# aerius-labs/zksnap-circuits-halo2

Measured on AMD Instinct MI355X. Metric: BN254 G1 MSM Mpoints/sec, higher is better.
Workload: dtype u32x9 (254-bit modular integer, radix 2^29); 1 GPU; BN254 G1 MSM, 2^20 random points/scalars per GPU (BASELINE configs[1]), point-range sharded x1, inputs resident in HBM, bases registered once (prepared fixed-base table, as under ParamsKZG::commit); points_per_gpu=1048576, parallelism=point-range shard x1 + all_gather(96 B) + fold

## Files before the change

zksnap_circuits_halo2_amd/csrc/msm.hip:

```cpp
#include <hip/hip_runtime.h>
#include <atomic>
#include <cstdint>
#include <cstdio>
#include <cstring>
#include <cstdlib>
#include <mutex>
#include "ec_quad.hpp"
#include "fe_inverse.hpp"
#include "zkhip_internal.hpp"

namespace zkhip {

static inline size_t align_up(size_t v, size_t a) { return (v + a - 1) / a * a; }

constexpr int FINE_BITS = 12;
constexpr int MAX_GROUPS = 128;
constexpr int MAX_WIDE_W = 16;
struct win_layout { int c, W, narrow; };
__host__ __device__ __forceinline__ int win_bits(const win_layout& L, int w) { return w < L.W - L.narrow ? L.c : L.c - 1; }
__host__ __device__ __forceinline__ int win_off(const win_layout& L, int w) { const int full = L.W - L.narrow; return w <= full ? w * L.c : full * L.c + (w - full) * (L.c - 1); }
static int msm_narrow_windows(int c, int W) {
  static const bool uniform = getenv("ZKHIP_UNIFORM_WINDOWS") != nullptr;
  if (c <= 16 || uniform) return 0;
  const int narrow = W * c - 256;
  return narrow > 0 && narrow <= W ? narrow : 0;
}
constexpr int MAX_TASK_LEN = 128;
constexpr int TASK_SHIFT = 6;

struct task_t {
  uint32_t bucket, start, len;
};

__device__ __forceinline__ xyzz load_xyzz(const uint32_t* base, size_t idx) {
  const uint4* q = reinterpret_cast<const uint4*>(base + idx * 36);
  uint32_t w[36];
#pragma unroll
  for (int i = 0; i < 9; i++) {
    uint4 v = q[i];
    w[4 * i] = v.x; w[4 * i + 1] = v.y; w[4 * i + 2] = v.z; w[4 * i + 3] = v.w;
  }
  xyzz r;
#pragma unroll
  for (int i = 0; i < 9; i++) { r.X.l[i] = w[i]; r.Y.l[i] = w[9 + i]; r.ZZ.l[i] = w[18 + i]; r.ZZZ.l[i] = w[27 + i]; }
  return r;
}

__device__ __forceinline__ void store_xyzz(uint32_t* base, size_t idx, const xyzz& a) {
  uint32_t w[36];
#pragma unroll
  for (int i = 0; i < 9; i++) { w[i] = a.X.l[i]; w[9 + i] = a.Y.l[i]; w[18 + i] = a.ZZ.l[i]; w[27 + i] = a.ZZZ.l[i]; }
  uint4* q = reinterpret_cast<uint4*>(base + idx * 36);
#pragma unroll
  for (int i = 0; i < 9; i++) q[i] = make_uint4(w[4 * i], w[4 * i + 1], w[4 * i + 2], w[4 * i + 3]);
}

__device__ __forceinline__ xyzz xyzz_shfl_xor(const xyzz& a, int mask) {
  xyzz r;
#pragma unroll
  for (int i = 0; i < NL; i++) {
    r.X.l[i] = (uint32_t)__shfl_xor((int)a.X.l[i], mask, 64);
    r.Y.l[i] = (uint32_t)__shfl_xor((int)a.Y.l[i], mask, 64);
    r.ZZ.l[i] = (uint32_t)__shfl_xor((int)a.ZZ.l[i], mask, 64);
    r.ZZZ.l[i] = (uint32_t)__shfl_xor((int)a.ZZZ.l[i], mask, 64);
  }
  return r;
}

__device__ __forceinline__ fe load_fe9_generic(const uint32_t* p, size_t idx) {
  fe r;
#pragma unroll
  for (int i = 0; i < 9; i++) r.l[i] = p[idx * 9 + i];
  return r;
}
__device__ __forceinline__ void store_fe9_generic(uint32_t* p, size_t idx, const fe& a) {
#pragma unroll
  for (int i = 0; i < 9; i++) p[idx * 9 + i] = a.l[i];
}

template <typename DIGIT>
__global__ void __launch_bounds__(256) k_digits(const uint32_t* __restrict__ scalars, DIGIT* __restrict__ digits,
                                                uint32_t n, uint32_t n_pad, int c, int W, uint32_t K, size_t scalar_stride, int narrow) {
  const size_t idx = (size_t)blockIdx.x * blockDim.x + threadIdx.x;
  if (idx >= (size_t)K * n_pad) return;
  const uint32_t kb = (uint32_t)(idx / n_pad), i = (uint32_t)(idx % n_pad);
  digits += (size_t)kb * n_pad;
  const size_t row = (size_t)K * n_pad;
  if (i >= n) {
    for (int win = 0; win < W; win++) digits[(size_t)win * row + i] = 0;
    return;
  }
  uint32_t w[8];
  load_words(scalars + ((size_t)kb * scalar_stride + i) * 8, w);
  fe c32;
#pragma unroll
  for (int k = 0; k < NL; k++) c32.l[k] = FrParams::FROM_EXT_CANON[k];
  fe s = fe_canon_lt2p<FrParams>(fe_mul<FrParams>(c32, fe_unpack<0>(w)));
  fe_pack(s, w);
  const win_layout lay{c, W, narrow};
  uint32_t carry = 0;
  for (int win = 0; win < W; win++) {
    const int bit = win_off(lay, win), cw = win_bits(lay, win);
    const uint32_t half = 1u << (cw - 1), mask = (1u << cw) - 1;
    uint32_t v = 0;
    if (bit < 256) {
      int wi = bit >> 5, sh = bit & 31;
      uint64_t two = w[wi];
      if (wi + 1 < 8) two |= (uint64_t)w[wi + 1] << 32;
      v = (uint32_t)(two >> sh) & mask;
    }
    v += carry;
    int32_t d;
    if (v >= half) { d = (int32_t)v - (int32_t)(1u << cw); carry = 1; } else { d = (int32_t)v; carry = 0; }
    digits[(size_t)win * row + i] = (DIGIT)d;
  }
}

__global__ void __launch_bounds__(1024) k_digits_wide(const uint32_t* __restrict__ scalars, int32_t* __restrict__ digits, uint32_t n, uint32_t n_pad,
                                                       int c, int W, uint32_t* __restrict__ gcount, int narrow) {
  __shared__ uint32_t cnt[MAX_WIDE_W * MAX_GROUPS];
  for (uint32_t t = threadIdx.x; t < (uint32_t)W * MAX_GROUPS; t += blockDim.x) cnt[t] = 0;
  __syncthreads();
  const win_layout lay{c, W, narrow};
  for (uint32_t i = blockIdx.x * blockDim.x + threadIdx.x; i < n_pad; i += gridDim.x * blockDim.x) {
    if (i >= n) {
      for (int win = 0; win < W; win++) digits[(size_t)win * n_pad + i] = 0;
      continue;
    }
    uint32_t w[8];
    load_words(scalars + (size_t)i * 8, w);
    fe c32;
#pragma unroll
    for (int k = 0; k < NL; k++) c32.l[k] = FrParams::FROM_EXT_CANON[k];
    fe sv = fe_canon_lt2p<FrParams>(fe_mul<FrParams>(c32, fe_unpack<0>(w)));
    fe_pack(sv, w);
    uint32_t carry = 0;
    for (int win = 0; win < W; win++) {
      const int bit = win_off(lay, win), cw = win_bits(lay, win);
      const uint32_t half = 1u << (cw - 1), mask = (1u << cw) - 1;
      uint32_t v = 0;
      if (bit < 256) {
        const int wi = bit >> 5, sh = bit & 31;
        uint64_t two = w[wi];
        if (wi + 1 < 8) two |= (uint64_t)w[wi + 1] << 32;
        v = (uint32_t)(two >> sh) & mask;
      }
      v += carry;
      int32_t d;
      if (v >= half) { d = (int32_t)v - (int32_t)(1u << cw); carry = 1; } else { d = (int32_t)v; carry = 0; }
      digits[(size_t)win * n_pad + i] = d;
      if (d != 0) atomicAdd(&cnt[win * MAX_GROUPS + (((uint32_t)(d < 0 ? -d : d) - 1) >> FINE_BITS)], 1u);
    }
  }
  __syncthreads();
  for (uint32_t t = threadIdx.x; t < (uint32_t)W * MAX_GROUPS; t += blockDim.x)
    if (cnt[t]) atomicAdd(&gcount[t], cnt[t]);
}

namespace glv {
__device__ constexpr uint32_t G1[3] = {0xc7e0b3d7u, 0xd91d232eu, 0x2u};
__device__ constexpr uint32_t G2[5] = {0x391eb18eu, 0x7a7bd9d4u, 0xa773d2cfu, 0x4ccef014u, 0x2u};
__device__ constexpr uint32_t A1[2] = {0x94d213e3u, 0x89d32568u};
__device__ constexpr uint32_t A2[4] = {0x1221250bu, 0x0be4e154u, 0xeeb859fdu, 0x6f4d8248u};
__device__ constexpr uint32_t NB1[4] = {0x7d4f1128u, 0x8211bbebu, 0xeeb859fcu, 0x6f4d8248u};
__device__ constexpr uint32_t BETA_EXT[8] = {0xd782e155u, 0x71930c11u, 0xffbe3323u, 0xa6bb947cu, 0xd4741444u, 0xaa303344u, 0x26594943u, 0x2c3b3f0du};

template <int NA, int NB, int NO>
__device__ __forceinline__ void mul_low(const uint32_t (&a)[NA], const uint32_t* __restrict__ b, uint32_t (&out)[NO]) {
#pragma unroll
  for (int i = 0; i < NO; i++) out[i] = 0;
#pragma unroll
  for (int i = 0; i < NA; i++) {
    uint32_t carry = 0;
#pragma unroll
    for (int j = 0; j < NB; j++) {
      if (i + j < NO) {
        const uint64_t t = (uint64_t)a[i] * b[j] + out[i + j] + carry;
        out[i + j] = (uint32_t)t;
        carry = (uint32_t)(t >> 32);
      }
    }
    if (i + NB < NO) out[i + NB] = carry;
  }
}

__device__ __forceinline__ bool abs160(uint32_t (&v)[5], uint32_t (&mag)[4]) {
  const bool neg = (v[4] >> 31) != 0;
  uint32_t carry = neg ? 1u : 0u;
#pragma unroll
  for (int i = 0; i < 4; i++) {
    const uint32_t w = neg ? ~v[i] : v[i];
    const uint32_t t = w + carry;
    carry = (t < w) ? 1u : 0u;
    mag[i] = t;
  }
  return neg;
}

__device__ __forceinline__ void decompose(const uint32_t (&k)[8], uint32_t (&m1)[4], bool& s1, uint32_t (&m2)[4], bool& s2) {
  uint32_t t1[11], t2[13];
  mul_low<8, 3, 11>(k, G1, t1);
  mul_low<8, 5, 13>(k, G2, t2);
  const uint32_t c1[2] = {t1[8], t1[9]};
  const uint32_t c2[4] = {t2[8], t2[9], t2[10], t2[11]};
  uint32_t p[5], q[5], v[5];
  mul_low<2, 2, 5>(c1, A1, p);
  mul_low<4, 4, 5>(c2, A2, q);
  uint64_t borrow = 0;
#pragma unroll
  for (int i = 0; i < 5; i++) {
    const uint64_t d = (uint64_t)k[i] - p[i] - q[i] - borrow;
    v[i] = (uint32_t)d;
    borrow = (d >> 32) ? ((~(d >> 32) + 1) & 3) : 0;
  }
  s1 = abs160(v, m1);
  mul_low<2, 4, 5>(c1, NB1, p);
  mul_low<4, 2, 5>(c2, A1, q);
  borrow = 0;
#pragma unroll
  for (int i = 0; i < 5; i++) {
    const uint64_t d = (uint64_t)p[i] - q[i] - borrow;
    v[i] = (uint32_t)d;
    borrow = (d >> 32) ? 1 : 0;
  }
  s2 = abs160(v, m2);
}
}

template <typename DIGIT>
__global__ void __launch_bounds__(256) k_digits_glv(const uint32_t* __restrict__ scalars, DIGIT* __restrict__ digits, uint32_t n, uint32_t n2_pad, int c, int W) {
  const uint32_t i = blockIdx.x * blockDim.x + threadIdx.x;
  if (i < n2_pad - 2 * n) {
    for (int win = 0; win < W; win++) digits[(size_t)win * n2_pad + 2 * n + i] = 0;
  }
  if (i >= n) return;
  uint32_t w[8];
  load_words(scalars + (size_t)i * 8, w);
  fe c32;
#pragma unroll
  for (int k = 0; k < NL; k++) c32.l[k] = FrParams::FROM_EXT_CANON[k];
  fe s = fe_canon_lt2p<FrParams>(fe_mul<FrParams>(c32, fe_unpack<0>(w)));
  fe_pack(s, w);
  uint32_t m[2][4];
  bool neg[2];
  glv::decompose(w, m[0], neg[0], m[1], neg[1]);
  const uint32_t half = 1u << (c - 1), mask = (1u << c) - 1;
#pragma unroll
  for (int h = 0; h < 2; h++) {
    uint32_t carry = 0;
    DIGIT* col = digits + (size_t)h * n + i;
    for (int win = 0; win < W; win++) {
      const int bit = win * c;
      uint32_t v = 0;
      if (bit < 128) {
        const int wi = bit >> 5, sh = bit & 31;
        uint64_t two = m[h][wi];
        if (wi + 1 < 4) two |= (uint64_t)m[h][wi + 1] << 32;
        v = (uint32_t)(two >> sh) & mask;
      }
      v += carry;
      int32_t d;
      if (neg[h] ? (v > half) : (v >= half)) { d = (int32_t)v - (int32_t)(1u << c); carry = 1; } else { d = (int32_t)v; carry = 0; }
      col[(size_t)win * n2_pad] = (DIGIT)(neg[h] ? -d : d);
    }
  }
}

__global__ void __launch_bounds__(256) k_endo_bases(const uint32_t* __restrict__ bases, uint32_t n, uint32_t* __restrict__ endo) {
  const uint32_t i = blockIdx.x * blockDim.x + threadIdx.x;
  if (i >= n) return;
  affine_words pt = load_affine(bases, i);
  uint32_t bw[8], xw[8];
#pragma unroll
  for (int k = 0; k < 8; k++) bw[k] = glv::BETA_EXT[k];
  const fe beta = fe_mul<Fq>(fe_one<Fq>(), fe_from_ext_lazy(bw));
  fe_to_ext<Fq>(fe_mul<Fq>(beta, fe_from_ext_lazy(pt.x)), xw);
  uint4* o = reinterpret_cast<uint4*>(endo + (size_t)i * 16);
  o[0] = make_uint4(xw[0], xw[1], xw[2], xw[3]);
  o[1] = make_uint4(xw[4], xw[5], xw[6], xw[7]);
  o[2] = make_uint4(pt.y[0], pt.y[1], pt.y[2], pt.y[3]);
  o[3] = make_uint4(pt.y[4], pt.y[5], pt.y[6], pt.y[7]);
}

template <bool SCATTER>
__global__ void __launch_bounds__(1024) k_sort_pass(const int16_t* __restrict__ digits, uint32_t n_pad, uint32_t chunk,
                                                    int c, uint32_t* __restrict__ count_or_cursor,
                                                    uint32_t* __restrict__ sorted, uint32_t win_bucket_stride,
                                                    uint32_t ref_base, uint32_t ref_stride) {
  extern __shared__ uint32_t hist[];
  const uint32_t B = 1u << (c - 1);
  const int win = blockIdx.y;
  const uint32_t kb = blockIdx.z, K = gridDim.z;
  const uint32_t lo = blockIdx.x * chunk;
  const uint32_t hi = min(n_pad, lo + chunk);
  for (uint32_t b = threadIdx.x; b < B; b += blockDim.x) hist[b] = 0;
  __syncthreads();
  const uint4* dv = reinterpret_cast<const uint4*>(digits + ((size_t)win * K + kb) * n_pad);
  const uint32_t v_lo = lo >> 3, v_hi = hi >> 3;
  for (uint32_t vi = v_lo + threadIdx.x; vi < v_hi; vi += blockDim.x) {
    const uint4 q = dv[vi];
    const uint32_t w[4] = {q.x, q.y, q.z, q.w};
#pragma unroll
    for (int k = 0; k < 8; k++) {
      const int d = (int16_t)(w[k >> 1] >> ((k & 1) * 16));
      if (d != 0) atomicAdd(&hist[(d < 0 ? -d : d) - 1], 1u);
    }
  }
  __syncthreads();
  uint32_t* g = count_or_cursor + (size_t)win * win_bucket_stride + (size_t)kb * B;
  if (!SCATTER) {
    for (uint32_t b = threadIdx.x; b < B; b += blockDim.x) {
      uint32_t v = hist[b];
      if (v) atomicAdd(&g[b], v);
    }
  } else {
    for (uint32_t b0 = threadIdx.x; b0 < B; b0 += 8 * blockDim.x) {
      uint32_t v[8], r[8];
#pragma unroll
      for (int k = 0; k < 8; k++) { const uint32_t b = b0 + k * blockDim.x; v[k] = b < B ? hist[b] : 0u; }
#pragma unroll
      for (int k = 0; k < 8; k++) r[k] = v[k] ? atomicAdd(&g[b0 + k * blockDim.x], v[k]) : 0u;
#pragma unroll
      for (int k = 0; k < 8; k++) { const uint32_t b = b0 + k * blockDim.x; if (b < B) hist[b] = r[k]; }
    }
    __syncthreads();
    const uint32_t rbase = ref_base + (uint32_t)win * ref_stride;
    for (uint32_t vi = v_lo + threadIdx.x; vi < v_hi; vi += blockDim.x) {
      const uint4 q = dv[vi];
      const uint32_t w[4] = {q.x, q.y, q.z, q.w};
#pragma unroll
      for (int k = 0; k < 8; k++) {
        const int d = (int16_t)(w[k >> 1] >> ((k & 1) * 16));
        if (d != 0) {
          const uint32_t pos = atomicAdd(&hist[(d < 0 ? -d : d) - 1], 1u);
          sorted[pos] = (rbase + vi * 8 + k) | (d < 0 ? 0x80000000u : 0u);
        }
      }
    }
  }
}



__global__ void __launch_bounds__(1024) k_coarse_count(const int32_t* __restrict__ digits, uint32_t n_pad, uint32_t chunk, uint32_t* __restrict__ gcount, uint32_t gstride) {
  __shared__ uint32_t cnt[MAX_GROUPS];
  const int win = blockIdx.y;
  const uint32_t lo = blockIdx.x * chunk, hi = min(n_pad, lo + chunk);
  if (threadIdx.x < MAX_GROUPS) cnt[threadIdx.x] = 0;
  __syncthreads();
  const uint4* dv = reinterpret_cast<const uint4*>(digits + (size_t)win * n_pad);
  const uint32_t v_lo = lo >> 2, v_hi = hi >> 2;
  for (uint32_t vi = v_lo + threadIdx.x; vi < v_hi; vi += 4 * blockDim.x) {
    uint4 q[4];
#pragma unroll
    for (int u = 0; u < 4; u++) { const uint32_t vj = vi + u * blockDim.x; q[u] = vj < v_hi ? dv[vj] : make_uint4(0, 0, 0, 0); }
#pragma unroll
    for (int u = 0; u < 4; u++) {
      const int32_t d4[4] = {(int32_t)q[u].x, (int32_t)q[u].y, (int32_t)q[u].z, (int32_t)q[u].w};
#pragma unroll
      for (int k = 0; k < 4; k++) {
        const int32_t d = d4[k];
        if (d != 0) atomicAdd(&cnt[(uint32_t)win * gstride + (((uint32_t)(d < 0 ? -d : d) - 1) >> FINE_BITS)], 1u);
      }
    }
  }
  __syncthreads();
  if (threadIdx.x < MAX_GROUPS && cnt[threadIdx.x]) atomicAdd(&gcount[win * MAX_GROUPS + threadIdx.x], cnt[threadIdx.x]);
}

constexpr uint32_t COARSE_CHUNK = 8192;
__global__ void __launch_bounds__(1024) k_coarse_sorted(const int32_t* __restrict__ digits, uint32_t n_pad, uint32_t* __restrict__ gcursor,
                                                        uint32_t* __restrict__ stage_ref, uint16_t* __restrict__ stage_fine,
                                                        uint32_t ref_base, uint32_t ref_stride, uint32_t gstride) {
  __shared__ uint32_t cur[MAX_GROUPS], delta[MAX_GROUPS];
  __shared__ uint32_t refs[COARSE_CHUNK];
  __shared__ uint16_t fines[COARSE_CHUNK];
  __shared__ uint32_t mask[COARSE_CHUNK / 32], wpre[COARSE_CHUNK / 32];
  const int win = blockIdx.y;
  const uint32_t gbase = (uint32_t)win * gstride;
  const uint32_t lo = blockIdx.x * COARSE_CHUNK, hi = min(n_pad, lo + COARSE_CHUNK);
  if (lo >= hi) return;
  if (threadIdx.x < MAX_GROUPS) cur[threadIdx.x] = 0;
  if (threadIdx.x < COARSE_CHUNK / 32) mask[threadIdx.x] = 0;
  __syncthreads();
  const uint4* dv = reinterpret_cast<const uint4*>(digits + (size_t)win * n_pad);
  const uint32_t v_lo = lo >> 2, v_hi = hi >> 2;
  static_assert(COARSE_CHUNK == 8192, "a lane owns two 4-digit vectors of the chunk");
  const uint32_t vi = v_lo + threadIdx.x, vj = vi + 1024u;
  const uint4 q0 = vi < v_hi ? dv[vi] : make_uint4(0, 0, 0, 0), q1 = vj < v_hi ? dv[vj] : make_uint4(0, 0, 0, 0);
  const int32_t d8[8] = {(int32_t)q0.x, (int32_t)q0.y, (int32_t)q0.z, (int32_t)q0.w, (int32_t)q1.x, (int32_t)q1.y, (int32_t)q1.z, (int32_t)q1.w};
#pragma unroll
  for (int k = 0; k < 8; k++) {
    const int32_t d = d8[k];
    if (d != 0) atomicAdd(&cur[gbase + (((uint32_t)(d < 0 ? -d : d) - 1) >> FINE_BITS)], 1u);
  }
  __syncthreads();
  if (threadIdx.x < 64) {
    const uint32_t c0 = cur[2 * threadIdx.x], c1 = cur[2 * threadIdx.x + 1], s = c0 + c1;
    uint32_t x = s;
#pragma unroll
    for (int off = 1; off < 64; off <<= 1) {
      const uint32_t y = __shfl_up(x, off, 64);
      if ((int)threadIdx.x >= off) x += y;
    }
    const uint32_t l0 = x - s, l1 = l0 + c0;
    uint32_t* const wcur = gcursor + (uint32_t)win * MAX_GROUPS;
    const uint32_t g0 = c0 ? atomicAdd(&wcur[2 * threadIdx.x], c0) : 0u, g1 = c1 ? atomicAdd(&wcur[2 * threadIdx.x + 1], c1) : 0u;
    cur[2 * threadIdx.x] = l0; cur[2 * threadIdx.x + 1] = l1;
    const uint32_t nz = (c0 != 0) + (c1 != 0);
    uint32_t y = nz;
#pragma unroll
    for (int off = 1; off < 64; off <<= 1) {
      const uint32_t t = __shfl_up(y, off, 64);
      if ((int)threadIdx.x >= off) y += t;
    }
    uint32_t rank = y - nz;
    if (c0) { delta[rank++] = g0 - l0; atomicOr(&mask[l0 >> 5], 1u << (l0 & 31)); }
    if (c1) { delta[rank] = g1 - l1; atomicOr(&mask[l1 >> 5], 1u << (l1 & 31)); }
    __threadfence_block();
    uint32_t pc[4], ps = 0;
#pragma unroll
    for (int k = 0; k < 4; k++) { pc[k] = (uint32_t)__popc(mask[4 * threadIdx.x + k]); ps += pc[k]; }
    uint32_t z = ps;
#pragma unroll
    for (int off = 1; off < 64; off <<= 1) {
      const uint32_t t = __shfl_up(z, off, 64);
      if ((int)threadIdx.x >= off) z += t;
    }
    uint32_t zb = z - ps;
#pragma unroll
    for (int k = 0; k < 4; k++) { wpre[4 * threadIdx.x + k] = zb; zb += pc[k]; }
  }
  __syncthreads();
  const uint32_t rbase = ref_base + (uint32_t)win * ref_stride;
#pragma unroll
  for (int k = 0; k < 8; k++) {
    const int32_t d = d8[k];
    if (d != 0) {
      const uint32_t b = (uint32_t)(d < 0 ? -d : d) - 1;
      const uint32_t pos = atomicAdd(&cur[gbase + (b >> FINE_BITS)], 1u);
      refs[pos] = (rbase + (k < 4 ? vi : vj) * 4 + (k & 3)) | (d < 0 ? 0x80000000u : 0u);
      fines[pos] = (uint16_t)(b & ((1u << FINE_BITS) - 1));
    }
  }
  __syncthreads();
  const uint32_t total = cur[MAX_GROUPS - 1];
  for (uint32_t i = threadIdx.x; i < total; i += blockDim.x) {
    const uint32_t r = wpre[i >> 5] + (uint32_t)__popc(mask[i >> 5] & ((2u << (i & 31)) - 1u)) - 1u;
    const uint32_t pos = delta[r] + i;
    stage_ref[pos] = refs[i];
    stage_fine[pos] = fines[i];
  }
}

constexpr uint32_t SORT_CHUNK = 28672;

__global__ void __launch_bounds__(64) k_group_offsets(const uint32_t* __restrict__ wcount, int W, int G, uint32_t* __restrict__ goff, uint32_t* __restrict__ wcursor,
                                                       uint32_t* __restrict__ cstart, uint32_t chunk) {
  if (blockIdx.x != 0 || threadIdx.x >= 64) return;
  const int lane = threadIdx.x;
  uint32_t c0 = 0, c1 = 0;
  for (int w = 0; w < W; w++) {
    if (2 * lane < G) c0 += wcount[w * MAX_GROUPS + 2 * lane];
    if (2 * lane + 1 < G) c1 += wcount[w * MAX_GROUPS + 2 * lane + 1];
  }
  const uint32_t k0 = (c0 + chunk - 1) / chunk, k1 = (c1 + chunk - 1) / chunk;
  uint32_t x = c0 + c1, y = k0 + k1;
#pragma unroll
  for (int off = 1; off < 64; off <<= 1) {
    const uint32_t xs = __shfl_up(x, off, 64), ys = __shfl_up(y, off, 64);
    if (lane >= off) { x += xs; y += ys; }
  }
  const uint32_t ex = x - (c0 + c1), ey = y - (k0 + k1);
  if (2 * lane < G) { goff[2 * lane] = ex; cstart[2 * lane] = ey; }
  if (2 * lane + 1 < G) { goff[2 * lane + 1] = ex + c0; cstart[2 * lane + 1] = ey + k0; }
  uint32_t r0 = ex, r1 = ex + c0;
  for (int w = 0; w < W; w++) {
    if (2 * lane < G) { wcursor[w * MAX_GROUPS + 2 * lane] = r0; r0 += wcount[w * MAX_GROUPS + 2 * lane]; }
    if (2 * lane + 1 < G) { wcursor[w * MAX_GROUPS + 2 * lane + 1] = r1; r1 += wcount[w * MAX_GROUPS + 2 * lane + 1]; }
  }
  if (lane == 63) { goff[G] = x; cstart[G] = y; }
}

#ifndef ZKHIP_FINE_BATCH
#define ZKHIP_FINE_BATCH 7
#endif
constexpr int FINE_BATCH = ZKHIP_FINE_BATCH;
__device__ __forceinline__ void fine_histogram(const uint16_t* __restrict__ stage_fine, uint32_t start, uint32_t end, uint32_t* __restrict__ cur) {
  for (uint32_t p = start + threadIdx.x; p < end; p += FINE_BATCH * blockDim.x) {
    uint32_t f[FINE_BATCH];
#pragma unroll
    for (int k = 0; k < FINE_BATCH; k++) { const uint32_t q = p + k * blockDim.x; f[k] = q < end ? stage_fine[q] : 0xffffffffu; }
#pragma unroll
    for (int k = 0; k < FINE_BATCH; k++) if (f[k] != 0xffffffffu) atomicAdd(&cur[f[k]], 1u);
  }
}

__global__ void __launch_bounds__(1024) k_fine_sorted(const uint16_t* __restrict__ stage_fine, const uint32_t* __restrict__ stage_ref,
                                                      const uint32_t* __restrict__ goff, const uint32_t* __restrict__ cstart, int G,
                                                      uint32_t* __restrict__ cursor, uint32_t* __restrict__ sorted) {
  extern __shared__ uint32_t hist[];
  constexpr uint32_t FB = 1u << FINE_BITS;
  constexpr uint32_t CHUNK = SORT_CHUNK;
  static_assert(FB == 4096, "one thread owns four buckets in the scan");
  __shared__ uint32_t wsum[16];
  uint32_t* cur = hist;
  uint32_t* delta = hist + FB;
  uint32_t* refs = hist + 2 * FB;
  const uint32_t w = blockIdx.x;
  if (w >= cstart[G]) return;
  uint32_t glo = 0, ghi = (uint32_t)G;
  while (ghi - glo > 1) { const uint32_t mid = (glo + ghi) >> 1; if (cstart[mid] <= w) glo = mid; else ghi = mid; }
  const uint32_t g = glo;
  const uint32_t start = goff[g] + (w - cstart[g]) * CHUNK, end = min(goff[g + 1], start + CHUNK), cnt_n = end - start;
  for (uint32_t b = threadIdx.x; b < FB; b += blockDim.x) cur[b] = 0;
  __syncthreads();
  fine_histogram(stage_fine, start, end, cur);
  __syncthreads();
  uint32_t c[4], l[4], s = 0;
#pragma unroll
  for (int k = 0; k < 4; k++) { c[k] = cur[4 * threadIdx.x + k]; s += c[k]; }
  const int lane = threadIdx.x & 63, wave = threadIdx.x >> 6;
  uint32_t x = s;
#pragma unroll
  for (int off = 1; off < 64; off <<= 1) {
    const uint32_t y = __shfl_up(x, off, 64);
    if (lane >= off) x += y;
  }
  if (lane == 63) wsum[wave] = x;
  __syncthreads();
  uint32_t before = 0;
#pragma unroll
  for (int i = 0; i < 16; i++) if (i < wave) before += wsum[i];
  uint32_t run = before + x - s;
  uint32_t* gl = cursor + (size_t)g * FB;
  uint32_t gb[4];
#pragma unroll
  for (int k = 0; k < 4; k++) { l[k] = run; run += c[k]; }
#pragma unroll
  for (int k = 0; k < 4; k++) gb[k] = c[k] ? atomicAdd(&gl[4 * threadIdx.x + k], c[k]) : 0u;
  {
    uint32_t* mask = refs + CHUNK;
    uint32_t* wpre = mask + CHUNK / 32;
    const uint32_t nz = (c[0] != 0) + (c[1] != 0) + (c[2] != 0) + (c[3] != 0);
    uint32_t y = nz;
#pragma unroll
    for (int off = 1; off < 64; off <<= 1) {
      const uint32_t t = __shfl_up(y, off, 64);
      if (lane >= off) y += t;
    }
    __syncthreads();
    if (lane == 63) wsum[wave] = y;
    for (uint32_t w2 = threadIdx.x; w2 < CHUNK / 32; w2 += blockDim.x) mask[w2] = 0;
    __syncthreads();
    uint32_t rank = y - nz;
#pragma unroll
    for (int i = 0; i < 16; i++) if (i < wave) rank += wsum[i];
#pragma unroll
    for (int k = 0; k < 4; k++) {
      cur[4 * threadIdx.x + k] = l[k];
      if (c[k]) {
        delta[rank++] = gb[k] - l[k];
        atomicOr(&mask[l[k] >> 5], 1u << (l[k] & 31));
      }
    }
    __syncthreads();
    const uint32_t pc = threadIdx.x < CHUNK / 32 ? (uint32_t)__popc(mask[threadIdx.x]) : 0u;
    uint32_t z = pc;
#pragma unroll
    for (int off = 1; off < 64; off <<= 1) {
      const uint32_t t = __shfl_up(z, off, 64);
      if (lane >= off) z += t;
    }
    __syncthreads();
    if (lane == 63) wsum[wave] = z;
    __syncthreads();
    uint32_t zb = z - pc;
#pragma unroll
    for (int i = 0; i < 16; i++) if (i < wave) zb += wsum[i];
    if (threadIdx.x < CHUNK / 32) wpre[threadIdx.x] = zb;
  }
  __syncthreads();
  {
    for (uint32_t p = start + threadIdx.x; p < end; p += FINE_BATCH * blockDim.x) {
      uint32_t f[FINE_BATCH], r[FINE_BATCH];
#pragma unroll
      for (int k = 0; k < FINE_BATCH; k++) { const uint32_t q = p + k * blockDim.x; f[k] = q < end ? stage_fine[q] : 0xffffffffu; r[k] = q < end ? stage_ref[q] : 0u; }
#pragma unroll
      for (int k = 0; k < FINE_BATCH; k++) if (f[k] != 0xffffffffu) refs[atomicAdd(&cur[f[k]], 1u)] = r[k];
    }
    __syncthreads();
    const uint32_t* mask = refs + CHUNK;
    const uint32_t* wpre = mask + CHUNK / 32;
    for (uint32_t i = threadIdx.x; i < cnt_n; i += blockDim.x) {
      const uint32_t r = wpre[i >> 5] + (uint32_t)__popc(mask[i >> 5] & ((2u << (i & 31)) - 1u)) - 1u;
      sorted[delta[r] + i] = refs[i];
    }
  }
}

__global__ void __launch_bounds__(1024) k_fine_count(const uint16_t* __restrict__ stage_fine, const uint32_t* __restrict__ goff,
                                                     const uint32_t* __restrict__ cstart, int G, uint32_t* __restrict__ count, uint32_t chunk) {
  constexpr uint32_t FB = 1u << FINE_BITS;
  __shared__ uint32_t cur[FB];
  const uint32_t w = blockIdx.x;
  if (w >= cstart[G]) return;
  uint32_t glo = 0, ghi = (uint32_t)G;
  while (ghi - glo > 1) { const uint32_t mid = (glo + ghi) >> 1; if (cstart[mid] <= w) glo = mid; else ghi = mid; }
  const uint32_t g = glo;
  const uint32_t start = goff[g] + (w - cstart[g]) * chunk, end = min(goff[g + 1], start + chunk);
  for (uint32_t b = threadIdx.x; b < FB; b += blockDim.x) cur[b] = 0;
  __syncthreads();
  fine_histogram(stage_fine, start, end, cur);
  __syncthreads();
  uint32_t* gl = count + (size_t)g * FB;
  for (uint32_t b = threadIdx.x; b < FB; b += blockDim.x) {
    const uint32_t v = cur[b];
    if (v) atomicAdd(&gl[b], v);
  }
}

constexpr int SCAN_BLOCK = 256, SCAN_PER_THREAD = 4,
          SCAN_TILE = SCAN_BLOCK * SCAN_PER_THREAD;

template <int MODE>
__device__ __forceinline__ uint32_t scan_xform(uint32_t v, uint32_t task_shift) {
  return MODE == 0 ? v : (v + (1u << task_shift) - 1) >> task_shift;
}

__device__ __forceinline__ uint32_t block_exclusive_scan(uint32_t v, uint32_t* lds, uint32_t& total) {
  const int lane = threadIdx.x & 63, wave = threadIdx.x >> 6;
  uint32_t x = v;
#pragma unroll
  for (int off = 1; off < 64; off <<= 1) {
    uint32_t y = __shfl_up(x, off, 64);
    if (lane >= off) x += y;
  }
  if (lane == 63) lds[wave] = x;
  __syncthreads();
  uint32_t base = 0, tot = 0;
#pragma unroll
  for (int i = 0; i < SCAN_BLOCK / 64; i++) {
    uint32_t t = lds[i];
    if (i < wave) base += t;
    tot += t;
  }
  __syncthreads();
  total = tot;
  return base + x - v;
}

__global__ void __launch_bounds__(SCAN_BLOCK) k_scan_sums2(const uint32_t* __restrict__ in, uint32_t n, uint32_t* __restrict__ sums0,
                                                           uint32_t* __restrict__ sums1, uint32_t task_shift) {
  __shared__ uint32_t lds[4];
  const uint32_t base = blockIdx.x * SCAN_TILE + threadIdx.x * SCAN_PER_THREAD;
  uint32_t s0 = 0, s1 = 0;
#pragma unroll
  for (int i = 0; i < SCAN_PER_THREAD; i++) if (base + i < n) { const uint32_t v = in[base + i]; s0 += v; s1 += scan_xform<1>(v, task_shift); }
  uint32_t t0, t1;
  block_exclusive_scan(s0, lds, t0);
  block_exclusive_scan(s1, lds, t1);
  if (threadIdx.x == 0) { sums0[blockIdx.x] = t0; sums1[blockIdx.x] = t1; }
}

__global__ void __launch_bounds__(SCAN_BLOCK) k_scan_top2(uint32_t* __restrict__ sums0, uint32_t* __restrict__ sums1, uint32_t nb,
                                                          uint32_t* __restrict__ total0, uint32_t* __restrict__ total1) {
  __shared__ uint32_t lds[4];
  uint32_t run0 = 0, run1 = 0;
  for (uint32_t base = 0; base < nb; base += SCAN_BLOCK) {
    const uint32_t i = base + threadIdx.x;
    const uint32_t v0 = i < nb ? sums0[i] : 0, v1 = i < nb ? sums1[i] : 0;
    uint32_t t0, t1;
    const uint32_t e0 = block_exclusive_scan(v0, lds, t0), e1 = block_exclusive_scan(v1, lds, t1);
    if (i < nb) { sums0[i] = run0 + e0; sums1[i] = run1 + e1; }
    run0 += t0; run1 += t1;
  }
  if (threadIdx.x == 0) { *total0 = run0; *total1 = run1; }
}

__global__ void __launch_bounds__(SCAN_BLOCK) k_scan_apply2(const uint32_t* __restrict__ in, uint32_t n, const uint32_t* __restrict__ sums0,
                                                            const uint32_t* __restrict__ sums1, const uint32_t* __restrict__ total0,
                                                            const uint32_t* __restrict__ total1, uint32_t* __restrict__ offset,
                                                            uint32_t* __restrict__ cursor, uint32_t* __restrict__ task_off, uint32_t task_shift) {
  __shared__ uint32_t lds[4];
  const uint32_t base = blockIdx.x * SCAN_TILE + threadIdx.x * SCAN_PER_THREAD;
  uint32_t v[SCAN_PER_THREAD], s0 = 0, s1 = 0;
#pragma unroll
  for (int i = 0; i < SCAN_PER_THREAD; i++) { v[i] = base + i < n ? in[base + i] : 0; s0 += v[i]; s1 += scan_xform<1>(v[i], task_shift); }
  uint32_t t0, t1;
  uint32_t e0 = block_exclusive_scan(s0, lds, t0) + sums0[blockIdx.x];
  uint32_t e1 = block_exclusive_scan(s1, lds, t1) + sums1[blockIdx.x];
#pragma unroll
  for (int i = 0; i < SCAN_PER_THREAD; i++) {
    if (base + i < n) { offset[base + i] = e0; cursor[base + i] = e0; task_off[base + i] = e1; }
    e0 += v[i];
    e1 += scan_xform<1>(v[i], task_shift);
  }
  if (blockIdx.x == 0 && threadIdx.x == 0) { offset[n] = *total0; task_off[n] = *total1; }
}

constexpr uint32_t SCAN_SINGLE_MAX = 8192;
template <int MODE>
__global__ void __launch_bounds__(1024) k_scan_single(const uint32_t* __restrict__ in, uint32_t n, uint32_t* __restrict__ total_out,
                                                      uint32_t* __restrict__ out, uint32_t* __restrict__ out2, uint32_t task_shift,
                                                      uint32_t* __restrict__ len_cursor) {
  __shared__ uint32_t wsum[16];
  __shared__ uint32_t lh[MAX_TASK_LEN + 1];
  if (MODE == 1 && threadIdx.x <= MAX_TASK_LEN) lh[threadIdx.x] = 0;
  __syncthreads();
  const int lane = threadIdx.x & 63, wave = threadIdx.x >> 6;
  const uint32_t full = 1u << task_shift;
  uint32_t running = 0, n_full = 0;
  for (uint32_t tile = 0; tile < n; tile += 8192) {
    const uint32_t base = tile + threadIdx.x * 8;
    uint32_t v[8], s = 0;
#pragma unroll
    for (int i = 0; i < 8; i++) {
      const uint32_t raw = base + i < n ? in[base + i] : 0u;
      v[i] = scan_xform<MODE>(raw, task_shift);
      s += v[i];
      if (MODE == 1 && raw) {
        n_full += v[i] - 1;
        atomicAdd(&lh[raw - ((v[i] - 1) << task_shift)], 1u);
      }
    }
    uint32_t x = s;
#pragma unroll
    for (int off = 1; off < 64; off <<= 1) {
      const uint32_t y = __shfl_up(x, off, 64);
      if (lane >= off) x += y;
    }
    if (lane == 63) wsum[wave] = x;
    __syncthreads();
    uint32_t before = 0, tot = 0;
#pragma unroll
    for (int i = 0; i < 16; i++) {
      const uint32_t t = wsum[i];
      if (i < wave) before += t;
      tot += t;
    }
    __syncthreads();
    uint32_t ex = running + before + x - s;
#pragma unroll
    for (int i = 0; i < 8; i++) {
      if (base + i < n) { out[base + i] = ex; if (out2) out2[base + i] = ex; }
      ex += v[i];
    }
    running += tot;
  }
  if (threadIdx.x == 0) { out[n] = running; *total_out = running; }
  if (MODE == 1) {
    if (n_full) atomicAdd(&lh[full], n_full);
    __syncthreads();
    if (threadIdx.x == 0) {
      uint32_t run = 0;
      for (int L = MAX_TASK_LEN; L >= 1; L--) { len_cursor[L] = run; run += lh[L]; }
    }
  }
}

constexpr uint32_t HEAVY_SLICE = 2048;
constexpr uint32_t COOP_TASKS = 32;
__global__ void __launch_bounds__(256) k_make_tasks(const uint32_t* __restrict__ offset, const uint32_t* __restrict__ task_off,
                                                    uint32_t nbuckets, task_t* __restrict__ tasks, uint32_t task_shift,
                                                    uint32_t* __restrict__ max_parts, uint32_t* __restrict__ len_count, uint32_t seq_parts,
                                                    uint32_t* __restrict__ heavy_count, uint2* __restrict__ heavy, uint32_t heavy_cap) {
  __shared__ uint32_t lh[MAX_TASK_LEN + 1];
  if (threadIdx.x <= MAX_TASK_LEN) lh[threadIdx.x] = 0;
  __syncthreads();
  uint32_t nt = 0;
  const uint32_t lane = threadIdx.x & 63u;
  for (uint32_t base = blockIdx.x * blockDim.x + (threadIdx.x & ~63u); base < nbuckets; base += gridDim.x * blockDim.x) {
    const uint32_t k = base + lane;
    uint32_t s = 0, e = 0, t = 0, m = 0;
    if (k < nbuckets) { s = offset[k]; e = offset[k + 1]; t = task_off[k]; m = task_off[k + 1] - t; }
    const bool coop = m > COOP_TASKS;
    if (!coop) {
      for (uint32_t j = 0; j < m; j++) {
        task_t tk;
        tk.bucket = k;
        tk.start = s + (j << task_shift);
        tk.len = min(1u << task_shift, e - tk.start);
        tasks[t + j] = tk;
      }
    }
    if (m) {
      if (m > 1) atomicAdd(&lh[1u << task_shift], m - 1);
      atomicAdd(&lh[(e - s) - ((m - 1) << task_shift)], 1u);
    }
    if (m > seq_parts) {
      const uint32_t P = (m + HEAVY_SLICE - 1) / HEAVY_SLICE;
      const uint32_t idx = atomicAdd(heavy_count, P);
      for (uint32_t i = 0; i < P; i++)
        if (idx + i < heavy_cap) heavy[idx + i] = make_uint2(k, i);
    }
    nt = max(nt, m);
    unsigned long long big = __ballot(coop);
    while (big) {
      const int src = __ffsll((long long)big) - 1;
      big &= big - 1;
      const uint32_t bk = (uint32_t)__shfl((int)k, src, 64), bs = (uint32_t)__shfl((int)s, src, 64), be = (uint32_t)__shfl((int)e, src, 64),
                     bt = (uint32_t)__shfl((int)t, src, 64), bm = (uint32_t)__shfl((int)m, src, 64);
      for (uint32_t j = lane; j < bm; j += 64) {
        task_t tk;
        tk.bucket = bk;
        tk.start = bs + (j << task_shift);
        tk.len = min(1u << task_shift, be - tk.start);
        tasks[bt + j] = tk;
      }
    }
  }
  __syncthreads();
  if (len_count && threadIdx.x <= MAX_TASK_LEN && lh[threadIdx.x]) atomicAdd(&len_count[threadIdx.x], lh[threadIdx.x]);
#pragma unroll
  for (int off = 32; off >= 1; off >>= 1) nt = max(nt, (uint32_t)__shfl_xor((int)nt, off, 64));
  if ((threadIdx.x & 63) == 0 && nt > 1) atomicMax(max_parts, nt);
}

__global__ void k_order_offsets(const uint32_t* __restrict__ len_count, uint32_t* __restrict__ len_cursor) {
  static_assert(MAX_TASK_LEN == 128, "two lengths per lane of one wavefront");
  if (blockIdx.x != 0 || threadIdx.x >= 64) return;
  const int lane = threadIdx.x, L0 = MAX_TASK_LEN - 2 * lane, L1 = L0 - 1;
  const uint32_t c0 = len_count[L0], c1 = len_count[L1];
  uint32_t x = c0 + c1;
#pragma unroll
  for (int off = 1; off < 64; off <<= 1) {
    const uint32_t y = __shfl_up(x, off, 64);
    if (lane >= off) x += y;
  }
  const uint32_t ex = x - (c0 + c1);
  len_cursor[L0] = ex;
  len_cursor[L1] = ex + c0;
}

constexpr int ORDER_JMAX = 64;
__global__ void __launch_bounds__(256) k_make_order(const uint32_t* __restrict__ offset, const uint32_t* __restrict__ task_off,
                                                    uint32_t nbuckets, uint32_t task_shift, uint32_t* __restrict__ len_cursor,
                                                    const uint32_t* __restrict__ sorted, uint4* __restrict__ order) {
  __shared__ uint32_t lh[MAX_TASK_LEN + 1];
  __shared__ uint32_t jcnt[ORDER_JMAX + 1], joff[ORDER_JMAX + 1];
  if (threadIdx.x <= MAX_TASK_LEN) lh[threadIdx.x] = 0;
  if (threadIdx.x <= ORDER_JMAX) jcnt[threadIdx.x] = 0;
  __syncthreads();
  const uint32_t full = 1u << task_shift, step = gridDim.x * blockDim.x;
  for (uint32_t k = blockIdx.x * blockDim.x + threadIdx.x; k < nbuckets; k += step) {
    const uint32_t nt = task_off[k + 1] - task_off[k];
    if (nt) {
      const uint32_t rem = (offset[k + 1] - offset[k]) - ((nt - 1) << task_shift);
      atomicAdd(&lh[rem], 1u);
      const uint32_t nfull = nt - 1, head = min(nfull, (uint32_t)ORDER_JMAX);
      for (uint32_t j = 0; j < head; j++) atomicAdd(&jcnt[j], 1u);
      if (nfull > head) atomicAdd(&jcnt[ORDER_JMAX], nfull - head);
    }
  }
  __syncthreads();
  if (threadIdx.x == 0) {
    uint32_t run = 0;
    for (int j = 0; j <= ORDER_JMAX; j++) { joff[j] = run; run += jcnt[j]; }
    const uint32_t base = run ? atomicAdd(&len_cursor[full], run) : 0u;
    for (int j = 0; j <= ORDER_JMAX; j++) joff[j] += base;
  }
  if (threadIdx.x <= MAX_TASK_LEN && threadIdx.x != full) { const uint32_t v = lh[threadIdx.x]; lh[threadIdx.x] = v ? atomicAdd(&len_cursor[threadIdx.x], v) : 0u; }
  __syncthreads();
  if (threadIdx.x == 0 && lh[full]) lh[full] = atomicAdd(&len_cursor[full], lh[full]);
  __syncthreads();
  const uint32_t lane = threadIdx.x & 63u;
  for (uint32_t base = blockIdx.x * blockDim.x + (threadIdx.x & ~63u); base < nbuckets; base += step) {
    const uint32_t k = base + lane;
    uint32_t t = 0, nt = 0, s0 = 0, pos = 0, nfull = 0, head = 0;
    if (k < nbuckets) { t = task_off[k]; nt = task_off[k + 1] - t; }
    if (nt) {
      s0 = offset[k];
      const uint32_t rem = (offset[k + 1] - s0) - ((nt - 1) << task_shift);
      nfull = nt - 1;
      head = min(nfull, (uint32_t)ORDER_JMAX);
      for (uint32_t j = 0; j < head; j++) {
        const uint32_t st = s0 + (j << task_shift);
        order[atomicAdd(&joff[j], 1u)] = make_uint4(t + j, st, full, sorted[st]);
      }
      if (nfull > head) pos = atomicAdd(&joff[ORDER_JMAX], nfull - head);
      const uint32_t st = s0 + ((nt - 1) << task_shift);
      order[atomicAdd(&lh[rem], 1u)] = make_uint4(nt == 1 ? (0x80000000u | k) : t + nt - 1, st, rem, sorted[st]);
    }
    const bool coop = nfull - head > COOP_TASKS;
    if (!coop) {
      for (uint32_t j = head; j < nfull; j++) {
        const uint32_t st = s0 + (j << task_shift);
        order[pos + j - head] = make_uint4(t + j, st, full, sorted[st]);
      }
    }
    unsigned long long big = __ballot(coop);
    while (big) {
      const int src = __ffsll((long long)big) - 1;
      big &= big - 1;
      const uint32_t bt = (uint32_t)__shfl((int)t, src, 64), bs0 = (uint32_t)__shfl((int)s0, src, 64), bpos = (uint32_t)__shfl((int)pos, src, 64),
                     bnfull = (uint32_t)__shfl((int)nfull, src, 64), bhead = (uint32_t)__shfl((int)head, src, 64);
      for (uint32_t j = bhead + lane; j < bnfull; j += 64) {
        const uint32_t st = bs0 + (j << task_shift);
        order[bpos + j - bhead] = make_uint4(bt + j, st, full, sorted[st]);
      }
    }
  }
}

template <bool TABLE>
__global__ void __launch_bounds__(128) __attribute__((amdgpu_waves_per_eu(4, 4))) k_accumulate(const task_t* __restrict__ tasks, const uint32_t* __restrict__ ntasks_p,
                                                    const uint4* __restrict__ order, const uint32_t* __restrict__ sorted,
                                                    const uint32_t* __restrict__ bases, uint32_t* __restrict__ partials,
                                                    uint32_t* __restrict__ buckets, const uint32_t* __restrict__ bases2, uint32_t split) {
  auto point = [&](uint32_t idx) -> affine_words {
    if constexpr (!TABLE) { if (idx >= split) return load_affine(bases2, idx - split); }
    return load_affine(bases, idx);
  };
  const uint32_t ntasks = *ntasks_p;
  for (uint32_t i = blockIdx.x * blockDim.x + threadIdx.x; i < ntasks; i += gridDim.x * blockDim.x) {
    const uint4 rec = order[i];
    const uint32_t t = rec.x;
    struct { uint32_t start, len; } tk = {rec.y, rec.z};
    xyzz acc = xyzz_identity();
    const uint32_t* refs = sorted + tk.start;
    uint32_t ref = rec.w;
    affine_words pt = point(ref & 0x7fffffffu);
    uint32_t j = 0;
    if constexpr (TABLE) {
      if (!affine_is_identity(pt)) {
        acc.X = fe_unpack<0>(pt.x);
        acc.Y = fe_unpack<0>(pt.y);
        if (ref >> 31) acc.Y = fe_norm(fe_neg_red(acc.Y, Fq::P2_S1));
        acc.ZZ = acc.ZZZ = fe_one<Fq>();
      }
      if (tk.len > 1) {
        ref = refs[1];
        pt = point(ref & 0x7fffffffu);
      }
      j = 1;
    }
    uint32_t nref = j + 1 < tk.len ? refs[j + 1] : 0u;
    for (; j < tk.len; j++) {
      affine_words cur = pt;
      uint32_t cref = ref;
      if (j + 1 < tk.len) {
        ref = nref;
        pt = point(ref & 0x7fffffffu);
      }
      if (j + 2 < tk.len) nref = refs[j + 2];
      if (affine_is_identity(cur)) continue;
      fe x2, y2;
      if constexpr (TABLE) {
        x2 = fe_unpack<0>(cur.x);
        y2 = fe_unpack<0>(cur.y);
        if (cref >> 31) y2 = fe_neg_red(y2, Fq::P2_S1);
      } else {
        x2 = fe_from_ext_lazy(cur.x);
        y2 = fe_from_ext_lazy(cur.y);
        if (cref >> 31) y2 = fe_neg_red(y2, Fq::P64_S1);
      }
      xyzz_madd<true>(acc, x2, y2);
    }
    if (t >> 31) store_xyzz(buckets, t & 0x7fffffffu, acc);
    else store_xyzz(partials, t, acc);
  }
}

constexpr uint32_t HEAVY_WGS = 256;
constexpr uint32_t HEAVY_QUAD_MAX = 256;

__device__ __forceinline__ xyzz workgroup_sum_128(xyzz acc, uint32_t* __restrict__ xch) {
#pragma unroll 1
  for (uint32_t half = 64; half >= 1; half >>= 1) {
    __syncthreads();
    if (threadIdx.x >= half && threadIdx.x < 2 * half) store_xyzz(xch, threadIdx.x - half, acc);
    __syncthreads();
    if (threadIdx.x < half) acc = xyzz_add(acc, load_xyzz(xch, threadIdx.x));
  }
  return acc;
}

__device__ __forceinline__ void combine_heavy_buckets(uint32_t wg, const uint32_t* __restrict__ task_off, uint32_t* __restrict__ partials,
                                                      uint32_t* __restrict__ buckets, const uint32_t* __restrict__ heavy_count,
                                                      const uint2* __restrict__ heavy, uint32_t heavy_cap, uint32_t* __restrict__ heavy_done,
                                                      uint32_t* __restrict__ xch , uint32_t quad_max) {
  __shared__ uint32_t is_last;
  const uint32_t nh = min(*heavy_count, heavy_cap);
  for (uint32_t i = wg; i < nh; i += HEAVY_WGS) {
    const uint2 e = heavy[i];
    const uint32_t k = e.x, sl = e.y, t = task_off[k], m = task_off[k + 1] - t;
    const uint32_t P = (m + HEAVY_SLICE - 1) / HEAVY_SLICE, lo = sl * HEAVY_SLICE, hi = min(m, lo + HEAVY_SLICE);
    if (m <= quad_max) {
      const uint32_t q = threadIdx.x & 3, quad = threadIdx.x >> 2;
      xyzz acc = xyzz_identity();
#pragma unroll 1
      for (uint32_t j = quad; j < m; j += 32) acc = xyzz_add_quad(acc, load_xyzz(partials, t + j), q);
#pragma unroll 1
      for (int mask = 4; mask < 64; mask <<= 1) acc = xyzz_add_quad(acc, xyzz_shfl_xor(acc, mask), q);
      __syncthreads();
      if (threadIdx.x == 64) store_xyzz(xch, 0, acc);
      __syncthreads();
      if (threadIdx.x < 4) {
        acc = xyzz_add_quad(acc, load_xyzz(xch, 0), q);
        if (q == 0) store_xyzz(buckets, k, acc);
      }
      continue;
    }
    xyzz acc = xyzz_identity();
#pragma unroll 1
    for (uint32_t j = lo + threadIdx.x; j < hi; j += 128) acc = xyzz_add(acc, load_xyzz(partials, t + j));
    acc = workgroup_sum_128(acc, xch);
    if (P == 1) {
      if (threadIdx.x == 0) store_xyzz(buckets, k, acc);
      continue;
    }
    if (threadIdx.x == 0) {
      store_xyzz(partials, t + lo, acc);
      __threadfence();
      is_last = atomicAdd(&heavy_done[i - sl], 1u) == P - 1;
    }
    __syncthreads();
    if (!is_last) continue;
    __threadfence();
    acc = xyzz_identity();
#pragma unroll 1
    for (uint32_t j = threadIdx.x; j < P; j += 128) acc = xyzz_add(acc, load_xyzz(partials, t + j * HEAVY_SLICE));
    acc = workgroup_sum_128(acc, xch);
    if (threadIdx.x == 0) store_xyzz(buckets, k, acc);
  }
}

template <int COMBINE_LANES>
__global__ void __launch_bounds__(128) k_combine_seq(const uint32_t* __restrict__ task_off, uint32_t nbuckets,
                                                     uint32_t* __restrict__ partials, uint32_t* __restrict__ buckets,
                                                     uint32_t seq_parts, uint32_t blocks, const uint32_t* __restrict__ heavy_count,
                                                     const uint2* __restrict__ heavy, uint32_t heavy_cap, uint32_t* __restrict__ heavy_done, uint32_t quad_max) {
  __shared__ __attribute__((aligned(16))) uint32_t xch[64 * 36];
  if (blockIdx.x >= blocks) { combine_heavy_buckets(blockIdx.x - blocks, task_off, partials, buckets, heavy_count, heavy, heavy_cap, heavy_done, xch, quad_max); return; }
  const uint32_t gid = blockIdx.x * blockDim.x + threadIdx.x;
  const uint32_t k = gid / COMBINE_LANES, q = gid % COMBINE_LANES;
  const bool live = k < nbuckets;
  xyzz acc = xyzz_identity();
  uint32_t m = 0;
  if (live) {
    const uint32_t t = task_off[k];
    m = task_off[k + 1] - t;
    const uint32_t left = (m == 1 || m > seq_parts) ? 0u : m;
#pragma unroll 1
    for (uint32_t j = q; j < left; j += COMBINE_LANES) acc = xyzz_add(acc, load_xyzz(partials, t + j));
  }
#pragma unroll 1
  for (int mask = 1; mask < COMBINE_LANES; mask <<= 1) acc = xyzz_add(acc, xyzz_shfl_xor(acc, mask));
  if (live && q == 0 && m != 1 && m <= seq_parts) store_xyzz(buckets, k, acc);
}

template <int COMBINE_LANES>
__global__ void __launch_bounds__(128) k_combine_seq_quad(const uint32_t* __restrict__ task_off, uint32_t nbuckets,
                                                          uint32_t* __restrict__ partials, uint32_t* __restrict__ buckets,
                                                          uint32_t seq_parts, uint32_t blocks, const uint32_t* __restrict__ heavy_count,
                                                          const uint2* __restrict__ heavy, uint32_t heavy_cap, uint32_t* __restrict__ heavy_done, uint32_t quad_max) {
  __shared__ __attribute__((aligned(16))) uint32_t xch[64 * 36];
  if (blockIdx.x >= blocks) { combine_heavy_buckets(blockIdx.x - blocks, task_off, partials, buckets, heavy_count, heavy, heavy_cap, heavy_done, xch, quad_max); return; }
  const uint32_t gid = blockIdx.x * blockDim.x + threadIdx.x;
  const uint32_t q = gid & 3, lane = (gid >> 2) % COMBINE_LANES, k = (gid >> 2) / COMBINE_LANES;
  const bool live = k < nbuckets;
  xyzz acc = xyzz_identity();
  uint32_t m = 0;
  if (live) {
    const uint32_t t = task_off[k];
    m = task_off[k + 1] - t;
    const uint32_t left = (m == 1 || m > seq_parts) ? 0u : m;
#pragma unroll 1
    for (uint32_t j = lane; j < left; j += COMBINE_LANES) acc = xyzz_add_quad(acc, load_xyzz(partials, t + j), q);
  }
#pragma unroll 1
  for (int mask = 1; mask < COMBINE_LANES; mask <<= 1) acc = xyzz_add_quad(acc, xyzz_shfl_xor(acc, 4 * mask), q);
  if (live && lane == 0 && q == 0 && m != 1 && m <= seq_parts) store_xyzz(buckets, k, acc);
}

__global__ void __launch_bounds__(128) k_pyramid_step(const uint32_t* __restrict__ in, uint32_t* __restrict__ out,
                                                      uint32_t N, int s, uint32_t in_stride, uint32_t out_stride) {
  const uint32_t per_win = N / 2 + (uint32_t)s * (N / 4);
  const int win = blockIdx.y;
  const uint32_t* wi = in + (size_t)win * in_stride * 36;
  uint32_t* wo = out + (size_t)win * out_stride * 36;
#pragma unroll 1
  for (uint32_t tid = blockIdx.x * blockDim.x + threadIdx.x; tid < per_win; tid += gridDim.x * blockDim.x) {
    uint32_t ia, ib;
    if (tid < N / 2) {
      ia = 2 * tid; ib = 2 * tid + 1;
    } else {
      uint32_t r = tid - N / 2;
      uint32_t l = r / (N / 4), u = r % (N / 4);
      if ((int)l == s - 1) { ia = 4 * u + 1; ib = 4 * u + 3; }
      else { ia = N + l * (N / 2) + 2 * u; ib = ia + 1; }
    }
    store_xyzz(wo, tid, xyzz_add(load_xyzz(wi, ia), load_xyzz(wi, ib)));
  }
}

__global__ void __launch_bounds__(128) k_pyramid_step_quad(const uint32_t* __restrict__ in, uint32_t* __restrict__ out,
                                                           uint32_t N, int s, uint32_t in_stride, uint32_t out_stride) {
  const uint32_t per_win = N / 2 + (uint32_t)s * (N / 4);
  const uint32_t gid = blockIdx.x * blockDim.x + threadIdx.x;
  const uint32_t tid = gid >> 2, q = gid & 3;
  if (tid >= per_win) return;
  const int win = blockIdx.y;
  const uint32_t* wi = in + (size_t)win * in_stride * 36;
  uint32_t* wo = out + (size_t)win * out_stride * 36;
  uint32_t ia, ib;
  if (tid < N / 2) {
    ia = 2 * tid; ib = 2 * tid + 1;
  } else {
    uint32_t r = tid - N / 2;
    uint32_t l = r / (N / 4), u = r % (N / 4);
    if ((int)l == s - 1) { ia = 4 * u + 1; ib = 4 * u + 3; }
    else { ia = N + l * (N / 2) + 2 * u; ib = ia + 1; }
  }
  const xyzz r = xyzz_add_quad(load_xyzz(wi, ia), load_xyzz(wi, ib), q);
  if (q == 0) store_xyzz(wo, tid, r);
}

__global__ void __launch_bounds__(64) k_window_horner(const uint32_t* __restrict__ in, uint32_t in_stride, int nz,
                                                      uint32_t* __restrict__ winsum, int W) {
  const int gid = blockIdx.x * blockDim.x + threadIdx.x;
  const int win = gid >> 5, lane = gid & 31;
  xyzz acc = xyzz_identity();
  if (win < W) {
    const uint32_t* wi = in + (size_t)win * in_stride * 36;
    int dbl = 0;
    if (lane < nz) { acc = load_xyzz(wi, 2 + lane); dbl = lane; }
    else if (lane == nz) { acc = load_xyzz(wi, 1); dbl = nz; }
    else if (lane == nz + 1) acc = xyzz_add(load_xyzz(wi, 0), load_xyzz(wi, 1));
#pragma unroll 1
    for (int i = 0; i < dbl; i++) acc = xyzz_dbl(acc);
  }
#pragma unroll 1
  for (int mask = 1; mask < 32; mask <<= 1) acc = xyzz_add(acc, xyzz_shfl_xor(acc, mask));
  if (win < W && lane == 0) store_xyzz(winsum, win, acc);
}

__global__ void __launch_bounds__(128) k_window_horner_quad(const uint32_t* __restrict__ in, uint32_t in_stride, int nz,
                                                            uint32_t* __restrict__ winsum, uint32_t* __restrict__ jac_out) {
  __shared__ __attribute__((aligned(16))) uint32_t xch[36];
  const int win = blockIdx.x, term = threadIdx.x >> 2;
  const uint32_t q = threadIdx.x & 3;
  const uint32_t* wi = in + (size_t)win * in_stride * 36;
  xyzz acc = xyzz_identity();
  int dbl = 0;
  if (term < nz) { acc = load_xyzz(wi, 2 + term); dbl = term; }
  else if (term == nz) { acc = load_xyzz(wi, 1); dbl = nz; }
  else if (term == nz + 1) acc = xyzz_add_quad(load_xyzz(wi, 0), load_xyzz(wi, 1), q);
#pragma unroll 1
  for (int i = 0; i < dbl; i++) acc = xyzz_dbl_quad(acc, q);
#pragma unroll 1
  for (int mask = 4; mask < 64; mask <<= 1) acc = xyzz_add_quad(acc, xyzz_shfl_xor(acc, mask), q);
  if (threadIdx.x == 64) store_xyzz(xch, 0, acc);
  __syncthreads();
  if (threadIdx.x < 4) {
    acc = xyzz_add_quad(acc, load_xyzz(xch, 0), q);
    if (q == 0) {
      if (jac_out) store_jacobian(acc, jac_out + (size_t)win * 24);
      else store_xyzz(winsum, win, acc);
    }
  }
}

__global__ void __launch_bounds__(64) k_fold(const uint32_t* __restrict__ winsum, int W, int c, uint32_t* __restrict__ out) {
  if (threadIdx.x >= 4 || blockIdx.x != 0) return;
  const uint32_t q = threadIdx.x;
  xyzz acc = load_xyzz(winsum, W - 1);
  for (int w = W - 2; w >= 0; w--) {
#pragma unroll 1
    for (int i = 0; i < c; i++) acc = xyzz_dbl_quad(acc, q);
    acc = xyzz_add_quad(acc, load_xyzz(winsum, w), q);
  }
  if (q == 0) store_jacobian(acc, out);
}

__global__ void __launch_bounds__(64) k_store_results(const uint32_t* __restrict__ winsum, uint32_t K, uint32_t* __restrict__ out) {
  const uint32_t k = blockIdx.x * blockDim.x + threadIdx.x;
  if (k < K) store_jacobian(load_xyzz(winsum, k), out + (size_t)k * 24);
}

__global__ void __launch_bounds__(64) k_sum_jacobian(const uint32_t* __restrict__ in, int m, uint32_t* __restrict__ out, uint32_t stride) {
  const uint32_t q = threadIdx.x & 3;
  const int grp = threadIdx.x >> 2;
  in += (size_t)blockIdx.x * 24;
  out += (size_t)blockIdx.x * 24;
  xyzz acc = xyzz_identity();
  for (int i = grp; i < m; i += 16) acc = xyzz_add_quad(acc, load_jacobian(in + (size_t)i * stride * 24), q);
#pragma unroll 1
  for (int mask = 4; mask < 64; mask <<= 1) {
    if ((mask >> 2) >= m && mask > 4) break;
    acc = xyzz_add_quad(acc, xyzz_shfl_xor(acc, mask), q);
  }
  if (threadIdx.x == 0) store_jacobian(acc, out);
}

static bool msm_top_window_is_degenerate(int c) {
  const int W = (256 + c - 1) / c, top_bits = 254 - (W - 1) * c;
  return top_bits > 0 && top_bits < 6;
}

static bool msm_glv_enabled() {
  static const bool on = getenv("ZKHIP_NO_GLV") == nullptr;
  return on;
}
static inline int msm_windows(int c, bool glv) {
  if (!glv) return (256 + c - 1) / c;
  return (128 + c - 1) / c + ((c == 2 || c == 4) ? 1 : 0);
}

int msm_pick_window(size_t n) {
  const bool glv = msm_glv_enabled();
  int best = 16;
  double best_cost = 1e300;
  for (int c = 2; c <= 16; c++) {
    const int Wi = msm_windows(c, glv), top_bits = (glv ? 127 : 254) - (Wi - 1) * c;
    if (top_bits > 0 && top_bits < 6) continue;
    const double cost = (double)Wi * (10.0 * (double)(glv ? 2 * n : n) + 28.0 * (double)(1u << (c - 1)));
    if (cost < best_cost) { best_cost = cost; best = c; }
  }
  return best;
}


constexpr int MAX_WINDOW_PREPARED = 20;

int msm_pick_window_prepared(size_t n) {
  const bool large = n >= ((size_t)1 << 20);
  int best = 2;
  double best_cost = 1e300;
  for (int c = 2; c <= MAX_WINDOW_PREPARED; c++) {
    const double W = (256 + c - 1) / c, buckets = (double)(1u << (c - 1));
    if (msm_top_window_is_degenerate(c) && c <= 16) continue;
    if (c > 16 && !large) continue;
    if (c == 17) continue;
    double cost;
    if (!large) cost = W * 10.0 * (double)n + 28.0 * buckets;
    else {
      const double eff = c == 20 ? 1.0 : (c == 19 ? 1.13 : (c == 18 ? 1.06 : 1.07));
      cost = W * (10.0 * eff + 1.0) * (double)n + 39.0 * buckets + 1.1e6 * (double)(c - 2) + 13.0e6;
    }
    if (cost < best_cost) { best_cost = cost; best = c; }
  }
  if (n >= ((size_t)1 << 14) && n < ((size_t)3 << 14)) best = 15;
  if (const char* e = getenv("ZKHIP_MAX_WINDOW")) { int m = atoi(e); if (m >= 2 && best > m) best = m; }
  return best;
}

struct msm_layout {
  uint32_t task_shift;
  size_t max_tasks;
  void* digits;
  uint32_t* stage_ref; uint16_t* stage_fine;
  char* zero_lo; size_t zero_bytes;
  uint32_t *gcounters, *counters, *count, *sorted, *offset, *cursor, *task_off, *bsum1, *bsum2;
  task_t* tasks; uint4* order;
  uint32_t *partials, *pyrA, *pyrB, *winsum;
  uint32_t* endo;
  int combine_lanes;
  uint32_t seq_parts;
  uint2* heavy; uint32_t heavy_cap;
  uint32_t* heavy_done;
  size_t total;
};

static uint32_t msm_task_shift(size_t entries , size_t NB, size_t xyzz_bytes = 144) {
  uint32_t task_shift = TASK_SHIFT;
  static const int knob = [] { const char* e = getenv("ZKHIP_TASK_SHIFT"); return e ? atoi(e) : 0; }();
  if (knob >= 2 && knob <= 7) task_shift = (uint32_t)knob;
  else if ((entries >> 7) >= ((size_t)3 << 16)) task_shift = 7;
  const bool g2 = xyzz_bytes == 288;
  if ((entries >> TASK_SHIFT) < ((size_t)1 << (g2 ? 14 : 17))) {
    const double occ = (double)entries / (double)NB;
    double best = 1e300;
    for (uint32_t sh = 2; sh <= (uint32_t)TASK_SHIFT; sh++) {
      const double L = (double)(1u << sh), parts = occ / L;
      const double est = 5.0 * L + (g2 ? 15.0 : 10.0) * (parts > 1.0 ? parts - 1.0 : 0.0);
      if (est < best) { best = est; task_shift = sh; }
    }
  }
  return task_shift;
}

static bool msm_two_level(int c, bool glv, size_t n_in, bool shared_buckets, size_t K) {
  if (c > 16) return true;
  static const long thr_glv = [] { const char* e = getenv("ZKHIP_GLV_TWO_LEVEL_MIN"); return e ? atol(e) : (1L << 18); }();
  static const long thr_prep = [] { const char* e = getenv("ZKHIP_PREP_TWO_LEVEL_MIN"); return e ? atol(e) : (1L << 16); }();
  if (c != 16 || K != 1) return false;
  if (glv) return thr_glv > 0 && n_in >= (size_t)thr_glv;
  return shared_buckets && thr_prep > 0 && n_in >= (size_t)thr_prep;
}

static msm_layout msm_lay_out(char* base, size_t n_in, size_t K, int c, bool prepared, size_t xyzz_bytes = 144, bool glv = false) {
  msm_layout L;
  const size_t n = glv ? 2 * n_in : n_in;
  const size_t W = (size_t)msm_windows(c, glv), B = (size_t)1 << (c - 1), WB = prepared ? K : W, NB = WB * B;
  const bool wide = msm_two_level(c, glv, n_in, prepared, K);
  const size_t nk = n * K, entries = W * nk;
  const size_t n_pad = (n + 7) & ~(size_t)7;
  L.task_shift = msm_task_shift(entries, NB, xyzz_bytes);
  L.max_tasks = (entries >> L.task_shift) + NB + 1;
  const double parts_avg = (double)entries / (double)NB / (double)(1u << L.task_shift);
  L.combine_lanes = parts_avg <= 2.0 ? 1 : (parts_avg <= 4.0 ? 2 : (parts_avg <= 12.0 ? 4 : 8));
  L.seq_parts = 16u * (uint32_t)L.combine_lanes;
  L.heavy_cap = (uint32_t)(std::min<size_t>(L.max_tasks / (L.seq_parts + 1) + 1, NB) + L.max_tasks / HEAVY_SLICE + 1);
  char* p = base;
  auto carve = [&](size_t bytes) { void* r = p; p += align_up(bytes, 256); return r; };
  L.digits = carve(W * K * n_pad * (wide ? sizeof(int32_t) : sizeof(int16_t)));
  L.stage_ref = wide ? (uint32_t*)carve(entries * sizeof(uint32_t)) : nullptr;
  L.stage_fine = wide ? (uint16_t*)carve(entries * sizeof(uint16_t)) : nullptr;
  L.zero_lo = p;
  L.gcounters = wide ? (uint32_t*)carve(32768) : nullptr;
  L.counters = (uint32_t*)carve(2048);
  L.count = (uint32_t*)carve((NB + 1) * sizeof(uint32_t));
  L.heavy_done = (uint32_t*)carve((size_t)L.heavy_cap * sizeof(uint32_t));
  L.zero_bytes = (size_t)(p - L.zero_lo);
  L.sorted = (uint32_t*)carve(entries * sizeof(uint32_t));
  L.offset = (uint32_t*)carve((NB + 1) * sizeof(uint32_t));
  L.cursor = (uint32_t*)carve((NB + 1) * sizeof(uint32_t));
  L.task_off = (uint32_t*)carve((NB + 1) * sizeof(uint32_t));
  L.heavy = (uint2*)carve((size_t)L.heavy_cap * sizeof(uint2));
  L.bsum1 = (uint32_t*)carve((NB / SCAN_TILE + 2) * sizeof(uint32_t));
  L.bsum2 = (uint32_t*)carve((NB / SCAN_TILE + 2) * sizeof(uint32_t));
  L.tasks = (task_t*)carve(L.max_tasks * sizeof(task_t));
  L.order = (uint4*)carve(L.max_tasks * sizeof(uint4));
  L.partials = (uint32_t*)carve(L.max_tasks * xyzz_bytes);
  L.pyrA = (uint32_t*)carve(WB * B * xyzz_bytes);
  L.pyrB = (uint32_t*)carve(WB * B * xyzz_bytes);
  L.winsum = (uint32_t*)carve((W + K) * xyzz_bytes);
  L.endo = glv ? (uint32_t*)carve(n_in * (xyzz_bytes == 288 ? 128 : 64)) : nullptr;
  L.total = (size_t)(p - base);
  return L;
}

bool msm_uses_glv(bool prepared, size_t batch, size_t xyzz_bytes) { return !prepared && batch == 1 && (xyzz_bytes == 144 || xyzz_bytes == 288) && msm_glv_enabled(); }
int msm_glv_windows(int c) { return msm_windows(c, true); }

int msm_direct_max_log() {
  static const int v = [] { const char* e = getenv("ZKHIP_DIRECT_MAX_LOG"); const int x = e ? atoi(e) : 15; return (x >= 0 && x <= 18) ? x : 15; }();
  return v;
}
static inline bool msm_direct_wanted(size_t n) { const int L = msm_direct_max_log(); return L > 0 && n >= 2 && n <= ((size_t)1 << L); }

size_t msm_workspace_bytes(size_t n_one, int c, bool prepared, size_t batch, size_t xyzz_bytes) {
  if (n_one == 0 || batch == 0) return 0;
  size_t b = msm_lay_out(nullptr, n_one, batch, c, prepared, xyzz_bytes, msm_uses_glv(prepared, batch, xyzz_bytes)).total;
  if (prepared && batch == 1 && xyzz_bytes == 144 && msm_direct_wanted(n_one)) b = std::max(b, msm_direct_workspace_bytes(n_one));
  return b;
}

int msm_build_tasks(const uint32_t* d_scalars, size_t n_in, size_t batch, size_t scalar_stride, int c, bool shared_buckets, uint32_t ref_base, uint32_t ref_stride,
                    size_t xyzz_bytes, void* ws, size_t ws_bytes, hipStream_t stream, msm_tasks_view* out, bool glv) {
  const uint32_t K = (uint32_t)batch;
  const bool wide = msm_two_level(c, glv, n_in, shared_buckets, batch);
  const int W = msm_windows(c, glv);
  if (glv && (K != 1 || c > 16 || shared_buckets)) { set_error("msm: GLV digits are for one vector of the general path"); return ZKHIP_EINVAL; }
  const size_t n = glv ? 2 * n_in : n_in;
  const uint32_t B = 1u << (c - 1);
  const int WB = shared_buckets ? (int)K : W;
  const uint32_t NB = (uint32_t)WB * B;
  if ((size_t)W * n * K >= (1ull << 32) || (size_t)WB * B >= (1ull << 31)) { set_error("msm: W*n*batch overflows 32-bit slot index"); return ZKHIP_EINVAL; }
  if (c > 16 && (!shared_buckets || K != 1)) { set_error("msm: windows above 16 bits need one shared bucket set"); return ZKHIP_EINVAL; }
  if (wide && !shared_buckets && (size_t)W * (B >> FINE_BITS) > (size_t)MAX_GROUPS) { set_error("msm: two-level sort: %d windows x %u groups exceed %d", W, B >> FINE_BITS, MAX_GROUPS); return ZKHIP_EINVAL; }
  if (wide && W > MAX_WIDE_W) { set_error("msm: %d windows of %d bits exceed the wide path's %d", W, c, MAX_WIDE_W); return ZKHIP_EINVAL; }
  const msm_layout lay = msm_lay_out((char*)ws, n_in, K, c, shared_buckets, xyzz_bytes, glv);
  if (ws_bytes < lay.total) { set_error("msm: workspace too small (%zu < %zu bytes)", ws_bytes, lay.total); return ZKHIP_EINVAL; }
  const uint32_t task_shift = lay.task_shift;
  const uint32_t n_pad = (uint32_t)((n + 7) & ~(size_t)7);
  void* const digits = lay.digits;
  uint32_t* const stage_ref = lay.stage_ref;
  uint16_t* const stage_fine = lay.stage_fine;
  uint32_t *const gcounters = lay.gcounters, *const counters = lay.counters, *const count = lay.count, *const sorted = lay.sorted,
           *const offset = lay.offset, *const cursor = lay.cursor, *const task_off = lay.task_off, *const bsum1 = lay.bsum1, *const bsum2 = lay.bsum2;
  task_t* const tasks = lay.tasks;
  uint4* const order = lay.order;

  prof_begin(stream);
  HIPCHK(hipMemsetAsync(lay.zero_lo, 0, lay.zero_bytes, stream));
  const size_t sstride = K > 1 ? scalar_stride : n;
  const size_t nk = n * K, max_tasks = lay.max_tasks;
  (void)nk; (void)max_tasks;
  const unsigned dblocks = (unsigned)(((size_t)K * n_pad + 255) / 256);
  const int narrow = (shared_buckets && !glv) ? msm_narrow_windows(c, W) : 0;
  if (glv && wide) hipLaunchKernelGGL(k_digits_glv<int32_t>, dim3((unsigned)((std::max<size_t>(n_in, 8) + 255) / 256)), dim3(256), 0, stream, d_scalars, (int32_t*)digits, (uint32_t)n_in, n_pad, c, W);
  else if (glv) hipLaunchKernelGGL(k_digits_glv<int16_t>, dim3((unsigned)((std::max<size_t>(n_in, 8) + 255) / 256)), dim3(256), 0, stream, d_scalars, (int16_t*)digits, (uint32_t)n_in, n_pad, c, W);
  else if (wide) {
    static const bool fused_count = getenv("ZKHIP_NO_FUSED_COUNT") == nullptr;
    if (fused_count) {
      static const unsigned wg_knob = [] { const char* e = getenv("ZKHIP_DIGIT_WGS"); const int v = e ? atoi(e) : 0; return v >= 64 && v <= 4096 ? (unsigned)v : 0u; }();
      const unsigned wg_cap = wg_knob ? wg_knob : (n_pad > (1u << 21) ? 1024u : 512u);
      const unsigned wblocks = (unsigned)std::min<size_t>(((size_t)n_pad + 1023) / 1024, wg_cap);
      hipLaunchKernelGGL(k_digits_wide, dim3(wblocks), dim3(1024), 0, stream, d_scalars, (int32_t*)digits, (uint32_t)n, n_pad, c, W, gcounters + 1024, narrow);
    } else {
      hipLaunchKernelGGL(k_digits<int32_t>, dim3(dblocks), dim3(256), 0, stream, d_scalars, (int32_t*)digits, (uint32_t)n, n_pad, c, W, K, sstride, narrow);
    }
  }
  else hipLaunchKernelGGL(k_digits<int16_t>, dim3(dblocks), dim3(256), 0, stream, d_scalars, (int16_t*)digits, (uint32_t)n, n_pad, c, W, K, sstride, 0);
  prof_mark(stream, "digits");
  uint32_t chunks = (uint32_t)((n + 65535) / 65536);
  while (chunks * (uint32_t)W * K < 256 && chunks < (n + 4095) / 4096) chunks *= 2;
  if (chunks == 0) chunks = 1;
  const uint32_t chunk = (uint32_t)((((n + chunks - 1) / chunks) + 7) & ~(size_t)7);
  const size_t lds = wide ? ((size_t)4 << FINE_BITS) : (size_t)B * sizeof(uint32_t);
  static std::once_flag attr_once[64];
  static hipError_t attr_err[64];
  int cur_dev = 0;
  HIPCHK(hipGetDevice(&cur_dev));
  std::call_once(attr_once[cur_dev & 63], [&] {
    hipError_t e = hipFuncSetAttribute((const void*)k_sort_pass<false>, hipFuncAttributeMaxDynamicSharedMemorySize, 128 * 1024);
    if (e == hipSuccess) e = hipFuncSetAttribute((const void*)k_sort_pass<true>, hipFuncAttributeMaxDynamicSharedMemorySize, 128 * 1024);
    if (e == hipSuccess) e = hipFuncSetAttribute((const void*)k_fine_sorted, hipFuncAttributeMaxDynamicSharedMemorySize, (2 * (1 << FINE_BITS) + SORT_CHUNK + SORT_CHUNK / 16) * 4);
    attr_err[cur_dev & 63] = e;
  });
  HIPCHK(attr_err[cur_dev & 63]);
  const uint32_t gstride = (wide && !shared_buckets) ? (B >> FINE_BITS) : 0u;
  const int G = wide ? (int)(gstride ? (uint32_t)W * gstride : (B >> FINE_BITS)) : 1;
  const uint32_t sort_chunk = SORT_CHUNK;
  const uint32_t sort_chunks = (uint32_t)(((size_t)W * n + sort_chunk - 1) / sort_chunk) + (uint32_t)G;
  const uint32_t wb_stride = shared_buckets ? 0u : B;
  if (wide) {
    static const bool fused_count2 = getenv("ZKHIP_NO_FUSED_COUNT") == nullptr;
    if (!fused_count2 || glv)
      hipLaunchKernelGGL(k_coarse_count, dim3(chunks, W), dim3(1024), 0, stream, (const int32_t*)digits, n_pad, chunk, gcounters + 1024, gstride);
    hipLaunchKernelGGL(k_group_offsets, dim3(1), dim3(64), 0, stream, gcounters + 1024, W, G, gcounters + 128, gcounters + 3072, gcounters + 512, sort_chunk);
    static_assert(MAX_GROUPS == 128, "k_coarse_sorted scans two groups per lane of one wavefront");
    hipLaunchKernelGGL(k_coarse_sorted, dim3((n_pad + COARSE_CHUNK - 1) / COARSE_CHUNK, W), dim3(1024), 0, stream, (const int32_t*)digits, n_pad, gcounters + 3072,
                       stage_ref, stage_fine, ref_base, ref_stride, gstride);
    prof_mark(stream, "coarse");
    hipLaunchKernelGGL(k_fine_count, dim3(sort_chunks), dim3(1024), 0, stream, stage_fine, gcounters + 128, gcounters + 512, G, count, sort_chunk);
  } else {
    hipLaunchKernelGGL(k_sort_pass<false>, dim3(chunks, W, K), dim3(1024), lds, stream, (const int16_t*)digits, n_pad, chunk, c, count, (uint32_t*)nullptr, wb_stride, ref_base, ref_stride);
  }
  prof_mark(stream, "count");
  const uint32_t nblk = (NB + SCAN_TILE - 1) / SCAN_TILE;
  const bool scan_single = NB <= SCAN_SINGLE_MAX;
  if (scan_single) {
    hipLaunchKernelGGL(k_scan_single<0>, dim3(1), dim3(1024), 0, stream, count, (uint32_t)NB, counters + 0, offset, cursor, 0u, (uint32_t*)nullptr);
  } else {
    hipLaunchKernelGGL(k_scan_sums2, dim3(nblk), dim3(SCAN_BLOCK), 0, stream, count, NB, bsum1, bsum2, task_shift);
    hipLaunchKernelGGL(k_scan_top2, dim3(1), dim3(SCAN_BLOCK), 0, stream, bsum1, bsum2, nblk, counters + 0, counters + 1);
    hipLaunchKernelGGL(k_scan_apply2, dim3(nblk), dim3(SCAN_BLOCK), 0, stream, count, NB, bsum1, bsum2, counters + 0, counters + 1, offset, cursor, task_off, task_shift);
  }
  prof_mark(stream, "scan");
  if (wide) {
    hipLaunchKernelGGL(k_fine_sorted, dim3(sort_chunks), dim3(1024), (size_t)(2u * (1u << FINE_BITS) + SORT_CHUNK + SORT_CHUNK / 16) * 4, stream, stage_fine, stage_ref,
                       gcounters + 128, gcounters + 512, G, cursor, sorted);
  }
  else hipLaunchKernelGGL(k_sort_pass<true>, dim3(chunks, W, K), dim3(1024), lds, stream, (const int16_t*)digits, n_pad, chunk, c, cursor, sorted, wb_stride, ref_base, ref_stride);
  prof_mark(stream, "scatter");
  static const unsigned task_wg_cap = [] { const char* e = getenv("ZKHIP_TASK_WGS"); const int v = e ? atoi(e) : 0; return v >= 1 && v <= 4096 ? (unsigned)v : 256u; }();
  const unsigned task_blocks = (unsigned)std::min<size_t>((NB + 255) / 256, task_wg_cap);
  if (scan_single) {
    hipLaunchKernelGGL(k_scan_single<1>, dim3(1), dim3(1024), 0, stream, count, (uint32_t)NB, counters + 1, task_off, (uint32_t*)nullptr, task_shift, counters + 192);
    hipLaunchKernelGGL(k_make_tasks, dim3(task_blocks), dim3(256), 0, stream, offset, task_off, NB, tasks, task_shift, counters + 2, (uint32_t*)nullptr, lay.seq_parts,
                       counters + 3, lay.heavy, lay.heavy_cap);
  } else {
    hipLaunchKernelGGL(k_make_tasks, dim3(task_blocks), dim3(256), 0, stream, offset, task_off, NB, tasks, task_shift, counters + 2, counters + 32, lay.seq_parts,
                       counters + 3, lay.heavy, lay.heavy_cap);
    hipLaunchKernelGGL(k_order_offsets, dim3(1), dim3(64), 0, stream, counters + 32, counters + 192);
  }
  hipLaunchKernelGGL(k_make_order, dim3(task_blocks), dim3(256), 0, stream, offset, task_off, NB, task_shift, counters + 192, sorted, order);
  prof_mark(stream, "tasks");
  out->c = c; out->W = W; out->WB = WB; out->B = B; out->NB = NB; out->task_shift = task_shift; out->max_tasks = lay.max_tasks; out->nk = n * K;
  out->tasks = tasks; out->ntasks = counters + 1; out->max_parts = counters + 2; out->order = order; out->sorted = sorted; out->task_off = task_off;
  out->partials = lay.partials; out->pyrA = lay.pyrA; out->pyrB = lay.pyrB; out->winsum = lay.winsum;
  out->combine_lanes = lay.combine_lanes; out->seq_parts = lay.seq_parts; out->heavy_count = counters + 3; out->heavy = lay.heavy; out->heavy_cap = lay.heavy_cap; out->heavy_done = lay.heavy_done;
  out->endo = lay.endo;
  HIPCHK(hipGetLastError());
  return ZKHIP_OK;
}

static int msm_accumulate_combine(const msm_tasks_view& tv, const uint32_t* d_bases, bool prepared, bool glv, size_t n, uint32_t* buckets, hipStream_t stream) {
  const uint32_t NB = tv.NB;
  const size_t max_tasks = tv.max_tasks;
  const task_t* const tasks = (const task_t*)tv.tasks;
  uint32_t* const counters = tv.ntasks - 1;
  const uint4* const order = tv.order;
  const uint32_t *const sorted = tv.sorted, *const task_off = tv.task_off;
  uint32_t* const partials = tv.partials;
  {
    uint32_t blocks = (uint32_t)((max_tasks + 127) / 128);
    if (blocks > 256 * 64) blocks = 256 * 64;
    if (prepared) hipLaunchKernelGGL(k_accumulate<true>, dim3(blocks), dim3(128), 0, stream, tasks, counters + 1, order, sorted, d_bases, partials, buckets, (const uint32_t*)nullptr, 0xffffffffu);
    else hipLaunchKernelGGL(k_accumulate<false>, dim3(blocks), dim3(128), 0, stream, tasks, counters + 1, order, sorted, d_bases, partials, buckets, (const uint32_t*)tv.endo,
                            glv ? (uint32_t)n : 0xffffffffu);
  }
  prof_mark(stream, "accumulate");
  {
    const int combine_lanes = tv.combine_lanes;
    const uint32_t seq_parts = tv.seq_parts;
    const size_t lanes_total = (size_t)NB * combine_lanes;
    const bool quad = lanes_total * 4 <= 131072;
    static const uint32_t heavy_quad_max = [] { const char* e = getenv("ZKHIP_HEAVY_QUAD_MAX"); const long v = e ? atol(e) : -1; return v >= 0 && v <= 2048 ? (uint32_t)v : HEAVY_QUAD_MAX; }();
    const unsigned blocks = (unsigned)((lanes_total * (quad ? 4 : 1) + 127) / 128);
#define ZK_LAUNCH_COMBINE(L)                                                                                                                        \
    do {                                                                                                                                              \
      if (quad) hipLaunchKernelGGL(k_combine_seq_quad<L>, dim3(blocks + HEAVY_WGS), dim3(128), 0, stream, task_off, NB, partials, buckets, seq_parts, blocks,   \
                                   tv.heavy_count, (const uint2*)tv.heavy, tv.heavy_cap, tv.heavy_done, heavy_quad_max);                              \
      else hipLaunchKernelGGL(k_combine_seq<L>, dim3(blocks + HEAVY_WGS), dim3(128), 0, stream, task_off, NB, partials, buckets, seq_parts, blocks,             \
                              tv.heavy_count, (const uint2*)tv.heavy, tv.heavy_cap, tv.heavy_done, heavy_quad_max);                                   \
    } while (0)
    if (combine_lanes == 1) ZK_LAUNCH_COMBINE(1);
    else if (combine_lanes == 2) ZK_LAUNCH_COMBINE(2);
    else if (combine_lanes == 4) ZK_LAUNCH_COMBINE(4);
    else ZK_LAUNCH_COMBINE(8);
#undef ZK_LAUNCH_COMBINE
  }
  prof_mark(stream, "combine");
  return ZKHIP_OK;
}

static int msm_reduce_buckets(int WB, uint32_t B, int c, uint32_t K, bool prepared, uint32_t* cur, uint32_t* nxt, uint32_t* winsum, uint32_t* d_out, hipStream_t stream) {
  static const size_t quad_max = [] { const char* e = getenv("ZKHIP_PYR_QUAD_MAX"); const long v = e ? atol(e) : 0; return v >= 256 && v <= (1 << 20) ? (size_t)v : (size_t)65536; }();
  static const long pyr_persist = [] { const char* e = getenv("ZKHIP_PYR_PERSIST"); const long v = e ? atol(e) : 0; return v >= 64 && v <= 65536 ? v : 0L; }();
  uint32_t in_stride = B;
  int nz = 0;
  {
    uint32_t N = B;
    int s = 1;
    while (N > 2) {
      uint32_t per_win = N / 2 + (uint32_t)s * (N / 4);
      uint32_t out_stride = per_win;
      if ((size_t)per_win * WB <= quad_max) hipLaunchKernelGGL(k_pyramid_step_quad, dim3((4 * per_win + 127) / 128, WB), dim3(128), 0, stream, cur, nxt, N, s, in_stride, out_stride);
      else {
        unsigned blocks = (per_win + 127) / 128;
        if (pyr_persist > 0 && WB == 1) blocks = std::min<unsigned>(blocks, (unsigned)pyr_persist);
        hipLaunchKernelGGL(k_pyramid_step, dim3(blocks, WB), dim3(128), 0, stream, cur, nxt, N, s, in_stride, out_stride);
      }
      uint32_t* t = cur; cur = nxt; nxt = t;
      in_stride = out_stride;
      N >>= 1;
      s++;
    }
    nz = s - 1;
  }
  prof_mark(stream, "pyramid");
  if (B == 1) { set_error("msm: internal: B == 1"); return ZKHIP_EINVAL; }
  const bool direct = prepared && WB <= 2048;
  if (WB <= 2048) hipLaunchKernelGGL(k_window_horner_quad, dim3(WB), dim3(128), 0, stream, cur, in_stride, nz, winsum, direct ? d_out : (uint32_t*)nullptr);
  else hipLaunchKernelGGL(k_window_horner, dim3((WB * 32 + 63) / 64), dim3(64), 0, stream, cur, in_stride, nz, winsum, WB);
  prof_mark(stream, "horner");
  if (prepared) { if (!direct) hipLaunchKernelGGL(k_store_results, dim3((K + 63) / 64), dim3(64), 0, stream, winsum, K, d_out); }
  else hipLaunchKernelGGL(k_fold, dim3(1), dim3(64), 0, stream, winsum, WB, c, d_out);
  prof_mark(stream, "fold");
  HIPCHK(hipGetLastError());
  return ZKHIP_OK;
}

int msm_g1_device(const uint32_t* d_scalars, const uint32_t* d_bases, size_t n, uint32_t* d_out, void* ws, size_t ws_bytes,
                  int c_override, hipStream_t stream, const prepared_bases* prepared, size_t prepared_off, size_t batch,
                  size_t scalar_stride) {
  if (batch == 0) return ZKHIP_OK;
  if (n == 0) {
    for (size_t k = 0; k < batch; k++) hipLaunchKernelGGL(k_sum_jacobian, dim3(1), dim3(64), 0, stream, (const uint32_t*)nullptr, 0, d_out + k * 24, 1u);
    HIPCHK(hipGetLastError());
    return ZKHIP_OK;
  }
  if (batch > 1 && (!prepared || prepared->c > 16 || batch > 65535)) { set_error("msm: batch needs prepared bases with a window <= 16 bits"); return ZKHIP_EINVAL; }
  const uint32_t K = (uint32_t)batch;
  if (n >= (1ull << 31)) { set_error("msm: n = %zu too large", n); return ZKHIP_EINVAL; }
  const int c = prepared ? prepared->c : (c_override > 0 ? c_override : msm_pick_window(n));
  if (c < 2 || c > (prepared ? MAX_WINDOW_PREPARED : 16)) { set_error("msm: window bits %d out of range", c); return ZKHIP_EINVAL; }
  if (prepared) {
    if (prepared_off + n > prepared->n) { set_error("msm: range exceeds the prepared bases"); return ZKHIP_EINVAL; }
    if ((size_t)((256 + c - 1) / c) * prepared->n >= (1ull << 31)) { set_error("msm: prepared table too large for 31-bit point references"); return ZKHIP_EINVAL; }
    d_bases = prepared->table;
    if (prepared->direct && batch == 1) return msm_g1_direct(d_scalars, n, prepared, prepared_off, d_out, ws, ws_bytes, stream);
  }
  msm_tasks_view tv;
  const bool glv = msm_uses_glv(prepared != nullptr, batch, 144);
  int rc = msm_build_tasks(d_scalars, n, batch, scalar_stride, c, prepared != nullptr, prepared ? (uint32_t)prepared_off : 0u, prepared ? (uint32_t)prepared->n : 0u,
                           144, ws, ws_bytes, stream, &tv, glv);
  if (rc != ZKHIP_OK) return rc;
  if (glv) hipLaunchKernelGGL(k_endo_bases, dim3((unsigned)((n + 255) / 256)), dim3(256), 0, stream, d_bases, (uint32_t)n, tv.endo);
  if ((rc = msm_accumulate_combine(tv, d_bases, prepared != nullptr, glv, n, tv.pyrA, stream)) != ZKHIP_OK) return rc;
  return msm_reduce_buckets(tv.WB, tv.B, c, K, prepared != nullptr, tv.pyrA, tv.pyrB, tv.winsum, d_out, stream);
}

__global__ void __launch_bounds__(128) k_bucket_sets_add(uint32_t* __restrict__ acc, const uint32_t* __restrict__ add, uint32_t nb) {
  const uint32_t k = blockIdx.x * blockDim.x + threadIdx.x;
  if (k >= nb) return;
  store_xyzz(acc, k, xyzz_add(load_xyzz(acc, k), load_xyzz(add, k)));
}

static size_t msm_chunk_lay_bytes(size_t chunk_cap, int c) {
  size_t b = msm_lay_out(nullptr, chunk_cap, 1, c, true).total;
  if (chunk_cap > 1) b = std::max(b, msm_lay_out(nullptr, chunk_cap - 1, 1, c, true).total);
  return align_up(b, 256);
}

size_t msm_chunk_workspace_bytes(size_t chunk_cap, int c) {
  if (chunk_cap == 0) return 0;
  return msm_chunk_lay_bytes(chunk_cap, c) + align_up(((size_t)1 << (c - 1)) * 144, 256);
}

int msm_chunk_add(const uint32_t* d_scalars, size_t n, const prepared_bases* pb, size_t pb_off, size_t chunk_cap, bool first, void* ws, size_t ws_bytes, hipStream_t stream) {
  if (!pb || n == 0 || n > chunk_cap || pb_off + n > pb->n) { set_error("msm_chunk_add: bad piece (n = %zu, capacity %zu)", n, chunk_cap); return ZKHIP_EINVAL; }
  const size_t lay_bytes = msm_chunk_lay_bytes(chunk_cap, pb->c);
  if (ws_bytes < msm_chunk_workspace_bytes(chunk_cap, pb->c)) { set_error("msm_chunk_add: workspace too small"); return ZKHIP_EINVAL; }
  uint32_t* const acc = (uint32_t*)((char*)ws + lay_bytes);
  msm_tasks_view tv;
  int rc = msm_build_tasks(d_scalars, n, 1, 0, pb->c, true, (uint32_t)pb_off, (uint32_t)pb->n, 144, ws, lay_bytes, stream, &tv, false);
  if (rc != ZKHIP_OK) return rc;
  if ((rc = msm_accumulate_combine(tv, pb->table, true, false, n, first ? acc : tv.pyrA, stream)) != ZKHIP_OK) return rc;
  if (!first) hipLaunchKernelGGL(k_bucket_sets_add, dim3((tv.NB + 127) / 128), dim3(128), 0, stream, acc, (const uint32_t*)tv.pyrA, tv.NB);
  HIPCHK(hipGetLastError());
  return ZKHIP_OK;
}

int msm_chunk_finish(const prepared_bases* pb, size_t chunk_cap, uint32_t* d_out, void* ws, size_t ws_bytes, hipStream_t stream) {
  if (!pb || ws_bytes < msm_chunk_workspace_bytes(chunk_cap, pb->c)) { set_error("msm_chunk_finish: workspace too small"); return ZKHIP_EINVAL; }
  const msm_layout lay = msm_lay_out((char*)ws, chunk_cap, 1, pb->c, true);
  uint32_t* const acc = (uint32_t*)((char*)ws + msm_chunk_lay_bytes(chunk_cap, pb->c));
  return msm_reduce_buckets(1, 1u << (pb->c - 1), pb->c, 1, true, acc, lay.pyrA, lay.winsum, d_out, stream);
}


constexpr int GEN_CHUNK = 32;

__device__ __forceinline__ xyzz scalar_mul_affine(const uint32_t (&kw)[8], const fe& gx, const fe& gy) {
  xyzz acc = xyzz_identity();
  for (int bit = 255; bit >= 0; bit--) {
    acc = xyzz_dbl(acc);
    if ((kw[bit >> 5] >> (bit & 31)) & 1) xyzz_madd(acc, gx, gy);
  }
  return acc;
}

__device__ __forceinline__ fe fq_inverse(const fe& a) { return fe_inverse<Fq>(a); }

__global__ void __launch_bounds__(64) k_gen_walk(const uint32_t* __restrict__ t0_d ,
                                                 uint32_t n, uint32_t* __restrict__ out, uint32_t* __restrict__ tmp_pts,
                                                 uint32_t* __restrict__ tmp_pref) {
  const uint32_t j = blockIdx.x * blockDim.x + threadIdx.x;
  const uint32_t lo = j * GEN_CHUNK;
  if (lo >= n) return;
  const uint32_t cnt = min((uint32_t)GEN_CHUNK, n - lo);
  uint32_t w0[8], wd[8], kw[8];
#pragma unroll
  for (int i = 0; i < 8; i++) { w0[i] = t0_d[i]; wd[i] = t0_d[8 + i]; }
  fe one_r = fe_one<FrParams>();
  fe t0 = fe_mul<FrParams>(one_r, fe_from_ext_lazy(w0));
  fe dd = fe_mul<FrParams>(one_r, fe_from_ext_lazy(wd));
  fe lo_f = fe_zero();
  lo_f.l[0] = lo & LMASK; lo_f.l[1] = lo >> LB;
  fe r2; 
#pragma unroll
  for (int i = 0; i < NL; i++) r2.l[i] = FrParams::R2[i];
  fe lo_m = fe_mul<FrParams>(r2, lo_f);
  fe k = fe_norm(fe_add(t0, fe_mul<FrParams>(lo_m, dd)));
  fe raw1;
#pragma unroll
  for (int i = 0; i < NL; i++) raw1.l[i] = FrParams::RAW_ONE[i];
  fe kc = fe_canon_lt2p<FrParams>(fe_mul<FrParams>(raw1, k));
  fe_pack(kc, kw);
  fe dc = fe_canon_lt2p<FrParams>(fe_mul<FrParams>(raw1, dd));
  uint32_t dw[8];
  fe_pack(dc, dw);
  fe gx = fe_one<Fq>();
  fe gy = fe_norm(fe_dbl(gx));
  xyzz P = scalar_mul_affine(kw, gx, gy);
  xyzz D = scalar_mul_affine(dw, gx, gy);
  fe pref = fe_one<Fq>();
  for (uint32_t i = 0; i < cnt; i++) {
    store_xyzz(tmp_pts, lo + i, P);
    store_fe9_generic(tmp_pref, lo + i, pref);
    if (!xyzz_is_identity(P)) pref = fe_mul<Fq>(pref, fe_mul<Fq>(P.ZZ, P.ZZZ));
    P = xyzz_add(P, D);
  }
  fe inv = fq_inverse(pref);
  for (uint32_t ii = cnt; ii-- > 0;) {
    xyzz Q = load_xyzz(tmp_pts, lo + ii);
    uint32_t* o = out + (size_t)(lo + ii) * 16;
    if (xyzz_is_identity(Q)) {
#pragma unroll
      for (int t = 0; t < 16; t++) o[t] = 0;
      continue;
    }
    fe pre = load_fe9_generic(tmp_pref, lo + ii);
    fe winv = fe_mul<Fq>(inv, pre);
    inv = fe_mul<Fq>(inv, fe_mul<Fq>(Q.ZZ, Q.ZZZ));
    fe x = fe_mul<Fq>(fe_mul<Fq>(winv, Q.ZZZ), Q.X);
    fe y = fe_mul<Fq>(fe_mul<Fq>(winv, Q.ZZ), Q.Y);
    uint32_t wx[8], wy[8];
    fe_to_ext<Fq>(x, wx);
    fe_to_ext<Fq>(y, wy);
#pragma unroll
    for (int t = 0; t < 8; t++) { o[t] = wx[t]; o[8 + t] = wy[t]; }
  }
}

static void fr_pow2_montgomery(int e, uint32_t out[8]) {
  static const uint64_t RMOD[4] = {0x43e1f593f0000001ull, 0x2833e84879b97091ull, 0xb85045b68181585dull, 0x30644e72e131a029ull};
  uint64_t v[4] = {0xac96341c4ffffffbull, 0x36fc76959f60cd29ull, 0x666ea36f7879462eull, 0x0e0a77c19a07df2full};
  for (int k = 0; k < e; k++) {
    uint64_t carry = 0;
    for (int i = 0; i < 4; i++) { const uint64_t nc = v[i] >> 63; v[i] = (v[i] << 1) | carry; carry = nc; }
    bool ge = true;
    for (int i = 3; i >= 0; i--) { if (v[i] != RMOD[i]) { ge = v[i] > RMOD[i]; break; } }
    if (ge) {
      unsigned __int128 borrow = 0;
      for (int i = 0; i < 4; i++) {
        const unsigned __int128 d = (unsigned __int128)v[i] - RMOD[i] - borrow;
        v[i] = (uint64_t)d;
        borrow = (d >> 64) ? 1 : 0;
      }
    }
  }
  for (int i = 0; i < 4; i++) { out[2 * i] = (uint32_t)v[i]; out[2 * i + 1] = (uint32_t)(v[i] >> 32); }
}

size_t g1_gen_walk_workspace(size_t n) { return align_up(n * 144, 256) + align_up(n * 36, 256) + 256; }

int g1_gen_walk_device(const uint32_t t0_ext[8], const uint32_t d_ext[8], size_t n, uint32_t* d_out, void* ws, size_t ws_bytes, hipStream_t stream) {
  if (n == 0) return ZKHIP_OK;
  if (n >= (1ull << 31)) { set_error("gen_walk: n too large"); return ZKHIP_EINVAL; }
  if (ws_bytes < g1_gen_walk_workspace(n)) { set_error("gen_walk: workspace too small"); return ZKHIP_EINVAL; }
  char* p = (char*)ws;
  uint32_t* tmp_pts = (uint32_t*)p; p += align_up(n * 144, 256);
  uint32_t* tmp_pref = (uint32_t*)p; p += align_up(n * 36, 256);
  uint32_t* consts = (uint32_t*)p;
  uint32_t h[16];
  memcpy(h, t0_ext, 32); memcpy(h + 8, d_ext, 32);
  HIPCHK(hipMemcpyAsync(consts, h, 64, hipMemcpyHostToDevice, stream));
  HIPCHK(hipStreamSynchronize(stream));
  const uint32_t threads = (uint32_t)((n + GEN_CHUNK - 1) / GEN_CHUNK);
  hipLaunchKernelGGL(k_gen_walk, dim3((threads + 63) / 64), dim3(64), 0, stream, consts, (uint32_t)n, d_out, tmp_pts, tmp_pref);
  HIPCHK(hipGetLastError());
  return ZKHIP_OK;
}


constexpr int FIXED_C = 16, FIXED_W = 16, FIXED_CHUNK = 32;
constexpr uint32_t FIXED_B = 1u << (FIXED_C - 1);

__global__ void __launch_bounds__(64) k_fixed_base_mul(const uint32_t* __restrict__ scalars, uint32_t n, const uint32_t* __restrict__ table,
                                                       uint32_t* __restrict__ out, uint32_t* __restrict__ tmp_pts, uint32_t* __restrict__ tmp_pref) {
  const uint32_t j = blockIdx.x * blockDim.x + threadIdx.x;
  const uint32_t lo = j * FIXED_CHUNK;
  if (lo >= n) return;
  const uint32_t cnt = min((uint32_t)FIXED_CHUNK, n - lo);
  fe c32;
#pragma unroll
  for (int k = 0; k < NL; k++) c32.l[k] = FrParams::FROM_EXT_CANON[k];
  fe pref = fe_one<Fq>();
  for (uint32_t i = 0; i < cnt; i++) {
    uint32_t w[8];
    load_words(scalars + (size_t)(lo + i) * 8, w);
    fe_pack(fe_canon_lt2p<FrParams>(fe_mul<FrParams>(c32, fe_unpack<0>(w))), w);
    xyzz acc = xyzz_identity();
    uint32_t carry = 0;
#pragma unroll 1
    for (int win = 0; win < FIXED_W; win++) {
      const uint32_t v = ((w[win >> 1] >> ((win & 1) * 16)) & 0xffffu) + carry;
      int32_t d;
      if (v >= FIXED_B) { d = (int32_t)v - (int32_t)(1u << FIXED_C); carry = 1; } else { d = (int32_t)v; carry = 0; }
      if (d == 0) continue;
      const affine_words pt = load_affine(table, (size_t)win * FIXED_B + (uint32_t)(d < 0 ? -d : d) - 1);
      fe y2 = fe_from_ext_lazy(pt.y);
      if (d < 0) y2 = fe_neg_red(y2, Fq::P64_S1);
      xyzz_madd(acc, fe_from_ext_lazy(pt.x), y2);
    }
    store_xyzz(tmp_pts, lo + i, acc);
    store_fe9_generic(tmp_pref, lo + i, pref);
    if (!xyzz_is_identity(acc)) pref = fe_mul<Fq>(pref, fe_mul<Fq>(acc.ZZ, acc.ZZZ));
  }
  fe inv = fq_inverse(pref);
  for (uint32_t ii = cnt; ii-- > 0;) {
    const xyzz Q = load_xyzz(tmp_pts, lo + ii);
    uint32_t* o = out + (size_t)(lo + ii) * 16;
    if (xyzz_is_identity(Q)) {
#pragma unroll
      for (int t = 0; t < 16; t++) o[t] = 0;
      continue;
    }
    const fe pre = load_fe9_generic(tmp_pref, lo + ii);
    const fe winv = fe_mul<Fq>(inv, pre);
    inv = fe_mul<Fq>(inv, fe_mul<Fq>(Q.ZZ, Q.ZZZ));
    const fe x = fe_mul<Fq>(fe_mul<Fq>(winv, Q.ZZZ), Q.X);
    const fe y = fe_mul<Fq>(fe_mul<Fq>(winv, Q.ZZ), Q.Y);
    uint32_t wx[8], wy[8];
    fe_to_ext<Fq>(x, wx);
    fe_to_ext<Fq>(y, wy);
#pragma unroll
    for (int t = 0; t < 8; t++) { o[t] = wx[t]; o[8 + t] = wy[t]; }
  }
}

size_t g1_fixed_base_table_bytes() { return (size_t)FIXED_W * FIXED_B * 64; }
size_t g1_fixed_base_workspace(size_t n) {
  const size_t a = g1_gen_walk_workspace(FIXED_B), b = align_up(n * 144, 256) + align_up(n * 36, 256);
  return (a > b ? a : b) + 256;
}

int g1_fixed_base_table_build(uint32_t* d_table, void* ws, size_t ws_bytes, hipStream_t stream) {
  for (int w = 0; w < FIXED_W; w++) {
    uint32_t step[8];
    fr_pow2_montgomery(16 * w, step);
    int rc = g1_gen_walk_device(step, step, FIXED_B, d_table + (size_t)w * FIXED_B * 16, ws, ws_bytes, stream);
    if (rc != ZKHIP_OK) return rc;
  }
  return ZKHIP_OK;
}

int g1_fixed_base_mul_device(const uint32_t* d_scalars, size_t n, const uint32_t* d_table, uint32_t* d_out, void* ws, size_t ws_bytes, hipStream_t stream) {
  if (n == 0) return ZKHIP_OK;
  if (n >= (1ull << 31)) { set_error("fixed_base_mul: n too large"); return ZKHIP_EINVAL; }
  if (ws_bytes < g1_fixed_base_workspace(n)) { set_error("fixed_base_mul: workspace too small"); return ZKHIP_EINVAL; }
  char* p = (char*)ws;
  uint32_t* tmp_pts = (uint32_t*)p; p += align_up(n * 144, 256);
  uint32_t* tmp_pref = (uint32_t*)p;
  const uint32_t threads = (uint32_t)((n + FIXED_CHUNK - 1) / FIXED_CHUNK);
  hipLaunchKernelGGL(k_fixed_base_mul, dim3((threads + 63) / 64), dim3(64), 0, stream, d_scalars, (uint32_t)n, d_table, d_out, tmp_pts, tmp_pref);
  HIPCHK(hipGetLastError());
  return ZKHIP_OK;
}

__device__ __forceinline__ void store_table_point(uint32_t* table, size_t idx, const fe& x, const fe& y) {
  uint32_t wx[8], wy[8];
  fe_pack(fe_canon_lt2p<Fq>(x), wx);
  fe_pack(fe_canon_lt2p<Fq>(y), wy);
  uint4* q = reinterpret_cast<uint4*>(table + idx * 16);
  q[0] = make_uint4(wx[0], wx[1], wx[2], wx[3]); q[1] = make_uint4(wx[4], wx[5], wx[6], wx[7]);
  q[2] = make_uint4(wy[0], wy[1], wy[2], wy[3]); q[3] = make_uint4(wy[4], wy[5], wy[6], wy[7]);
}

__global__ void __launch_bounds__(64) k_build_table(const uint32_t* __restrict__ bases, uint32_t n, int c, int W,
                                                    uint32_t* __restrict__ table, uint32_t* __restrict__ tmp_pts,
                                                    uint32_t* __restrict__ tmp_pref, int narrow) {
  const win_layout lay{c, W, narrow};
  const uint32_t i = blockIdx.x * blockDim.x + threadIdx.x;
  if (i >= n) return;
  affine_words pt = load_affine(bases, i);
  if (affine_is_identity(pt)) {
    for (int w = 0; w < W; w++) {
      uint4* q = reinterpret_cast<uint4*>(table + ((size_t)w * n + i) * 16);
      q[0] = q[1] = q[2] = q[3] = make_uint4(0, 0, 0, 0);
    }
    return;
  }
  xyzz P = xyzz_identity();
  xyzz_madd(P, fe_from_ext_lazy(pt.x), fe_from_ext_lazy(pt.y));
  store_table_point(table, i, P.X, P.Y);
  fe pref = fe_one<Fq>();
  for (int w = 1; w < W; w++) {
    for (int k = 0, nd = win_bits(lay, w - 1); k < nd; k++) P = xyzz_dbl(P);
    store_xyzz(tmp_pts, (size_t)(w - 1) * n + i, P);
    store_fe9_generic(tmp_pref, (size_t)(w - 1) * n + i, pref);
    pref = fe_mul<Fq>(pref, fe_mul<Fq>(P.ZZ, P.ZZZ));
  }
  fe inv = fq_inverse(pref);
  for (int w = W - 1; w >= 1; w--) {
    xyzz Q = load_xyzz(tmp_pts, (size_t)(w - 1) * n + i);
    fe pre = load_fe9_generic(tmp_pref, (size_t)(w - 1) * n + i);
    fe winv = fe_mul<Fq>(inv, pre);
    inv = fe_mul<Fq>(inv, fe_mul<Fq>(Q.ZZ, Q.ZZZ));
    fe x = fe_mul<Fq>(fe_mul<Fq>(winv, Q.ZZZ), Q.X);
    fe y = fe_mul<Fq>(fe_mul<Fq>(winv, Q.ZZ), Q.Y);
    store_table_point(table, (size_t)w * n + i, x, y);
  }
}

int prepare_bases_device(const uint32_t* d_bases, size_t n, hipStream_t stream, prepared_bases** out, int c_override, size_t n_whole) {
  if (n == 0 || n >= (1ull << 27)) { set_error("prepare_bases: n = %zu out of range", n); return ZKHIP_EINVAL; }
  const int c = c_override > 0 ? c_override : msm_pick_window_prepared(n);
  if (c < 2 || c > MAX_WINDOW_PREPARED) { set_error("prepare_bases: window bits %d out of range [2,%d]", c, MAX_WINDOW_PREPARED); return ZKHIP_EINVAL; }
  const int W = (256 + c - 1) / c;
  prepared_bases* pb = new prepared_bases();
  pb->n = n; pb->c = c; pb->W = W; pb->table = nullptr; pb->direct = nullptr;
  void *table = nullptr, *tmp = nullptr;
  const size_t tbytes = (size_t)W * n * 64, tmp_pts = align_up((size_t)(W - 1) * n * 144, 256), tmp_pref = align_up((size_t)(W - 1) * n * 36, 256);
  if (hipMalloc(&table, tbytes) != hipSuccess) { delete pb; set_error("prepare_bases: hipMalloc(%zu) failed", tbytes); return ZKHIP_ENOMEM; }
  if (hipMalloc(&tmp, tmp_pts + tmp_pref) != hipSuccess) { (void)hipFree(table); delete pb; set_error("prepare_bases: hipMalloc(%zu) failed", tmp_pts + tmp_pref); return ZKHIP_ENOMEM; }
  hipLaunchKernelGGL(k_build_table, dim3((unsigned)((n + 63) / 64)), dim3(64), 0, stream, d_bases, (uint32_t)n, c, W, (uint32_t*)table,
                     (uint32_t*)tmp, (uint32_t*)((char*)tmp + tmp_pts), msm_narrow_windows(c, W));
  hipError_t e = hipGetLastError();
  if (e == hipSuccess) e = hipStreamSynchronize(stream);
  (void)hipFree(tmp);
  if (e != hipSuccess) { (void)hipFree(table); delete pb; set_error("prepare_bases: %s", hipGetErrorString(e)); return ZKHIP_EHIP; }
  pb->table = (uint32_t*)table;
  if (c_override <= 0 && msm_direct_wanted(std::max(n, n_whole)) && prepare_direct_table(pb, d_bases, stream) != ZKHIP_OK) pb->direct = nullptr;
  *out = pb;
  return ZKHIP_OK;
}

size_t direct_table_bytes(size_t n);
static std::atomic<size_t> g_direct_bytes{0};

void release_prepared(prepared_bases* pb) {
  if (!pb) return;
  if (pb->table) (void)hipFree(pb->table);
  if (pb->direct) { (void)hipFree(pb->direct); g_direct_bytes -= direct_table_bytes(pb->n); }
  delete pb;
}

constexpr int DIRECT_W = 32, DIRECT_M = 128;

__global__ void __launch_bounds__(64) k_direct_build(const uint32_t* __restrict__ wtable , uint32_t n_all,
                                                     uint32_t i0, uint32_t cnt, uint32_t* __restrict__ direct, uint32_t* __restrict__ tmp_pts,
                                                     uint32_t* __restrict__ tmp_pref) {
  const uint32_t tid = blockIdx.x * blockDim.x + threadIdx.x, T = cnt * DIRECT_W;
  if (tid >= T) return;
  const uint32_t i = i0 + tid / DIRECT_W, w = tid % DIRECT_W;
  const affine_words pt = load_affine(wtable, (size_t)w * n_all + i);
  uint4* const slot = reinterpret_cast<uint4*>(direct + ((size_t)i * DIRECT_W + w) * DIRECT_M * 16);
  if (affine_is_identity(pt)) {
    for (int k = 0; k < DIRECT_M * 4; k++) slot[k] = make_uint4(0, 0, 0, 0);
    return;
  }
  slot[0] = make_uint4(pt.x[0], pt.x[1], pt.x[2], pt.x[3]); slot[1] = make_uint4(pt.x[4], pt.x[5], pt.x[6], pt.x[7]);
  slot[2] = make_uint4(pt.y[0], pt.y[1], pt.y[2], pt.y[3]); slot[3] = make_uint4(pt.y[4], pt.y[5], pt.y[6], pt.y[7]);
  const fe x = fe_unpack<0>(pt.x), y = fe_unpack<0>(pt.y);
  xyzz acc = xyzz_identity();
  xyzz_madd(acc, x, y);
  fe pref = fe_one<Fq>();
  for (int k = 2; k <= DIRECT_M; k++) {
    xyzz_madd(acc, x, y);
    store_xyzz(tmp_pts, (size_t)(k - 2) * T + tid, acc);
    store_fe9_generic(tmp_pref, (size_t)(k - 2) * T + tid, pref);
    pref = fe_mul<Fq>(pref, fe_mul<Fq>(acc.ZZ, acc.ZZZ));
  }
  fe inv = fq_inverse(pref);
  for (int k = DIRECT_M; k >= 2; k--) {
    const xyzz Q = load_xyzz(tmp_pts, (size_t)(k - 2) * T + tid);
    const fe pre = load_fe9_generic(tmp_pref, (size_t)(k - 2) * T + tid);
    const fe winv = fe_mul<Fq>(inv, pre);
    inv = fe_mul<Fq>(inv, fe_mul<Fq>(Q.ZZ, Q.ZZZ));
    store_table_point(direct, ((size_t)i * DIRECT_W + w) * DIRECT_M + (k - 1), fe_mul<Fq>(fe_mul<Fq>(winv, Q.ZZZ), Q.X), fe_mul<Fq>(fe_mul<Fq>(winv, Q.ZZ), Q.Y));
  }
}

template <int WPT>
__device__ __forceinline__ void direct_accumulate_body(const uint32_t* __restrict__ scalars, uint32_t n, uint32_t off,
                                                       const uint32_t* __restrict__ direct, uint32_t* __restrict__ partials) {
  constexpr uint32_t GROUPS = DIRECT_W / WPT;
  constexpr int WORDS = WPT >= 4 ? WPT / 4 : 1;
  constexpr int PER = WPT >= 4 ? 4 : WPT;
  const uint32_t tid = blockIdx.x * blockDim.x + threadIdx.x;
  if (tid >= n * GROUPS) return;
  const uint32_t i = tid / GROUPS, g = tid % GROUPS;
  uint32_t w[8];
  load_words(scalars + (size_t)i * 8, w);
  fe c32;
#pragma unroll
  for (int k = 0; k < NL; k++) c32.l[k] = FrParams::FROM_EXT_CANON[k];
  fe sv = fe_canon_lt2p<FrParams>(fe_mul<FrParams>(c32, fe_unpack<0>(w)));
  fe_pack(sv, w);
  uint32_t carry = 0;
  const uint32_t first = g * WPT;
#pragma unroll
  for (int wi = 0; wi < 8; wi++) {
#pragma unroll
    for (int b = 0; b < 4; b++) {
      const uint32_t win = (uint32_t)(wi * 4 + b);
      const uint32_t v = ((w[wi] >> (8 * b)) & 255u) + carry;
      if (win < first) carry = v >= 128u ? 1u : 0u;
    }
  }
  xyzz acc = xyzz_identity();
  static_for<0, WORDS>([&](auto hc) {
    constexpr int h = decltype(hc)::value;
    const uint32_t word = first / 4 + h, byte0 = WPT >= 4 ? 0u : first % 4;
    uint32_t own = 0;
#pragma unroll
    for (int wi = 0; wi < 8; wi++) own = ((uint32_t)wi == word) ? w[wi] : own;
    int32_t dg[PER];
#pragma unroll
    for (int b = 0; b < PER; b++) {
      const uint32_t v = ((own >> (8 * (byte0 + b))) & 255u) + carry;
      if (v >= 128u) { dg[b] = (int32_t)v - 256; carry = 1; } else { dg[b] = (int32_t)v; carry = 0; }
    }
    affine_words pts[PER];
    static_for<0, PER>([&](auto bc) {
      constexpr int b = decltype(bc)::value;
      const uint32_t mag = (uint32_t)(dg[b] < 0 ? -dg[b] : dg[b]);
      const size_t idx = (((size_t)(off + i) * DIRECT_W + first + PER * h + b) * DIRECT_M) + (mag ? mag - 1 : 0);
      pts[b] = load_affine(direct, idx);
    });
    static_for<0, PER>([&](auto bc) {
      constexpr int b = decltype(bc)::value;
      if (dg[b] != 0 && !affine_is_identity(pts[b])) {
        fe x2 = fe_unpack<0>(pts[b].x), y2 = fe_unpack<0>(pts[b].y);
        if (dg[b] < 0) y2 = fe_neg_red(y2, Fq::P2_S1);
        if (xyzz_is_identity(acc)) { acc.X = x2; acc.Y = dg[b] < 0 ? fe_norm(y2) : y2; acc.ZZ = acc.ZZZ = fe_one<Fq>(); }
        else xyzz_madd_nz<true>(acc, x2, y2);
      }
    });
  });
  store_xyzz(partials, tid, acc);
}
static inline int direct_wpt(size_t n) {
  if (n <= 1024) return 1;
  if (n <= 2048) return 2;
  if (n <= 4096) return 4;
  if (n <= 8192) return 2;
  if (n <= 16384) return 4;
  return 8;
}
#define ZK_DIRECT_KERNEL(W, OCC_LO, OCC_HI)                                                                                                          \
  __global__ void __launch_bounds__(128) __attribute__((amdgpu_waves_per_eu(OCC_LO, OCC_HI))) k_direct_accumulate##W(                                 \
      const uint32_t* __restrict__ scalars, uint32_t n, uint32_t off, const uint32_t* __restrict__ direct, uint32_t* __restrict__ partials) {         \
    direct_accumulate_body<W>(scalars, n, off, direct, partials);                                                                                     \
  }
ZK_DIRECT_KERNEL(1, 4, 4)
ZK_DIRECT_KERNEL(2, 4, 4)
ZK_DIRECT_KERNEL(4, 4, 4)
ZK_DIRECT_KERNEL(8, 2, 3)
#undef ZK_DIRECT_KERNEL

__global__ void __launch_bounds__(512) k_points_sum_quad(const uint32_t* __restrict__ in, uint32_t m, uint32_t S, uint32_t* __restrict__ out,
                                                         uint32_t* __restrict__ jac_out) {
  __shared__ __attribute__((aligned(16))) uint32_t xch[8 * 36];
  const uint32_t q = threadIdx.x & 3, quad = threadIdx.x >> 2, wave = threadIdx.x >> 6;
  const uint32_t base = blockIdx.x * 128u * S;
  xyzz acc = xyzz_identity();
#pragma unroll 1
  for (uint32_t s_ = 0; s_ < S; s_++) {
    const uint32_t idx = base + s_ * 128u + quad;
    if (idx < m) acc = xyzz_add_quad(acc, load_xyzz(in, idx), q);
  }
#pragma unroll 1
  for (int mask = 4; mask < 64; mask <<= 1) acc = xyzz_add_quad(acc, xyzz_shfl_xor(acc, mask), q);
  if ((threadIdx.x & 63) == 0) store_xyzz(xch, wave, acc);
  __syncthreads();
  if (wave == 0) {
    acc = (quad < 8) ? load_xyzz(xch, quad) : xyzz_identity();
#pragma unroll 1
    for (int mask = 4; mask < 32; mask <<= 1) acc = xyzz_add_quad(acc, xyzz_shfl_xor(acc, mask), q);
    if (threadIdx.x == 0) {
      if (jac_out) store_jacobian(acc, jac_out);
      else store_xyzz(out, blockIdx.x, acc);
    }
  }
}

size_t direct_table_bytes(size_t n) { return n * (size_t)DIRECT_W * DIRECT_M * 64; }

static inline size_t direct_partials(size_t n) { return n * (size_t)DIRECT_W / (size_t)direct_wpt(n); }
size_t msm_direct_workspace_bytes(size_t n) { return align_up(direct_partials(n) * 144, 256) + align_up(((direct_partials(n) + 511) / 512 + 1) * 144, 256); }

int prepare_direct_table(prepared_bases* pb, const uint32_t* d_bases, hipStream_t stream) {
  const size_t n = pb->n;
  void *direct = nullptr, *wt = nullptr, *tmp = nullptr;
  const size_t slice = std::min<size_t>(n, 4096), T = slice * DIRECT_W;
  const size_t wt_bytes = (size_t)DIRECT_W * n * 64, wtmp_pts = align_up((size_t)(DIRECT_W - 1) * n * 144, 256), wtmp_pref = align_up((size_t)(DIRECT_W - 1) * n * 36, 256);
  const size_t tmp_pts = align_up((size_t)(DIRECT_M - 1) * T * 144, 256), tmp_pref = align_up((size_t)(DIRECT_M - 1) * T * 36, 256);
  const size_t tmp_bytes = std::max(wtmp_pts + wtmp_pref, tmp_pts + tmp_pref);
  {
    static const size_t budget = [] { const char* e = getenv("ZKHIP_DIRECT_BUDGET_GIB"); const long v = e ? atol(e) : 24; return (size_t)(v >= 0 && v <= 4096 ? v : 24) << 30; }();
    size_t free_b = 0, total_b = 0;
    const size_t want = direct_table_bytes(n) + wt_bytes + tmp_bytes;
    if (g_direct_bytes.load() + direct_table_bytes(n) > budget || hipMemGetInfo(&free_b, &total_b) != hipSuccess || want > free_b / 2) {
      (void)hipGetLastError();
      set_error("direct table: %zu bytes not built (budget %zu, in use %zu, free %zu)", direct_table_bytes(n), budget, g_direct_bytes.load(), free_b);
      return ZKHIP_ENOMEM;
    }
  }
  if (hipMalloc(&direct, direct_table_bytes(n)) != hipSuccess) { (void)hipGetLastError(); set_error("direct table: hipMalloc(%zu) failed", direct_table_bytes(n)); return ZKHIP_ENOMEM; }
  if (hipMalloc(&wt, wt_bytes) != hipSuccess || hipMalloc(&tmp, tmp_bytes) != hipSuccess) {
    (void)hipGetLastError();
    (void)hipFree(direct); if (wt) (void)hipFree(wt);
    set_error("direct table: temporary allocation failed");
    return ZKHIP_ENOMEM;
  }
  hipLaunchKernelGGL(k_build_table, dim3((unsigned)((n + 63) / 64)), dim3(64), 0, stream, d_bases, (uint32_t)n, 8, DIRECT_W, (uint32_t*)wt, (uint32_t*)tmp,
                     (uint32_t*)((char*)tmp + wtmp_pts), 0);
  for (size_t i0 = 0; i0 < n; i0 += slice) {
    const size_t cnt = std::min(slice, n - i0);
    hipLaunchKernelGGL(k_direct_build, dim3((unsigned)((cnt * DIRECT_W + 63) / 64)), dim3(64), 0, stream, (const uint32_t*)wt, (uint32_t)n, (uint32_t)i0, (uint32_t)cnt,
                       (uint32_t*)direct, (uint32_t*)tmp, (uint32_t*)((char*)tmp + tmp_pts));
  }
  hipError_t e = hipGetLastError();
  if (e == hipSuccess) e = hipStreamSynchronize(stream);
  (void)hipFree(wt); (void)hipFree(tmp);
  if (e != hipSuccess) { (void)hipFree(direct); set_error("direct table: %s", hipGetErrorString(e)); return ZKHIP_EHIP; }
  pb->direct = (uint32_t*)direct;
  g_direct_bytes += direct_table_bytes(n);
  return ZKHIP_OK;
}

int msm_g1_direct(const uint32_t* d_scalars, size_t n, const prepared_bases* pb, size_t off, uint32_t* d_out, void* ws, size_t ws_bytes, hipStream_t stream) {
  if (!pb || !pb->direct || off + n > pb->n) { set_error("msm_direct: bad range"); return ZKHIP_EINVAL; }
  if (n == 0) { hipLaunchKernelGGL(k_sum_jacobian, dim3(1), dim3(64), 0, stream, (const uint32_t*)nullptr, 0, d_out, 1u); HIPCHK(hipGetLastError()); return ZKHIP_OK; }
  if (ws_bytes < msm_direct_workspace_bytes(n)) { set_error("msm_direct: workspace too small"); return ZKHIP_EINVAL; }
  uint32_t* const partials = (uint32_t*)ws;
  uint32_t* const level1 = (uint32_t*)((char*)ws + align_up(direct_partials(n) * 144, 256));
  prof_begin(stream);
  const int wpt = direct_wpt(n);
  uint32_t m = (uint32_t)direct_partials(n);
  const dim3 grid((m + 127) / 128), block(128);
  const uint32_t* const tab = (const uint32_t*)pb->direct;
  if (wpt == 1) hipLaunchKernelGGL(k_direct_accumulate1, grid, block, 0, stream, d_scalars, (uint32_t)n, (uint32_t)off, tab, partials);
  else if (wpt == 2) hipLaunchKernelGGL(k_direct_accumulate2, grid, block, 0, stream, d_scalars, (uint32_t)n, (uint32_t)off, tab, partials);
  else if (wpt == 4) hipLaunchKernelGGL(k_direct_accumulate4, grid, block, 0, stream, d_scalars, (uint32_t)n, (uint32_t)off, tab, partials);
  else hipLaunchKernelGGL(k_direct_accumulate8, grid, block, 0, stream, d_scalars, (uint32_t)n, (uint32_t)off, tab, partials);
  prof_mark(stream, "direct_accumulate");
  const uint32_t* cur = partials;
  uint32_t* nxt = level1;
  while (m > 512) {
    const uint32_t outs = (m + 511) / 512;
    hipLaunchKernelGGL(k_points_sum_quad, dim3(outs), dim3(512), 0, stream, cur, m, 4u, nxt, (uint32_t*)nullptr);
    const uint32_t* t = cur; cur = nxt; nxt = (uint32_t*)t;
    m = outs;
  }
  hipLaunchKernelGGL(k_points_sum_quad, dim3(1), dim3(512), 0, stream, cur, m, (m + 127) / 128, (uint32_t*)nullptr, d_out);
  prof_mark(stream, "direct_sum");
  HIPCHK(hipGetLastError());
  return ZKHIP_OK;
}

__device__ __forceinline__ xyzz xyzz_negate(const xyzz& a) {
  xyzz r = a;
  r.Y = fe_norm(fe_neg_red(a.Y, Fq::P6_S1));
  return r;
}

__device__ __forceinline__ xyzz xyzz_scalar_mul(const xyzz& B, const uint32_t (&kw)[8]) {
  xyzz acc = xyzz_identity();
  if (xyzz_is_identity(B)) return acc;
  int bit = 253;
  while (bit >= 0 && !((kw[bit >> 5] >> (bit & 31)) & 1)) bit--;
#pragma unroll 1
  for (; bit >= 0; bit--) {
    acc = xyzz_dbl(acc);
    if ((kw[bit >> 5] >> (bit & 31)) & 1) acc = xyzz_add(acc, B);
  }
  return acc;
}

__device__ __forceinline__ void fr_ext_to_integer(const fe& internal_reduced, uint32_t (&kw)[8]) {
  fe raw1;
#pragma unroll
  for (int i = 0; i < NL; i++) raw1.l[i] = FrParams::RAW_ONE[i];
  fe_pack(fe_canon_lt2p<FrParams>(fe_mul<FrParams>(raw1, internal_reduced)), kw);
}

__device__ __forceinline__ fe fr_ext_to_internal(const uint32_t* ext_words) {
  fe k;
#pragma unroll
  for (int i = 0; i < NL; i++) k.l[i] = FrParams::FROM_EXT[i];
  uint32_t w[8];
#pragma unroll
  for (int i = 0; i < 8; i++) w[i] = ext_words[i];
  return fe_mul<FrParams>(k, fe_unpack<0>(w));
}

__device__ __forceinline__ fe fr_pow_small(fe base, uint32_t e) {
  fe acc = fe_one<FrParams>();
  while (e) {
    if (e & 1) acc = fe_mul<FrParams>(acc, base);
    base = fe_sqr<FrParams>(base);
    e >>= 1;
  }
  return acc;
}

struct fr_words { uint32_t w[8]; };

template <int FORMAT>
__global__ void __launch_bounds__(64) k_g1fft_load(const uint32_t* __restrict__ in, uint32_t n, int log_n, fr_words scale, int has_scale,
                                                   uint32_t* __restrict__ work) {
  const uint32_t i = blockIdx.x * blockDim.x + threadIdx.x;
  if (i >= n) return;
  xyzz P;
  if (FORMAT == 0) {
    const affine_words pt = load_affine(in, i);
    P = xyzz_identity();
    if (!affine_is_identity(pt)) xyzz_madd(P, fe_from_ext_lazy(pt.x), fe_from_ext_lazy(pt.y));
  } else {
    P = load_jacobian(in + (size_t)i * 24);
  }
  if (has_scale) {
    uint32_t kw[8];
    fr_ext_to_integer(fr_ext_to_internal(scale.w), kw);
    P = xyzz_scalar_mul(P, kw);
  }
  store_xyzz(work, log_n ? (__brev(i) >> (32 - log_n)) : 0u, P);
}

__global__ void __launch_bounds__(64) k_g1fft_level(uint32_t* __restrict__ work, uint32_t n, int s, int log_n, fr_words omega) {
  const uint32_t t = blockIdx.x * blockDim.x + threadIdx.x;
  if (t >= n / 2) return;
  const uint32_t blocks = n >> s, half = 1u << (s - 1);
  const uint32_t j = t / blocks, blk = t - j * blocks;
  const uint32_t i0 = (blk << s) + j, i1 = i0 + half;
  xyzz T = load_xyzz(work, i1);
  if (j) {
    uint32_t kw[8];
    fr_ext_to_integer(fr_pow_small(fr_ext_to_internal(omega.w), j * blocks), kw);
    T = xyzz_scalar_mul(T, kw);
  }
  const xyzz A = load_xyzz(work, i0);
  store_xyzz(work, i0, xyzz_add(A, T));
  store_xyzz(work, i1, xyzz_add(A, xyzz_negate(T)));
}

__global__ void __launch_bounds__(64) k_g1fft_store_jacobian(const uint32_t* __restrict__ work, uint32_t n, uint32_t* __restrict__ out) {
  const uint32_t i = blockIdx.x * blockDim.x + threadIdx.x;
  if (i < n) store_jacobian(load_xyzz(work, i), out + (size_t)i * 24);
}

constexpr int AFFINE_CHUNK = 32;
static inline uint32_t affine_chunk(size_t n) { uint32_t ch = AFFINE_CHUNK; while (ch > 1 && n / ch < 65536) ch >>= 1; return ch; }
__global__ void __launch_bounds__(64) k_xyzz_to_affine(const uint32_t* __restrict__ work, uint32_t n, uint32_t* __restrict__ out,
                                                       uint32_t* __restrict__ tmp_pref, uint32_t ch) {
  const uint32_t lo = (blockIdx.x * blockDim.x + threadIdx.x) * ch;
  if (lo >= n) return;
  const uint32_t cnt = min(ch, n - lo);
  fe pref = fe_one<Fq>();
  for (uint32_t i = 0; i < cnt; i++) {
    const xyzz Q = load_xyzz(work, lo + i);
    store_fe9_generic(tmp_pref, lo + i, pref);
    if (!xyzz_is_identity(Q)) pref = fe_mul<Fq>(pref, fe_mul<Fq>(Q.ZZ, Q.ZZZ));
  }
  fe inv = fq_inverse(pref);
  for (uint32_t ii = cnt; ii-- > 0;) {
    const xyzz Q = load_xyzz(work, lo + ii);
    uint32_t* o = out + (size_t)(lo + ii) * 16;
    if (xyzz_is_identity(Q)) {
#pragma unroll
      for (int t = 0; t < 16; t++) o[t] = 0;
      continue;
    }
    const fe pre = load_fe9_generic(tmp_pref, lo + ii);
    const fe winv = fe_mul<Fq>(inv, pre);
    inv = fe_mul<Fq>(inv, fe_mul<Fq>(Q.ZZ, Q.ZZZ));
    const fe x = fe_mul<Fq>(fe_mul<Fq>(winv, Q.ZZZ), Q.X);
    const fe y = fe_mul<Fq>(fe_mul<Fq>(winv, Q.ZZ), Q.Y);
    uint32_t wx[8], wy[8];
    fe_to_ext<Fq>(x, wx);
    fe_to_ext<Fq>(y, wy);
#pragma unroll
    for (int t = 0; t < 8; t++) { o[t] = wx[t]; o[8 + t] = wy[t]; }
  }
}

__global__ void __launch_bounds__(64) k_jacobian_to_xyzz(const uint32_t* __restrict__ in, uint32_t n, uint32_t* __restrict__ work) {
  const uint32_t i = blockIdx.x * blockDim.x + threadIdx.x;
  if (i < n) store_xyzz(work, i, load_jacobian(in + (size_t)i * 24));
}

size_t g1_batch_normalize_workspace(size_t n) { return align_up(n * 144, 256) + align_up(n * 36, 256) + 256; }

int g1_batch_normalize_device(const uint32_t* d_in, size_t n, uint32_t* d_out, void* ws, size_t ws_bytes, hipStream_t stream) {
  if (n == 0) return ZKHIP_OK;
  if (n >= (1ull << 31)) { set_error("batch_normalize: n too large"); return ZKHIP_EINVAL; }
  if (ws_bytes < g1_batch_normalize_workspace(n)) { set_error("batch_normalize: workspace too small"); return ZKHIP_EINVAL; }
  uint32_t* work = (uint32_t*)ws;
  uint32_t* pref = (uint32_t*)((char*)ws + align_up(n * 144, 256));
  hipLaunchKernelGGL(k_jacobian_to_xyzz, dim3((unsigned)((n + 63) / 64)), dim3(64), 0, stream, d_in, (uint32_t)n, work);
  { const uint32_t ach = affine_chunk(n); hipLaunchKernelGGL(k_xyzz_to_affine, dim3((unsigned)(((n + ach - 1) / ach + 63) / 64)), dim3(64), 0, stream, work, (uint32_t)n, d_out, pref, ach); }
  HIPCHK(hipGetLastError());
  return ZKHIP_OK;
}

size_t g1_fft_workspace(size_t n) { return align_up(n * 144, 256) + align_up(n * 36, 256) + 256; }

int g1_fft_device(const uint32_t* d_in, int in_format, uint32_t* d_out, int out_format, uint32_t log_n, const uint32_t omega_ext[8],
                  const uint32_t* scale_ext, void* ws, size_t ws_bytes, hipStream_t stream) {
  if (log_n > 26) { set_error("g1_fft: log_n = %u out of range", log_n); return ZKHIP_EINVAL; }
  const size_t n = (size_t)1 << log_n;
  if (ws_bytes < g1_fft_workspace(n)) { set_error("g1_fft: workspace too small"); return ZKHIP_EINVAL; }
  uint32_t* work = (uint32_t*)ws;
  uint32_t* pref = (uint32_t*)((char*)ws + align_up(n * 144, 256));
  fr_words om, sc;
  for (int i = 0; i < 8; i++) { om.w[i] = omega_ext[i]; sc.w[i] = scale_ext ? scale_ext[i] : 0u; }
  const unsigned gb = (unsigned)((n + 63) / 64);
  if (in_format == 0) hipLaunchKernelGGL(k_g1fft_load<0>, dim3(gb), dim3(64), 0, stream, d_in, (uint32_t)n, (int)log_n, sc, scale_ext ? 1 : 0, work);
  else hipLaunchKernelGGL(k_g1fft_load<1>, dim3(gb), dim3(64), 0, stream, d_in, (uint32_t)n, (int)log_n, sc, scale_ext ? 1 : 0, work);
  for (uint32_t s = 1; s <= log_n; s++)
    hipLaunchKernelGGL(k_g1fft_level, dim3((unsigned)((n / 2 + 63) / 64)), dim3(64), 0, stream, work, (uint32_t)n, (int)s, (int)log_n, om);
  if (out_format == 1) hipLaunchKernelGGL(k_g1fft_store_jacobian, dim3(gb), dim3(64), 0, stream, work, (uint32_t)n, d_out);
  else { const uint32_t ach = affine_chunk(n); hipLaunchKernelGGL(k_xyzz_to_affine, dim3((unsigned)(((n + ach - 1) / ach + 63) / 64)), dim3(64), 0, stream, work, (uint32_t)n, d_out, pref, ach); }
  HIPCHK(hipGetLastError());
  return ZKHIP_OK;
}

int sum_jacobian_device(const uint32_t* d_in, int m, uint32_t* d_out, hipStream_t stream, size_t count) {
  if (count == 0) return ZKHIP_OK;
  hipLaunchKernelGGL(k_sum_jacobian, dim3((uint32_t)count), dim3(64), 0, stream, d_in, m, d_out, (uint32_t)count);
  HIPCHK(hipGetLastError());
  return ZKHIP_OK;
}

}
```

zksnap_circuits_halo2_amd/csrc/zkhip_internal.hpp:

```cpp
#pragma once
#include <string>
#include <hip/hip_runtime.h>
#include <cstddef>
#include <cstdint>
#include <cstring>
#include "../../include/zkhip.h"

namespace zkhip {

void set_error(const char* fmt, ...) __attribute__((format(printf, 1, 2)));

#define HIPCHK(x) do { hipError_t e_ = (x); if (e_ != hipSuccess) { ::zkhip::set_error("%s failed: %s", #x, hipGetErrorString(e_)); return ZKHIP_EHIP; } } while (0)

void prof_begin(hipStream_t stream);
void prof_mark(hipStream_t stream, const char* name);

int g1_gen_walk_device(const uint32_t t0_ext[8], const uint32_t d_ext[8], size_t n, uint32_t* d_out, void* ws, size_t ws_bytes, hipStream_t stream);
size_t g1_gen_walk_workspace(size_t n);
size_t g1_fixed_base_table_bytes();
size_t g1_fixed_base_workspace(size_t n);
int g1_fixed_base_table_build(uint32_t* d_table, void* ws, size_t ws_bytes, hipStream_t stream);
int g1_fixed_base_mul_device(const uint32_t* d_scalars, size_t n, const uint32_t* d_table, uint32_t* d_out, void* ws, size_t ws_bytes, hipStream_t stream);
int msm_pick_window(size_t n);
size_t msm_workspace_bytes(size_t n, int c, bool prepared = false, size_t batch = 1, size_t xyzz_bytes = 144);
struct msm_tasks_view {
  int c, W, WB;
  uint32_t B, NB, task_shift;
  size_t max_tasks, nk;
  const void* tasks;
  uint32_t* ntasks;
  uint32_t* max_parts;
  const uint4* order;
  const uint32_t* sorted;
  const uint32_t* task_off;
  uint32_t *partials, *pyrA, *pyrB, *winsum;
  int combine_lanes;
  uint32_t seq_parts;
  const uint32_t* heavy_count;
  const void* heavy;
  uint32_t heavy_cap;
  uint32_t* heavy_done;
  uint32_t* endo;
};
bool msm_uses_glv(bool prepared, size_t batch, size_t xyzz_bytes);
int msm_glv_windows(int c);
int msm_build_tasks(const uint32_t* d_scalars, size_t n, size_t batch, size_t scalar_stride, int c, bool shared_buckets, uint32_t ref_base, uint32_t ref_stride,
                    size_t xyzz_bytes, void* ws, size_t ws_bytes, hipStream_t stream, msm_tasks_view* out, bool glv = false);
size_t msm_g2_workspace_bytes(size_t n);
int msm_g2_device(const uint32_t* d_scalars, const uint32_t* d_bases, size_t n, uint32_t* d_out, void* ws, size_t ws_bytes, hipStream_t stream);
int test_g2_op(int op, const uint32_t* d_a, const uint32_t* d_b, uint32_t* d_out, size_t n, hipStream_t stream);
struct prepared_bases {
  uint32_t* table;
  size_t n;
  int c, W;
  uint32_t* direct = nullptr;
};
size_t direct_table_bytes(size_t n);
size_t msm_direct_workspace_bytes(size_t n);
int prepare_direct_table(prepared_bases* pb, const uint32_t* d_bases, hipStream_t stream);
int msm_g1_direct(const uint32_t* d_scalars, size_t n, const prepared_bases* pb, size_t off, uint32_t* d_out, void* ws, size_t ws_bytes, hipStream_t stream);
int msm_pick_window_prepared(size_t n);
int msm_g1_device(const uint32_t* d_scalars, const uint32_t* d_bases, size_t n, uint32_t* d_out, void* ws, size_t ws_bytes,
                  int c_override, hipStream_t stream, const prepared_bases* prepared = nullptr, size_t prepared_off = 0, size_t batch = 1,
                  size_t scalar_stride = 0);
size_t msm_chunk_workspace_bytes(size_t chunk_cap, int c);
int msm_chunk_add(const uint32_t* d_scalars, size_t n, const prepared_bases* pb, size_t pb_off, size_t chunk_cap, bool first, void* ws, size_t ws_bytes, hipStream_t stream);
int msm_chunk_finish(const prepared_bases* pb, size_t chunk_cap, uint32_t* d_out, void* ws, size_t ws_bytes, hipStream_t stream);
int prepare_bases_device(const uint32_t* d_bases, size_t n, hipStream_t stream, prepared_bases** out, int c_override = 0, size_t n_whole = 0);
void release_prepared(prepared_bases* pb);
int sum_jacobian_device(const uint32_t* d_in, int m, uint32_t* d_out, hipStream_t stream, size_t count = 1);
size_t g1_batch_normalize_workspace(size_t n);
int g1_batch_normalize_device(const uint32_t* d_in, size_t n, uint32_t* d_out, void* ws, size_t ws_bytes, hipStream_t stream);
size_t g1_fft_workspace(size_t n);
int g1_fft_device(const uint32_t* d_in, int in_format, uint32_t* d_out, int out_format, uint32_t log_n, const uint32_t omega_ext[8],
                  const uint32_t* scale_ext, void* ws, size_t ws_bytes, hipStream_t stream);

int ntt_passes(uint32_t L);
int ntt_transform(const uint32_t* d_in, uint32_t in_len, uint32_t in_stride, uint32_t* d_out, uint32_t out_len, uint32_t out_stride,
                  uint32_t batch, uint32_t L, const uint32_t omega_ext[8], const uint32_t* in_scale, uint32_t in_period,
                  const uint32_t* out_scale, uint32_t out_period, uint32_t* tmp0, uint32_t* tmp1, hipStream_t stream);
int fr_mul_periodic_device(uint32_t* d_a, size_t n, const uint32_t* d_table_ext, uint32_t period, hipStream_t stream);
int fr_scale_device(uint32_t* d_a, size_t n, const uint32_t scale_ext[8], hipStream_t stream);
void ntt_clear_cache();

struct arg_ring {
  static constexpr int SLOTS = 8;
  static constexpr size_t SLOT_BYTES = 32768;
  void* host = nullptr;
  hipEvent_t ev[SLOTS] = {};
  bool used[SLOTS] = {};
  int turn = 0;
  int upload(void* dst, const void* src, size_t bytes, hipStream_t stream) {
    if (bytes == 0) return ZKHIP_OK;
    if (bytes > SLOT_BYTES) return plain(dst, src, bytes, stream);
    if (!host && hipHostMalloc(&host, SLOTS * SLOT_BYTES, hipHostMallocDefault) != hipSuccess) { (void)hipGetLastError(); host = nullptr; return plain(dst, src, bytes, stream); }
    const int s = turn;
    turn = (turn + 1) % SLOTS;
    if (!ev[s] && hipEventCreateWithFlags(&ev[s], hipEventDisableTiming) != hipSuccess) { (void)hipGetLastError(); ev[s] = nullptr; return plain(dst, src, bytes, stream); }
    if (used[s] && hipEventSynchronize(ev[s]) != hipSuccess) { set_error("arg_ring: event wait failed"); return ZKHIP_EHIP; }
    void* slot = (char*)host + (size_t)s * SLOT_BYTES;
    std::memcpy(slot, src, bytes);
    if (hipMemcpyAsync(dst, slot, bytes, hipMemcpyHostToDevice, stream) != hipSuccess || hipEventRecord(ev[s], stream) != hipSuccess) { set_error("arg_ring: copy failed"); return ZKHIP_EHIP; }
    used[s] = true;
    return ZKHIP_OK;
  }
  static int plain(void* dst, const void* src, size_t bytes, hipStream_t stream) {
    if (hipMemcpyAsync(dst, src, bytes, hipMemcpyHostToDevice, stream) != hipSuccess || hipStreamSynchronize(stream) != hipSuccess) { set_error("upload of call arguments failed"); return ZKHIP_EHIP; }
    return ZKHIP_OK;
  }
  void release() {
    for (int i = 0; i < SLOTS; i++) if (ev[i]) { if (used[i]) (void)hipEventSynchronize(ev[i]); (void)hipEventDestroy(ev[i]); ev[i] = nullptr; used[i] = false; }
    if (host) { (void)hipHostFree(host); host = nullptr; }
  }
};
static inline int upload_args(arg_ring* ring, void* dst, const void* src, size_t bytes, hipStream_t stream) {
  return ring ? ring->upload(dst, src, bytes, stream) : arg_ring::plain(dst, src, bytes, stream);
}

size_t poly_workspace_bytes(size_t n);
int fr_eval_polynomial_device(const uint32_t* d_a, size_t n, const uint32_t x_host[8], uint32_t* d_result, void* ws, size_t ws_bytes, hipStream_t stream);
size_t poly_batch_workspace_bytes(size_t n, size_t count);
int fr_eval_polynomial_batch_device(const void* const* d_polys_host, size_t count, size_t n, const uint32_t x_host[8], uint32_t* d_results,
                                    void* ws, size_t ws_bytes, hipStream_t stream, arg_ring* ring = nullptr);
int fr_kate_division_device(const uint32_t* d_a, size_t n, const uint32_t b_host[8], uint32_t* d_q, void* ws, size_t ws_bytes, hipStream_t stream);
size_t poly_roots_workspace_bytes(size_t n, uint32_t m);
int fr_divide_by_roots_device(const uint32_t* d_a, size_t n, const uint32_t (*roots_host)[8], uint32_t m, uint32_t* d_q, uint32_t* d_evals, void* ws,
                              size_t ws_bytes, hipStream_t stream);
int fr_prefix_product_device(const uint32_t* d_v, size_t n, uint32_t* d_out, void* ws, size_t ws_bytes, hipStream_t stream);
int fr_batch_invert_device(uint32_t* d_a, size_t n, void* ws, size_t ws_bytes, hipStream_t stream);
int fr_lagrange_cosets_window_device(uint32_t* out_l0, uint32_t* out_last, uint32_t* out_active, size_t W, uint64_t start, uint32_t k, uint32_t ext_k,
                                     uint32_t n_terms, int active_is_sum, const uint32_t consts[10][8], hipStream_t stream);
size_t lincomb_workspace_bytes(size_t count, size_t n);
int fr_linear_combination_device(const void* const* d_cols_host, const uint32_t* coeffs_host, size_t count, size_t n, uint32_t* d_out, void* ws, size_t ws_bytes,
                                 hipStream_t stream, arg_ring* ring = nullptr);
size_t perm_workspace_bytes(uint32_t nperm, uint32_t chunk, uint32_t log_n);
int fr_permutation_products_device(const void* const* d_values_host, const void* const* d_sigmas_host, uint32_t nperm, uint32_t chunk, uint32_t log_n,
                                   size_t usable, const uint32_t beta[8], const uint32_t gamma[8], const uint32_t delta[8], const uint32_t omega[8],
                                   uint32_t* d_z, void* ws, size_t ws_bytes, hipStream_t stream, arg_ring* ring = nullptr);
size_t lookup_products_workspace_bytes(uint32_t n_lookups, uint32_t log_n);
int fr_lookup_products_device(const void* const* d_inputs_host, const void* const* d_tables_host, const uint32_t* d_permuted_inputs, const uint32_t* d_permuted_tables,
                              uint32_t n_lookups, uint32_t log_n, size_t usable, const uint32_t beta[8], const uint32_t gamma[8], uint32_t* d_z, void* ws,
                              size_t ws_bytes, hipStream_t stream, arg_ring* ring = nullptr);

int row_vm_validate(const zkhip_vm_program* p, uint32_t n_columns, uint32_t log_rows, int accumulate);
size_t row_vm_workspace_bytes(const zkhip_vm_program* p, uint32_t n_columns, uint32_t log_rows);
struct vm_staging {
  void* host[2] = {nullptr, nullptr};
  size_t cap[2] = {0, 0};
  hipEvent_t copied[2] = {nullptr, nullptr};
  int turn = 0;
  void release();
};
size_t row_vm_multi_workspace_bytes(const zkhip_vm_program* progs, uint32_t n_progs, uint32_t n_columns, uint32_t log_rows);
int row_vm_device_multi(const zkhip_vm_program* progs, uint32_t n_progs, const void* const* d_columns, uint32_t n_columns, uint32_t log_rows, uint32_t* const* d_outs,
                        void* ws, size_t ws_bytes, hipStream_t stream, vm_staging* staging = nullptr);
bool row_vm_jit_wanted(const zkhip_vm_program* p, uint32_t n_columns, uint32_t log_rows);
bool row_vm_jit_wanted_window(const zkhip_vm_program* p, uint32_t n_columns, uint64_t count);
int row_vm_jit_launch(const zkhip_vm_program* p, const void* const* d_columns, uint32_t n_columns, uint32_t log_rows, bool window, uint64_t row0, uint64_t count,
                      int accumulate, const uint32_t* d_consts, const uint32_t* d_pow_lo, const uint32_t* d_pow_hi, uint32_t* d_out, hipStream_t stream);
void row_vm_jit_clear();
int row_vm_jit_source(const zkhip_vm_program* p, uint32_t n_columns, uint32_t log_rows, std::string* out);
int row_vm_jit_compile_only(const zkhip_vm_program* p, uint32_t n_columns, uint32_t log_rows, size_t* code_bytes);
int row_vm_device(const zkhip_vm_program* p, const void* const* d_columns, uint32_t n_columns, uint32_t log_rows, int accumulate,
                  uint32_t* d_out, void* ws, size_t ws_bytes, hipStream_t stream, vm_staging* staging = nullptr, int* compiled = nullptr);
void row_vm_halos(const zkhip_vm_program* p, uint64_t* lo, uint64_t* hi);
int row_vm_window_device(const zkhip_vm_program* p, const void* const* d_windows, uint32_t n_columns, uint32_t log_rows, uint64_t row0, uint64_t count,
                         int accumulate, uint32_t* d_out, void* ws, size_t ws_bytes, hipStream_t stream, vm_staging* staging = nullptr, int* compiled = nullptr);
int fr_pointwise_mul_device(const uint32_t* d_a, const uint32_t* d_b, size_t n, uint32_t* d_out, hipStream_t stream);
int fr_gather_mul_device(const uint32_t* d_a, uint32_t a_len, const uint32_t* d_ia, const uint32_t* d_b, uint32_t b_len, const uint32_t* d_ib, size_t n,
                         uint32_t* d_out, hipStream_t stream);

size_t lookup_permute_workspace_bytes(size_t usable_rows);
int lookup_permute_device(const uint32_t* d_input, const uint32_t* d_table, size_t usable_rows, uint32_t* d_out_input, uint32_t* d_out_table,
                          void* ws, size_t ws_bytes, hipStream_t stream);
size_t lookup_permute_many_workspace_bytes(uint32_t n_lookups, size_t usable_rows);
int lookup_permute_many_device(const void* const* d_inputs_host, const void* const* d_tables_host, uint32_t n_lookups, size_t n, size_t usable_rows,
                               uint32_t* d_out_input, uint32_t* d_out_table, void* ws, size_t ws_bytes, hipStream_t stream, arg_ring* ring = nullptr);

int fr_random_device(const uint8_t seed[32], uint64_t stream_id, uint64_t first, size_t n, uint32_t* d_out, hipStream_t stream);
size_t fr_random_rows_workspace_bytes(uint32_t n_cols);
int fr_random_rows_device(const uint8_t seed[32], uint64_t stream_id, uint64_t first, const void* const* d_cols_host, uint32_t n_cols, size_t row0, size_t count,
                          void* ws, size_t ws_bytes, hipStream_t stream, arg_ring* ring = nullptr);

int g1_compress_device(const uint32_t* d_points, size_t n, uint32_t* d_out, int layout, hipStream_t stream);
int g1_decompress_device(const uint32_t* d_in, size_t n, uint32_t* d_points, int layout, unsigned long long* d_first_bad, hipStream_t stream);

int test_field_op(int field, int op, const uint32_t* d_a, const uint32_t* d_b, uint32_t* d_out, size_t n, hipStream_t stream);
int g1_check_points_device(const uint32_t* d_points, size_t n, unsigned long long* d_first_bad, hipStream_t stream);
int test_g1_op(int op, const uint32_t* d_a, const uint32_t* d_b, uint32_t* d_out, size_t n, hipStream_t stream);

}
```

Before: 764.0 Mpoints/s.

## Widen coarse bucket groups, add single-pass group sort, fuse scan top and order offsets

Raises the coarse group count to 512 with a variable fine-bit width and templates the coarse and fine sort kernels on chunk size and fine bits. It adds a one-pass per-group fine sort kernel for small groups, folds the scan top pass into the apply pass, and folds order offsets into make_order. It also adds an empty-bucket count so combine can skip empty work. The aim is fewer kernel launches and less scatter and sort traffic, at the cost of more LDS per block and more code paths.

Result: no change. 766.4 Mpoints/s, median of 6 (+0.3%).

```diff
diff --git a/zksnap_circuits_halo2_amd/csrc/msm.hip b/zksnap_circuits_halo2_amd/csrc/msm.hip
--- a/zksnap_circuits_halo2_amd/csrc/msm.hip
+++ b/zksnap_circuits_halo2_amd/csrc/msm.hip
@@ -14,7 +14,9 @@
 static inline size_t align_up(size_t v, size_t a) { return (v + a - 1) / a * a; }
 
 constexpr int FINE_BITS = 12;
-constexpr int MAX_GROUPS = 128;
+constexpr int MIN_FINE_BITS = 10;
+constexpr int MAX_GROUPS = 512;
+constexpr int COARSE_GROUPS = 128;
 constexpr int MAX_WIDE_W = 16;
 struct win_layout { int c, W, narrow; };
 __host__ __device__ __forceinline__ int win_bits(const win_layout& L, int w) { return w < L.W - L.narrow ? L.c : L.c - 1; }
@@ -117,9 +119,9 @@
 }
 
 __global__ void __launch_bounds__(1024) k_digits_wide(const uint32_t* __restrict__ scalars, int32_t* __restrict__ digits, uint32_t n, uint32_t n_pad,
-                                                       int c, int W, uint32_t* __restrict__ gcount, int narrow) {
+                                                       int c, int W, uint32_t* __restrict__ gcount, int narrow, int G, int fbits) {
   __shared__ uint32_t cnt[MAX_WIDE_W * MAX_GROUPS];
-  for (uint32_t t = threadIdx.x; t < (uint32_t)W * MAX_GROUPS; t += blockDim.x) cnt[t] = 0;
+  for (uint32_t t = threadIdx.x; t < (uint32_t)(W * G); t += blockDim.x) cnt[t] = 0;
   __syncthreads();
   const win_layout lay{c, W, narrow};
   for (uint32_t i = blockIdx.x * blockDim.x + threadIdx.x; i < n_pad; i += gridDim.x * blockDim.x) {
@@ -149,12 +151,12 @@
       int32_t d;
       if (v >= half) { d = (int32_t)v - (int32_t)(1u << cw); carry = 1; } else { d = (int32_t)v; carry = 0; }
       digits[(size_t)win * n_pad + i] = d;
-      if (d != 0) atomicAdd(&cnt[win * MAX_GROUPS + (((uint32_t)(d < 0 ? -d : d) - 1) >> FINE_BITS)], 1u);
-    }
-  }
-  __syncthreads();
-  for (uint32_t t = threadIdx.x; t < (uint32_t)W * MAX_GROUPS; t += blockDim.x)
-    if (cnt[t]) atomicAdd(&gcount[t], cnt[t]);
+      if (d != 0) atomicAdd(&cnt[win * G + (int)(((uint32_t)(d < 0 ? -d : d) - 1) >> fbits)], 1u);
+    }
+  }
+  __syncthreads();
+  for (uint32_t t = threadIdx.x; t < (uint32_t)(W * G); t += blockDim.x)
+    if (cnt[t]) atomicAdd(&gcount[(t / (uint32_t)G) * MAX_GROUPS + t % (uint32_t)G], cnt[t]);
 }
 
 namespace glv {
@@ -343,10 +345,10 @@
 
 
 __global__ void __launch_bounds__(1024) k_coarse_count(const int32_t* __restrict__ digits, uint32_t n_pad, uint32_t chunk, uint32_t* __restrict__ gcount, uint32_t gstride) {
-  __shared__ uint32_t cnt[MAX_GROUPS];
+  __shared__ uint32_t cnt[COARSE_GROUPS];
   const int win = blockIdx.y;
   const uint32_t lo = blockIdx.x * chunk, hi = min(n_pad, lo + chunk);
-  if (threadIdx.x < MAX_GROUPS) cnt[threadIdx.x] = 0;
+  if (threadIdx.x < COARSE_GROUPS) cnt[threadIdx.x] = 0;
   __syncthreads();
   const uint4* dv = reinterpret_cast<const uint4*>(digits + (size_t)win * n_pad);
   const uint32_t v_lo = lo >> 2, v_hi = hi >> 2;
@@ -365,49 +367,68 @@
     }
   }
   __syncthreads();
-  if (threadIdx.x < MAX_GROUPS && cnt[threadIdx.x]) atomicAdd(&gcount[win * MAX_GROUPS + threadIdx.x], cnt[threadIdx.x]);
+  if (threadIdx.x < COARSE_GROUPS && cnt[threadIdx.x]) atomicAdd(&gcount[win * MAX_GROUPS + threadIdx.x], cnt[threadIdx.x]);
 }
 
 constexpr uint32_t COARSE_CHUNK = 8192;
+constexpr uint32_t COARSE_CHUNK_WIDE = 16384;
+template <uint32_t CH, int NG>
 __global__ void __launch_bounds__(1024) k_coarse_sorted(const int32_t* __restrict__ digits, uint32_t n_pad, uint32_t* __restrict__ gcursor,
                                                         uint32_t* __restrict__ stage_ref, uint16_t* __restrict__ stage_fine,
-                                                        uint32_t ref_base, uint32_t ref_stride, uint32_t gstride) {
-  __shared__ uint32_t cur[MAX_GROUPS], delta[MAX_GROUPS];
-  __shared__ uint32_t refs[COARSE_CHUNK];
-  __shared__ uint16_t fines[COARSE_CHUNK];
-  __shared__ uint32_t mask[COARSE_CHUNK / 32], wpre[COARSE_CHUNK / 32];
+                                                        uint32_t ref_base, uint32_t ref_stride, uint32_t gstride, int fbits) {
+  constexpr int VPL = CH / 4096, GPL = NG / 64, MPL = CH / 32 / 64;
+  static_assert(CH % 4096 == 0 && NG % 64 == 0 && NG <= MAX_GROUPS, "a lane owns VPL 4-digit vectors; one wavefront scans GPL groups per lane");
+  __shared__ uint32_t cur[NG], delta[NG];
+  __shared__ uint32_t refs[CH];
+  __shared__ uint16_t fines[CH];
+  __shared__ uint32_t mask[CH / 32], wpre[CH / 32];
   const int win = blockIdx.y;
   const uint32_t gbase = (uint32_t)win * gstride;
-  const uint32_t lo = blockIdx.x * COARSE_CHUNK, hi = min(n_pad, lo + COARSE_CHUNK);
+  const uint32_t lo = blockIdx.x * CH, hi = min(n_pad, lo + CH);
   if (lo >= hi) return;
-  if (threadIdx.x < MAX_GROUPS) cur[threadIdx.x] = 0;
-  if (threadIdx.x < COARSE_CHUNK / 32) mask[threadIdx.x] = 0;
+  for (uint32_t t = threadIdx.x; t < (uint32_t)NG; t += blockDim.x) cur[t] = 0;
+  if (threadIdx.x < CH / 32) mask[threadIdx.x] = 0;
   __syncthreads();
   const uint4* dv = reinterpret_cast<const uint4*>(digits + (size_t)win * n_pad);
   const uint32_t v_lo = lo >> 2, v_hi = hi >> 2;
-  static_assert(COARSE_CHUNK == 8192, "a lane owns two 4-digit vectors of the chunk");
-  const uint32_t vi = v_lo + threadIdx.x, vj = vi + 1024u;
-  const uint4 q0 = vi < v_hi ? dv[vi] : make_uint4(0, 0, 0, 0), q1 = vj < v_hi ? dv[vj] : make_uint4(0, 0, 0, 0);
-  const int32_t d8[8] = {(int32_t)q0.x, (int32_t)q0.y, (int32_t)q0.z, (int32_t)q0.w, (int32_t)q1.x, (int32_t)q1.y, (int32_t)q1.z, (int32_t)q1.w};
-#pragma unroll
-  for (int k = 0; k < 8; k++) {
-    const int32_t d = d8[k];
-    if (d != 0) atomicAdd(&cur[gbase + (((uint32_t)(d < 0 ? -d : d) - 1) >> FINE_BITS)], 1u);
+  const uint32_t vi = v_lo + threadIdx.x;
+  int32_t dd[4 * VPL];
+#pragma unroll
+  for (int u = 0; u < VPL; u++) {
+    const uint32_t vj = vi + 1024u * u;
+    const uint4 q = vj < v_hi ? dv[vj] : make_uint4(0, 0, 0, 0);
+    dd[4 * u] = (int32_t)q.x; dd[4 * u + 1] = (int32_t)q.y; dd[4 * u + 2] = (int32_t)q.z; dd[4 * u + 3] = (int32_t)q.w;
+  }
+#pragma unroll
+  for (int k = 0; k < 4 * VPL; k++) {
+    const int32_t d = dd[k];
+    if (d != 0) atomicAdd(&cur[gbase + (((uint32_t)(d < 0 ? -d : d) - 1) >> fbits)], 1u);
   }
   __syncthreads();
   if (threadIdx.x < 64) {
-    const uint32_t c0 = cur[2 * threadIdx.x], c1 = cur[2 * threadIdx.x + 1], s = c0 + c1;
+    uint32_t cg[GPL], lg[GPL], s = 0;
+#pragma unroll
+    for (int k = 0; k < GPL; k++) { cg[k] = cur[GPL * threadIdx.x + k]; s += cg[k]; }
     uint32_t x = s;
 #pragma unroll
     for (int off = 1; off < 64; off <<= 1) {
       const uint32_t y = __shfl_up(x, off, 64);
       if ((int)threadIdx.x >= off) x += y;
     }
-    const uint32_t l0 = x - s, l1 = l0 + c0;
+    {
+      uint32_t run = x - s;
+#pragma unroll
+      for (int k = 0; k < GPL; k++) { lg[k] = run; run += cg[k]; }
+    }
     uint32_t* const wcur = gcursor + (uint32_t)win * MAX_GROUPS;
-    const uint32_t g0 = c0 ? atomicAdd(&wcur[2 * threadIdx.x], c0) : 0u, g1 = c1 ? atomicAdd(&wcur[2 * threadIdx.x + 1], c1) : 0u;
-    cur[2 * threadIdx.x] = l0; cur[2 * threadIdx.x + 1] = l1;
-    const uint32_t nz = (c0 != 0) + (c1 != 0);
+    uint32_t gg[GPL];
+#pragma unroll
+    for (int k = 0; k < GPL; k++) gg[k] = cg[k] ? atomicAdd(&wcur[GPL * threadIdx.x + k], cg[k]) : 0u;
+#pragma unroll
+    for (int k = 0; k < GPL; k++) cur[GPL * threadIdx.x + k] = lg[k];
+    uint32_t nz = 0;
+#pragma unroll
+    for (int k = 0; k < GPL; k++) nz += cg[k] != 0;
     uint32_t y = nz;
 #pragma unroll
     for (int off = 1; off < 64; off <<= 1) {
@@ -415,12 +436,13 @@
       if ((int)threadIdx.x >= off) y += t;
     }
     uint32_t rank = y - nz;
-    if (c0) { delta[rank++] = g0 - l0; atomicOr(&mask[l0 >> 5], 1u << (l0 & 31)); }
-    if (c1) { delta[rank] = g1 - l1; atomicOr(&mask[l1 >> 5], 1u << (l1 & 31)); }
+#pragma unroll
+    for (int k = 0; k < GPL; k++)
+      if (cg[k]) { delta[rank++] = gg[k] - lg[k]; atomicOr(&mask[lg[k] >> 5], 1u << (lg[k] & 31)); }
     __threadfence_block();
-    uint32_t pc[4], ps = 0;
-#pragma unroll
-    for (int k = 0; k < 4; k++) { pc[k] = (uint32_t)__popc(mask[4 * threadIdx.x + k]); ps += pc[k]; }
+    uint32_t pc[MPL], ps = 0;
+#pragma unroll
+    for (int k = 0; k < MPL; k++) { pc[k] = (uint32_t)__popc(mask[MPL * threadIdx.x + k]); ps += pc[k]; }
     uint32_t z = ps;
 #pragma unroll
     for (int off = 1; off < 64; off <<= 1) {
@@ -429,22 +451,22 @@
     }
     uint32_t zb = z - ps;
 #pragma unroll
-    for (int k = 0; k < 4; k++) { wpre[4 * threadIdx.x + k] = zb; zb += pc[k]; }
+    for (int k = 0; k < MPL; k++) { wpre[MPL * threadIdx.x + k] = zb; zb += pc[k]; }
   }
   __syncthreads();
   const uint32_t rbase = ref_base + (uint32_t)win * ref_stride;
 #pragma unroll
-  for (int k = 0; k < 8; k++) {
-    const int32_t d = d8[k];
+  for (int k = 0; k < 4 * VPL; k++) {
+    const int32_t d = dd[k];
     if (d != 0) {
       const uint32_t b = (uint32_t)(d < 0 ? -d : d) - 1;
-      const uint32_t pos = atomicAdd(&cur[gbase + (b >> FINE_BITS)], 1u);
-      refs[pos] = (rbase + (k < 4 ? vi : vj) * 4 + (k & 3)) | (d < 0 ? 0x80000000u : 0u);
-      fines[pos] = (uint16_t)(b & ((1u << FINE_BITS) - 1));
-    }
-  }
-  __syncthreads();
-  const uint32_t total = cur[MAX_GROUPS - 1];
+      const uint32_t pos = atomicAdd(&cur[gbase + (b >> fbits)], 1u);
+      refs[pos] = (rbase + (vi + 1024u * (k >> 2)) * 4 + (k & 3)) | (d < 0 ? 0x80000000u : 0u);
+      fines[pos] = (uint16_t)(b & ((1u << fbits) - 1));
+    }
+  }
+  __syncthreads();
+  const uint32_t total = cur[NG - 1];
   for (uint32_t i = threadIdx.x; i < total; i += blockDim.x) {
     const uint32_t r = wpre[i >> 5] + (uint32_t)__popc(mask[i >> 5] & ((2u << (i & 31)) - 1u)) - 1u;
     const uint32_t pos = delta[r] + i;
@@ -456,28 +478,40 @@
 constexpr uint32_t SORT_CHUNK = 28672;
 
 __global__ void __launch_bounds__(64) k_group_offsets(const uint32_t* __restrict__ wcount, int W, int G, uint32_t* __restrict__ goff, uint32_t* __restrict__ wcursor,
-                                                       uint32_t* __restrict__ cstart, uint32_t chunk) {
+                                                       uint32_t* __restrict__ cstart, uint32_t chunk, uint32_t one_pass_cap) {
+  constexpr int GPL = MAX_GROUPS / 64;
   if (blockIdx.x != 0 || threadIdx.x >= 64) return;
   const int lane = threadIdx.x;
-  uint32_t c0 = 0, c1 = 0;
+  static_assert(GPL == 8, "a lane reads its eight counts of a window as two vectors");
+  uint32_t cg[GPL], kg[GPL], cs = 0, ks = 0;
+#pragma unroll
+  for (int k = 0; k < GPL; k++) cg[k] = 0;
   for (int w = 0; w < W; w++) {
-    if (2 * lane < G) c0 += wcount[w * MAX_GROUPS + 2 * lane];
-    if (2 * lane + 1 < G) c1 += wcount[w * MAX_GROUPS + 2 * lane + 1];
-  }
-  const uint32_t k0 = (c0 + chunk - 1) / chunk, k1 = (c1 + chunk - 1) / chunk;
-  uint32_t x = c0 + c1, y = k0 + k1;
+    const uint4* row = reinterpret_cast<const uint4*>(wcount + w * MAX_GROUPS + GPL * lane);
+    const uint4 a = row[0], b = row[1];
+    cg[0] += a.x; cg[1] += a.y; cg[2] += a.z; cg[3] += a.w; cg[4] += b.x; cg[5] += b.y; cg[6] += b.z; cg[7] += b.w;
+  }
+#pragma unroll
+  for (int k = 0; k < GPL; k++) {
+    kg[k] = (one_pass_cap && cg[k] <= one_pass_cap) ? 0u : (cg[k] + chunk - 1) / chunk;
+    cs += cg[k]; ks += kg[k];
+  }
+  uint32_t x = cs, y = ks;
 #pragma unroll
   for (int off = 1; off < 64; off <<= 1) {
     const uint32_t xs = __shfl_up(x, off, 64), ys = __shfl_up(y, off, 64);
     if (lane >= off) { x += xs; y += ys; }
   }
-  const uint32_t ex = x - (c0 + c1), ey = y - (k0 + k1);
-  if (2 * lane < G) { goff[2 * lane] = ex; cstart[2 * lane] = ey; }
-  if (2 * lane + 1 < G) { goff[2 * lane + 1] = ex + c0; cstart[2 * lane + 1] = ey + k0; }
-  uint32_t r0 = ex, r1 = ex + c0;
-  for (int w = 0; w < W; w++) {
-    if (2 * lane < G) { wcursor[w * MAX_GROUPS + 2 * lane] = r0; r0 += wcount[w * MAX_GROUPS + 2 * lane]; }
-    if (2 * lane + 1 < G) { wcursor[w * MAX_GROUPS + 2 * lane + 1] = r1; r1 += wcount[w * MAX_GROUPS + 2 * lane + 1]; }
+  uint32_t ex = x - cs, ey = y - ks;
+#pragma unroll
+  for (int k = 0; k < GPL; k++) {
+    const int g = GPL * lane + k;
+    if (g < G) {
+      goff[g] = ex; cstart[g] = ey;
+      uint32_t r = ex;
+      for (int w = 0; w < W; w++) { wcursor[w * MAX_GROUPS + g] = r; r += wcount[w * MAX_GROUPS + g]; }
+    }
+    ex += cg[k]; ey += kg[k];
   }
   if (lane == 63) { goff[G] = x; cstart[G] = y; }
 }
@@ -496,13 +530,15 @@
   }
 }
 
+template <int FBITS>
 __global__ void __launch_bounds__(1024) k_fine_sorted(const uint16_t* __restrict__ stage_fine, const uint32_t* __restrict__ stage_ref,
                                                       const uint32_t* __restrict__ goff, const uint32_t* __restrict__ cstart, int G,
                                                       uint32_t* __restrict__ cursor, uint32_t* __restrict__ sorted) {
   extern __shared__ uint32_t hist[];
-  constexpr uint32_t FB = 1u << FINE_BITS;
+  constexpr uint32_t FB = 1u << FBITS;
+  constexpr int PER = FB / 1024;
   constexpr uint32_t CHUNK = SORT_CHUNK;
-  static_assert(FB == 4096, "one thread owns four buckets in the scan");
+  static_assert(FB % 1024 == 0 && PER <= 4, "one thread owns PER buckets in the scan");
   __shared__ uint32_t wsum[16];
   uint32_t* cur = hist;
   uint32_t* delta = hist + FB;
@@ -517,9 +553,9 @@
   __syncthreads();
   fine_histogram(stage_fine, start, end, cur);
   __syncthreads();
-  uint32_t c[4], l[4], s = 0;
-#pragma unroll
-  for (int k = 0; k < 4; k++) { c[k] = cur[4 * threadIdx.x + k]; s += c[k]; }
+  uint32_t c[PER], l[PER], s = 0;
+#pragma unroll
+  for (int k = 0; k < PER; k++) { c[k] = cur[PER * threadIdx.x + k]; s += c[k]; }
   const int lane = threadIdx.x & 63, wave = threadIdx.x >> 6;
   uint32_t x = s;
 #pragma unroll
@@ -534,15 +570,17 @@
   for (int i = 0; i < 16; i++) if (i < wave) before += wsum[i];
   uint32_t run = before + x - s;
   uint32_t* gl = cursor + (size_t)g * FB;
-  uint32_t gb[4];
-#pragma unroll
-  for (int k = 0; k < 4; k++) { l[k] = run; run += c[k]; }
-#pragma unroll
-  for (int k = 0; k < 4; k++) gb[k] = c[k] ? atomicAdd(&gl[4 * threadIdx.x + k], c[k]) : 0u;
+  uint32_t gb[PER];
+#pragma unroll
+  for (int k = 0; k < PER; k++) { l[k] = run; run += c[k]; }
+#pragma unroll
+  for (int k = 0; k < PER; k++) gb[k] = c[k] ? atomicAdd(&gl[PER * threadIdx.x + k], c[k]) : 0u;
   {
     uint32_t* mask = refs + CHUNK;
     uint32_t* wpre = mask + CHUNK / 32;
-    const uint32_t nz = (c[0] != 0) + (c[1] != 0) + (c[2] != 0) + (c[3] != 0);
+    uint32_t nz = 0;
+#pragma unroll
+    for (int k = 0; k < PER; k++) nz += c[k] != 0;
     uint32_t y = nz;
 #pragma unroll
     for (int off = 1; off < 64; off <<= 1) {
@@ -557,8 +595,8 @@
 #pragma unroll
     for (int i = 0; i < 16; i++) if (i < wave) rank += wsum[i];
 #pragma unroll
-    for (int k = 0; k < 4; k++) {
-      cur[4 * threadIdx.x + k] = l[k];
+    for (int k = 0; k < PER; k++) {
+      cur[PER * threadIdx.x + k] = l[k];
       if (c[k]) {
         delta[rank++] = gb[k] - l[k];
         atomicOr(&mask[l[k] >> 5], 1u << (l[k] & 31));
@@ -620,6 +658,72 @@
   }
 }
 
+constexpr uint32_t FINE_GROUP_CAP = 36864;
+__global__ void __launch_bounds__(1024) k_fine_group(const uint16_t* __restrict__ stage_fine, const uint32_t* __restrict__ stage_ref,
+                                                     const uint32_t* __restrict__ goff, const uint32_t* __restrict__ cstart, int G, int fbits,
+                                                     uint32_t cap, uint32_t* __restrict__ count, uint32_t* __restrict__ sorted) {
+  extern __shared__ uint32_t hist[];
+  __shared__ uint32_t wsum[16];
+  const uint32_t FB = 1u << fbits, per = FB >> 10;
+  uint32_t* cur = hist;
+  uint32_t* refs = hist + FB;
+  if (blockIdx.x >= (uint32_t)G) {
+    const uint32_t w = blockIdx.x - (uint32_t)G;
+    if (w >= cstart[G]) return;
+    uint32_t glo = 0, ghi = (uint32_t)G;
+    while (ghi - glo > 1) { const uint32_t mid = (glo + ghi) >> 1; if (cstart[mid] <= w) glo = mid; else ghi = mid; }
+    const uint32_t g = glo;
+    const uint32_t start = goff[g] + (w - cstart[g]) * SORT_CHUNK, end = min(goff[g + 1], start + SORT_CHUNK);
+    for (uint32_t b = threadIdx.x; b < FB; b += blockDim.x) cur[b] = 0;
+    __syncthreads();
+    fine_histogram(stage_fine, start, end, cur);
+    __syncthreads();
+    uint32_t* gl = count + (size_t)g * FB;
+    for (uint32_t b = threadIdx.x; b < FB; b += blockDim.x) {
+      const uint32_t v = cur[b];
+      if (v) atomicAdd(&gl[b], v);
+    }
+    return;
+  }
+  const uint32_t g = blockIdx.x;
+  const uint32_t start = goff[g], end = goff[g + 1], cnt_n = end - start;
+  if (cnt_n > cap) return;
+  for (uint32_t b = threadIdx.x; b < FB; b += blockDim.x) cur[b] = 0;
+  __syncthreads();
+  fine_histogram(stage_fine, start, end, cur);
+  __syncthreads();
+  uint32_t c[4], s = 0;
+#pragma unroll
+  for (uint32_t k = 0; k < 4; k++) { c[k] = k < per ? cur[per * threadIdx.x + k] : 0u; s += c[k]; }
+  const int lane = threadIdx.x & 63, wave = threadIdx.x >> 6;
+  uint32_t x = s;
+#pragma unroll
+  for (int off = 1; off < 64; off <<= 1) {
+    const uint32_t y = __shfl_up(x, off, 64);
+    if (lane >= off) x += y;
+  }
+  if (lane == 63) wsum[wave] = x;
+  __syncthreads();
+  uint32_t run = x - s;
+#pragma unroll
+  for (int i = 0; i < 16; i++) if (i < wave) run += wsum[i];
+  uint32_t* gl = count + (size_t)g * FB;
+#pragma unroll
+  for (uint32_t k = 0; k < 4; k++)
+    if (k < per) { gl[per * threadIdx.x + k] = c[k]; cur[per * threadIdx.x + k] = run; run += c[k]; }
+  __syncthreads();
+  for (uint32_t p = start + threadIdx.x; p < end; p += FINE_BATCH * blockDim.x) {
+    uint32_t f[FINE_BATCH], r[FINE_BATCH];
+#pragma unroll
+    for (int k = 0; k < FINE_BATCH; k++) { const uint32_t q = p + k * blockDim.x; f[k] = q < end ? stage_fine[q] : 0xffffffffu; r[k] = q < end ? stage_ref[q] : 0u; }
+#pragma unroll
+    for (int k = 0; k < FINE_BATCH; k++) if (f[k] != 0xffffffffu) refs[atomicAdd(&cur[f[k]], 1u)] = r[k];
+  }
+  __syncthreads();
+  uint32_t* const dst = sorted + start;
+  for (uint32_t i = threadIdx.x; i < cnt_n; i += blockDim.x) dst[i] = refs[i];
+}
+
 constexpr int SCAN_BLOCK = 256, SCAN_PER_THREAD = 4,
           SCAN_TILE = SCAN_BLOCK * SCAN_PER_THREAD;
 
@@ -678,25 +782,40 @@
   if (threadIdx.x == 0) { *total0 = run0; *total1 = run1; }
 }
 
+constexpr uint32_t SCAN_SELF_TOP_MAX = 1024;
+template <bool SELF_TOP>
 __global__ void __launch_bounds__(SCAN_BLOCK) k_scan_apply2(const uint32_t* __restrict__ in, uint32_t n, const uint32_t* __restrict__ sums0,
-                                                            const uint32_t* __restrict__ sums1, const uint32_t* __restrict__ total0,
-                                                            const uint32_t* __restrict__ total1, uint32_t* __restrict__ offset,
+                                                            const uint32_t* __restrict__ sums1, uint32_t* __restrict__ total0,
+                                                            uint32_t* __restrict__ total1, uint32_t* __restrict__ offset,
                                                             uint32_t* __restrict__ cursor, uint32_t* __restrict__ task_off, uint32_t task_shift) {
   __shared__ uint32_t lds[4];
   const uint32_t base = blockIdx.x * SCAN_TILE + threadIdx.x * SCAN_PER_THREAD;
   uint32_t v[SCAN_PER_THREAD], s0 = 0, s1 = 0;
 #pragma unroll
   for (int i = 0; i < SCAN_PER_THREAD; i++) { v[i] = base + i < n ? in[base + i] : 0; s0 += v[i]; s1 += scan_xform<1>(v[i], task_shift); }
-  uint32_t t0, t1;
-  uint32_t e0 = block_exclusive_scan(s0, lds, t0) + sums0[blockIdx.x];
-  uint32_t e1 = block_exclusive_scan(s1, lds, t1) + sums1[blockIdx.x];
+  uint32_t t0, t1, before0, before1, all0 = 0, all1 = 0;
+  if (SELF_TOP) {
+    const uint32_t nb = blockIdx.x == 0 ? gridDim.x : blockIdx.x;
+    uint32_t p0 = 0, p1 = 0;
+    for (uint32_t i = threadIdx.x; i < nb; i += SCAN_BLOCK) { p0 += sums0[i]; p1 += sums1[i]; }
+    block_exclusive_scan(p0, lds, t0);
+    block_exclusive_scan(p1, lds, t1);
+    before0 = blockIdx.x == 0 ? 0u : t0; before1 = blockIdx.x == 0 ? 0u : t1;
+    all0 = t0; all1 = t1;
+  } else {
+    before0 = sums0[blockIdx.x]; before1 = sums1[blockIdx.x];
+  }
+  uint32_t e0 = block_exclusive_scan(s0, lds, t0) + before0;
+  uint32_t e1 = block_exclusive_scan(s1, lds, t1) + before1;
 #pragma unroll
   for (int i = 0; i < SCAN_PER_THREAD; i++) {
     if (base + i < n) { offset[base + i] = e0; cursor[base + i] = e0; task_off[base + i] = e1; }
     e0 += v[i];
     e1 += scan_xform<1>(v[i], task_shift);
   }
-  if (blockIdx.x == 0 && threadIdx.x == 0) { offset[n] = *total0; task_off[n] = *total1; }
+  if (SELF_TOP) {
+    if (blockIdx.x == 0 && threadIdx.x == 0) { *total0 = all0; *total1 = all1; offset[n] = all0; task_off[n] = all1; }
+  } else if (blockIdx.x == 0 && threadIdx.x == 0) { offset[n] = *total0; task_off[n] = *total1; }
 }
 
 constexpr uint32_t SCAN_SINGLE_MAX = 8192;
@@ -764,10 +883,12 @@
 __global__ void __launch_bounds__(256) k_make_tasks(const uint32_t* __restrict__ offset, const uint32_t* __restrict__ task_off,
                                                     uint32_t nbuckets, task_t* __restrict__ tasks, uint32_t task_shift,
                                                     uint32_t* __restrict__ max_parts, uint32_t* __restrict__ len_count, uint32_t seq_parts,
-                                                    uint32_t* __restrict__ heavy_count, uint2* __restrict__ heavy, uint32_t heavy_cap) {
+                                                    uint32_t* __restrict__ heavy_count, uint2* __restrict__ heavy, uint32_t heavy_cap,
+                                                    uint32_t* __restrict__ empty_count ) {
   __shared__ uint32_t lh[MAX_TASK_LEN + 1];
   if (threadIdx.x <= MAX_TASK_LEN) lh[threadIdx.x] = 0;
   __syncthreads();
+  uint32_t n_empty = 0;
   uint32_t nt = 0;
   const uint32_t lane = threadIdx.x & 63u;
   for (uint32_t base = blockIdx.x * blockDim.x + (threadIdx.x & ~63u); base < nbuckets; base += gridDim.x * blockDim.x) {
@@ -795,6 +916,7 @@
         if (idx + i < heavy_cap) heavy[idx + i] = make_uint2(k, i);
     }
     nt = max(nt, m);
+    n_empty += (k < nbuckets && m == 0);
     unsigned long long big = __ballot(coop);
     while (big) {
       const int src = __ffsll((long long)big) - 1;
@@ -815,6 +937,11 @@
 #pragma unroll
   for (int off = 32; off >= 1; off >>= 1) nt = max(nt, (uint32_t)__shfl_xor((int)nt, off, 64));
   if ((threadIdx.x & 63) == 0 && nt > 1) atomicMax(max_parts, nt);
+  if (empty_count) {
+#pragma unroll
+    for (int off = 32; off >= 1; off >>= 1) n_empty += (uint32_t)__shfl_xor((int)n_empty, off, 64);
+    if ((threadIdx.x & 63) == 0 && n_empty) atomicAdd(empty_count, n_empty);
+  }
 }
 
 __global__ void k_order_offsets(const uint32_t* __restrict__ len_count, uint32_t* __restrict__ len_cursor) {
@@ -834,13 +961,28 @@
 }
 
 constexpr int ORDER_JMAX = 64;
+template <bool SELF_OFFSETS>
 __global__ void __launch_bounds__(256) k_make_order(const uint32_t* __restrict__ offset, const uint32_t* __restrict__ task_off,
                                                     uint32_t nbuckets, uint32_t task_shift, uint32_t* __restrict__ len_cursor,
-                                                    const uint32_t* __restrict__ sorted, uint4* __restrict__ order) {
+                                                    const uint32_t* __restrict__ sorted, uint4* __restrict__ order, const uint32_t* __restrict__ len_count) {
   __shared__ uint32_t lh[MAX_TASK_LEN + 1];
   __shared__ uint32_t jcnt[ORDER_JMAX + 1], joff[ORDER_JMAX + 1];
+  __shared__ uint32_t lfirst[MAX_TASK_LEN + 1];
   if (threadIdx.x <= MAX_TASK_LEN) lh[threadIdx.x] = 0;
   if (threadIdx.x <= ORDER_JMAX) jcnt[threadIdx.x] = 0;
+  if (SELF_OFFSETS && threadIdx.x < 64) {
+    const int lane = threadIdx.x, L0 = MAX_TASK_LEN - 2 * lane, L1 = L0 - 1;
+    const uint32_t c0 = len_count[L0], c1 = len_count[L1];
+    uint32_t x = c0 + c1;
+#pragma unroll
+    for (int off = 1; off < 64; off <<= 1) {
+      const uint32_t y = __shfl_up(x, off, 64);
+      if (lane >= off) x += y;
+    }
+    const uint32_t ex = x - (c0 + c1);
+    lfirst[L0] = ex;
+    lfirst[L1] = ex + c0;
+  }
   __syncthreads();
   const uint32_t full = 1u << task_shift, step = gridDim.x * blockDim.x;
   for (uint32_t k = blockIdx.x * blockDim.x + threadIdx.x; k < nbuckets; k += step) {
@@ -857,12 +999,15 @@
   if (threadIdx.x == 0) {
     uint32_t run = 0;
     for (int j = 0; j <= ORDER_JMAX; j++) { joff[j] = run; run += jcnt[j]; }
-    const uint32_t base = run ? atomicAdd(&len_cursor[full], run) : 0u;
+    const uint32_t base = run ? atomicAdd(&len_cursor[full], run) + (SELF_OFFSETS ? lfirst[full] : 0u) : 0u;
     for (int j = 0; j <= ORDER_JMAX; j++) joff[j] += base;
   }
-  if (threadIdx.x <= MAX_TASK_LEN && threadIdx.x != full) { const uint32_t v = lh[threadIdx.x]; lh[threadIdx.x] = v ? atomicAdd(&len_cursor[threadIdx.x], v) : 0u; }
-  __syncthreads();
-  if (threadIdx.x == 0 && lh[full]) lh[full] = atomicAdd(&len_cursor[full], lh[full]);
+  if (threadIdx.x <= MAX_TASK_LEN && threadIdx.x != full) {
+    const uint32_t v = lh[threadIdx.x];
+    lh[threadIdx.x] = v ? atomicAdd(&len_cursor[threadIdx.x], v) + (SELF_OFFSETS ? lfirst[threadIdx.x] : 0u) : 0u;
+  }
+  __syncthreads();
+  if (threadIdx.x == 0 && lh[full]) lh[full] = atomicAdd(&len_cursor[full], lh[full]) + (SELF_OFFSETS ? lfirst[full] : 0u);
   __syncthreads();
   const uint32_t lane = threadIdx.x & 63u;
   for (uint32_t base = blockIdx.x * blockDim.x + (threadIdx.x & ~63u); base < nbuckets; base += step) {
@@ -1030,9 +1175,11 @@
 __global__ void __launch_bounds__(128) k_combine_seq(const uint32_t* __restrict__ task_off, uint32_t nbuckets,
                                                      uint32_t* __restrict__ partials, uint32_t* __restrict__ buckets,
                                                      uint32_t seq_parts, uint32_t blocks, const uint32_t* __restrict__ heavy_count,
-                                                     const uint2* __restrict__ heavy, uint32_t heavy_cap, uint32_t* __restrict__ heavy_done, uint32_t quad_max) {
+                                                     const uint2* __restrict__ heavy, uint32_t heavy_cap, uint32_t* __restrict__ heavy_done, uint32_t quad_max,
+                                                     const uint32_t* __restrict__ max_parts, const uint32_t* __restrict__ empty_count ) {
   __shared__ __attribute__((aligned(16))) uint32_t xch[64 * 36];
   if (blockIdx.x >= blocks) { combine_heavy_buckets(blockIdx.x - blocks, task_off, partials, buckets, heavy_count, heavy, heavy_cap, heavy_done, xch, quad_max); return; }
+  if (empty_count && *max_parts <= 1 && *empty_count == 0) return;
   const uint32_t gid = blockIdx.x * blockDim.x + threadIdx.x;
   const uint32_t k = gid / COMBINE_LANES, q = gid % COMBINE_LANES;
   const bool live = k < nbuckets;
@@ -1290,6 +1437,30 @@
   return shared_buckets && thr_prep > 0 && n_in >= (size_t)thr_prep;
 }
 
+static uint32_t msm_fine_group_cap() {
+  static const uint32_t cap = [] {
+    if (getenv("ZKHIP_NO_FINE_GROUP") != nullptr || getenv("ZKHIP_NO_FUSED_COUNT") != nullptr) return 0u;
+    const char* e = getenv("ZKHIP_FINE_GROUP_CAP");
+    const long v = e ? atol(e) : 0;
+    return v >= 1 && v < (long)FINE_GROUP_CAP ? (uint32_t)v : FINE_GROUP_CAP;
+  }();
+  return cap;
+}
+static int msm_fine_group_bits(int c, int W, size_t n, bool shared_buckets, size_t K, bool glv) {
+  if (c <= 16 || !shared_buckets || K != 1 || glv || msm_fine_group_cap() == 0) return 0;
+  const size_t B = (size_t)1 << (c - 1), entries = (size_t)W * n;
+  for (int fb = MIN_FINE_BITS; fb <= FINE_BITS; fb++) {
+    const size_t G = B >> fb;
+    if (G == 0 || G > (size_t)MAX_GROUPS) continue;
+    const size_t room = std::min<size_t>(FINE_GROUP_CAP, (160 * 1024 - 1024) / 4 - ((size_t)1 << fb));
+    if ((entries / G) * 9 / 8 <= room) return fb;
+  }
+  return 0;
+}
+
+constexpr size_t GC_GOFF = 1024, GC_CSTART = 2048, GC_COUNT = 4096, GC_CURSOR = GC_COUNT + (size_t)MAX_WIDE_W * MAX_GROUPS,
+                 GC_WORDS = GC_CURSOR + (size_t)MAX_WIDE_W * MAX_GROUPS;
+static_assert(GC_GOFF + MAX_GROUPS + 1 <= GC_CSTART && GC_CSTART + MAX_GROUPS + 1 <= GC_COUNT, "gcounters regions overlap");
 static msm_layout msm_lay_out(char* base, size_t n_in, size_t K, int c, bool prepared, size_t xyzz_bytes = 144, bool glv = false) {
   msm_layout L;
   const size_t n = glv ? 2 * n_in : n_in;
@@ -1309,7 +1480,7 @@
   L.stage_ref = wide ? (uint32_t*)carve(entries * sizeof(uint32_t)) : nullptr;
   L.stage_fine = wide ? (uint16_t*)carve(entries * sizeof(uint16_t)) : nullptr;
   L.zero_lo = p;
-  L.gcounters = wide ? (uint32_t*)carve(32768) : nullptr;
+  L.gcounters = wide ? (uint32_t*)carve(GC_WORDS * sizeof(uint32_t)) : nullptr;
   L.counters = (uint32_t*)carve(2048);
   L.count = (uint32_t*)carve((NB + 1) * sizeof(uint32_t));
   L.heavy_done = (uint32_t*)carve((size_t)L.heavy_cap * sizeof(uint32_t));
@@ -1360,11 +1531,14 @@
   const uint32_t NB = (uint32_t)WB * B;
   if ((size_t)W * n * K >= (1ull << 32) || (size_t)WB * B >= (1ull << 31)) { set_error("msm: W*n*batch overflows 32-bit slot index"); return ZKHIP_EINVAL; }
   if (c > 16 && (!shared_buckets || K != 1)) { set_error("msm: windows above 16 bits need one shared bucket set"); return ZKHIP_EINVAL; }
-  if (wide && !shared_buckets && (size_t)W * (B >> FINE_BITS) > (size_t)MAX_GROUPS) { set_error("msm: two-level sort: %d windows x %u groups exceed %d", W, B >> FINE_BITS, MAX_GROUPS); return ZKHIP_EINVAL; }
+  if (wide && !shared_buckets && (size_t)W * (B >> FINE_BITS) > (size_t)COARSE_GROUPS) { set_error("msm: two-level sort: %d windows x %u groups exceed %d", W, B >> FINE_BITS, COARSE_GROUPS); return ZKHIP_EINVAL; }
   if (wide && W > MAX_WIDE_W) { set_error("msm: %d windows of %d bits exceed the wide path's %d", W, c, MAX_WIDE_W); return ZKHIP_EINVAL; }
   const msm_layout lay = msm_lay_out((char*)ws, n_in, K, c, shared_buckets, xyzz_bytes, glv);
   if (ws_bytes < lay.total) { set_error("msm: workspace too small (%zu < %zu bytes)", ws_bytes, lay.total); return ZKHIP_EINVAL; }
   const uint32_t task_shift = lay.task_shift;
+  const int group_bits = msm_fine_group_bits(c, W, n, shared_buckets, batch, glv);
+  const int fbits = group_bits ? group_bits : FINE_BITS;
+  const bool wide_shared = wide && shared_buckets && K == 1 && c > 16;
   const uint32_t n_pad = (uint32_t)((n + 7) & ~(size_t)7);
   void* const digits = lay.digits;
   uint32_t* const stage_ref = lay.stage_ref;
@@ -1389,7 +1563,8 @@
       static const unsigned wg_knob = [] { const char* e = getenv("ZKHIP_DIGIT_WGS"); const int v = e ? atoi(e) : 0; return v >= 64 && v <= 4096 ? (unsigned)v : 0u; }();
       const unsigned wg_cap = wg_knob ? wg_knob : (n_pad > (1u << 21) ? 1024u : 512u);
       const unsigned wblocks = (unsigned)std::min<size_t>(((size_t)n_pad + 1023) / 1024, wg_cap);
-      hipLaunchKernelGGL(k_digits_wide, dim3(wblocks), dim3(1024), 0, stream, d_scalars, (int32_t*)digits, (uint32_t)n, n_pad, c, W, gcounters + 1024, narrow);
+      hipLaunchKernelGGL(k_digits_wide, dim3(wblocks), dim3(1024), 0, stream, d_scalars, (int32_t*)digits, (uint32_t)n, n_pad, c, W, gcounters + GC_COUNT, narrow,
+                         (int)(B >> fbits), fbits);
     } else {
       hipLaunchKernelGGL(k_digits<int32_t>, dim3(dblocks), dim3(256), 0, stream, d_scalars, (int32_t*)digits, (uint32_t)n, n_pad, c, W, K, sstride, narrow);
     }
@@ -1408,42 +1583,63 @@
   std::call_once(attr_once[cur_dev & 63], [&] {
     hipError_t e = hipFuncSetAttribute((const void*)k_sort_pass<false>, hipFuncAttributeMaxDynamicSharedMemorySize, 128 * 1024);
     if (e == hipSuccess) e = hipFuncSetAttribute((const void*)k_sort_pass<true>, hipFuncAttributeMaxDynamicSharedMemorySize, 128 * 1024);
-    if (e == hipSuccess) e = hipFuncSetAttribute((const void*)k_fine_sorted, hipFuncAttributeMaxDynamicSharedMemorySize, (2 * (1 << FINE_BITS) + SORT_CHUNK + SORT_CHUNK / 16) * 4);
+    if (e == hipSuccess) e = hipFuncSetAttribute((const void*)k_fine_sorted<12>, hipFuncAttributeMaxDynamicSharedMemorySize, (2 * (1 << FINE_BITS) + SORT_CHUNK + SORT_CHUNK / 16) * 4);
+    if (e == hipSuccess) e = hipFuncSetAttribute((const void*)k_fine_sorted<11>, hipFuncAttributeMaxDynamicSharedMemorySize, (2 * (1 << FINE_BITS) + SORT_CHUNK + SORT_CHUNK / 16) * 4);
+    if (e == hipSuccess) e = hipFuncSetAttribute((const void*)k_fine_sorted<10>, hipFuncAttributeMaxDynamicSharedMemorySize, (2 * (1 << FINE_BITS) + SORT_CHUNK + SORT_CHUNK / 16) * 4);
+    if (e == hipSuccess) e = hipFuncSetAttribute((const void*)k_fine_group, hipFuncAttributeMaxDynamicSharedMemorySize, 160 * 1024 - 1024);
     attr_err[cur_dev & 63] = e;
   });
   HIPCHK(attr_err[cur_dev & 63]);
   const uint32_t gstride = (wide && !shared_buckets) ? (B >> FINE_BITS) : 0u;
-  const int G = wide ? (int)(gstride ? (uint32_t)W * gstride : (B >> FINE_BITS)) : 1;
+  const int G = wide ? (int)(gstride ? (uint32_t)W * gstride : (B >> fbits)) : 1;
   const uint32_t sort_chunk = SORT_CHUNK;
-  const uint32_t sort_chunks = (uint32_t)(((size_t)W * n + sort_chunk - 1) / sort_chunk) + (uint32_t)G;
+  const uint32_t group_cap = group_bits ? std::min<uint32_t>(msm_fine_group_cap(), (160 * 1024 - 1024) / 4 - (1u << fbits)) : 0u;
+  const uint32_t sort_chunks = (uint32_t)(((size_t)W * n + sort_chunk - 1) / sort_chunk) + (group_cap ? (uint32_t)std::min<size_t>((size_t)G, (size_t)W * n / group_cap) : (uint32_t)G);
+  const size_t fine_sorted_lds = (size_t)(2u * (1u << FINE_BITS) + SORT_CHUNK + SORT_CHUNK / 16) * 4;
   const uint32_t wb_stride = shared_buckets ? 0u : B;
   if (wide) {
     static const bool fused_count2 = getenv("ZKHIP_NO_FUSED_COUNT") == nullptr;
     if (!fused_count2 || glv)
-      hipLaunchKernelGGL(k_coarse_count, dim3(chunks, W), dim3(1024), 0, stream, (const int32_t*)digits, n_pad, chunk, gcounters + 1024, gstride);
-    hipLaunchKernelGGL(k_group_offsets, dim3(1), dim3(64), 0, stream, gcounters + 1024, W, G, gcounters + 128, gcounters + 3072, gcounters + 512, sort_chunk);
-    static_assert(MAX_GROUPS == 128, "k_coarse_sorted scans two groups per lane of one wavefront");
-    hipLaunchKernelGGL(k_coarse_sorted, dim3((n_pad + COARSE_CHUNK - 1) / COARSE_CHUNK, W), dim3(1024), 0, stream, (const int32_t*)digits, n_pad, gcounters + 3072,
-                       stage_ref, stage_fine, ref_base, ref_stride, gstride);
+      hipLaunchKernelGGL(k_coarse_count, dim3(chunks, W), dim3(1024), 0, stream, (const int32_t*)digits, n_pad, chunk, gcounters + GC_COUNT, gstride);
+    hipLaunchKernelGGL(k_group_offsets, dim3(1), dim3(64), 0, stream, gcounters + GC_COUNT, W, G, gcounters + GC_GOFF, gcounters + GC_CURSOR, gcounters + GC_CSTART, sort_chunk, group_cap);
+    if (G > COARSE_GROUPS)
+      hipLaunchKernelGGL((k_coarse_sorted<COARSE_CHUNK_WIDE, MAX_GROUPS>), dim3((n_pad + COARSE_CHUNK_WIDE - 1) / COARSE_CHUNK_WIDE, W), dim3(1024), 0, stream, (const int32_t*)digits, n_pad,
+                         gcounters + GC_CURSOR, stage_ref, stage_fine, ref_base, ref_stride, gstride, fbits);
+    else
+      hipLaunchKernelGGL((k_coarse_sorted<COARSE_CHUNK, COARSE_GROUPS>), dim3((n_pad + COARSE_CHUNK - 1) / COARSE_CHUNK, W), dim3(1024), 0, stream, (const int32_t*)digits, n_pad,
+                         gcounters + GC_CURSOR, stage_ref, stage_fine, ref_base, ref_stride, gstride, fbits);
     prof_mark(stream, "coarse");
-    hipLaunchKernelGGL(k_fine_count, dim3(sort_chunks), dim3(1024), 0, stream, stage_fine, gcounters + 128, gcounters + 512, G, count, sort_chunk);
+    if (group_cap)
+      hipLaunchKernelGGL(k_fine_group, dim3((uint32_t)G + sort_chunks), dim3(1024), ((size_t)group_cap + ((size_t)1 << fbits)) * 4, stream, stage_fine, stage_ref,
+                         gcounters + GC_GOFF, gcounters + GC_CSTART, G, fbits, group_cap, count, sorted);
+    else
+      hipLaunchKernelGGL(k_fine_count, dim3(sort_chunks), dim3(1024), 0, stream, stage_fine, gcounters + GC_GOFF, gcounters + GC_CSTART, G, count, sort_chunk);
   } else {
     hipLaunchKernelGGL(k_sort_pass<false>, dim3(chunks, W, K), dim3(1024), lds, stream, (const int16_t*)digits, n_pad, chunk, c, count, (uint32_t*)nullptr, wb_stride, ref_base, ref_stride);
   }
   prof_mark(stream, "count");
   const uint32_t nblk = (NB + SCAN_TILE - 1) / SCAN_TILE;
   const bool scan_single = NB <= SCAN_SINGLE_MAX;
+  static const bool self_top_on = getenv("ZKHIP_NO_SCAN_SELF_TOP") == nullptr, self_order_on = getenv("ZKHIP_NO_ORDER_SELF") == nullptr,
+                    combine_skip_on = getenv("ZKHIP_NO_COMBINE_SKIP") == nullptr;
+  const bool self_top = wide_shared && self_top_on && !scan_single && nblk <= SCAN_SELF_TOP_MAX;
+  const bool self_order = wide_shared && self_order_on && !scan_single;
+  uint32_t* const empty_count = (wide_shared && combine_skip_on) ? counters + 4 : nullptr;
   if (scan_single) {
     hipLaunchKernelGGL(k_scan_single<0>, dim3(1), dim3(1024), 0, stream, count, (uint32_t)NB, counters + 0, offset, cursor, 0u, (uint32_t*)nullptr);
   } else {
     hipLaunchKernelGGL(k_scan_sums2, dim3(nblk), dim3(SCAN_BLOCK), 0, stream, count, NB, bsum1, bsum2, task_shift);
-    hipLaunchKernelGGL(k_scan_top2, dim3(1), dim3(SCAN_BLOCK), 0, stream, bsum1, bsum2, nblk, counters + 0, counters + 1);
-    hipLaunchKernelGGL(k_scan_apply2, dim3(nblk), dim3(SCAN_BLOCK), 0, stream, count, NB, bsum1, bsum2, counters + 0, counters + 1, offset, cursor, task_off, task_shift);
+    if (self_top) hipLaunchKernelGGL(k_scan_apply2<true>, dim3(nblk), dim3(SCAN_BLOCK), 0, stream, count, NB, bsum1, bsum2, counters + 0, counters + 1, offset, cursor, task_off, task_shift);
+    else {
+      hipLaunchKernelGGL(k_scan_top2, dim3(1), dim3(SCAN_BLOCK), 0, stream, bsum1, bsum2, nblk, counters + 0, counters + 1);
+      hipLaunchKernelGGL(k_scan_apply2<false>, dim3(nblk), dim3(SCAN_BLOCK), 0, stream, count, NB, bsum1, bsum2, counters + 0, counters + 1, offset, cursor, task_off, task_shift);
+    }
   }
   prof_mark(stream, "scan");
   if (wide) {
-    hipLaunchKernelGGL(k_fine_sorted, dim3(sort_chunks), dim3(1024), (size_t)(2u * (1u << FINE_BITS) + SORT_CHUNK + SORT_CHUNK / 16) * 4, stream, stage_fine, stage_ref,
-                       gcounters + 128, gcounters + 512, G, cursor, sorted);
+    if (fbits == 10) hipLaunchKernelGGL(k_fine_sorted<10>, dim3(sort_chunks), dim3(1024), fine_sorted_lds, stream, stage_fine, stage_ref, gcounters + GC_GOFF, gcounters + GC_CSTART, G, cursor, sorted);
+    else if (fbits == 11) hipLaunchKernelGGL(k_fine_sorted<11>, dim3(sort_chunks), dim3(1024), fine_sorted_lds, stream, stage_fine, stage_ref, gcounters + GC_GOFF, gcounters + GC_CSTART, G, cursor, sorted);
+    else hipLaunchKernelGGL(k_fine_sorted<12>, dim3(sort_chunks), dim3(1024), fine_sorted_lds, stream, stage_fine, stage_ref, gcounters + GC_GOFF, gcounters + GC_CSTART, G, cursor, sorted);
   }
   else hipLaunchKernelGGL(k_sort_pass<true>, dim3(chunks, W, K), dim3(1024), lds, stream, (const int16_t*)digits, n_pad, chunk, c, cursor, sorted, wb_stride, ref_base, ref_stride);
   prof_mark(stream, "scatter");
@@ -1452,16 +1648,17 @@
   if (scan_single) {
     hipLaunchKernelGGL(k_scan_single<1>, dim3(1), dim3(1024), 0, stream, count, (uint32_t)NB, counters + 1, task_off, (uint32_t*)nullptr, task_shift, counters + 192);
     hipLaunchKernelGGL(k_make_tasks, dim3(task_blocks), dim3(256), 0, stream, offset, task_off, NB, tasks, task_shift, counters + 2, (uint32_t*)nullptr, lay.seq_parts,
-                       counters + 3, lay.heavy, lay.heavy_cap);
+                       counters + 3, lay.heavy, lay.heavy_cap, empty_count);
   } else {
     hipLaunchKernelGGL(k_make_tasks, dim3(task_blocks), dim3(256), 0, stream, offset, task_off, NB, tasks, task_shift, counters + 2, counters + 32, lay.seq_parts,
-                       counters + 3, lay.heavy, lay.heavy_cap);
-    hipLaunchKernelGGL(k_order_offsets, dim3(1), dim3(64), 0, stream, counters + 32, counters + 192);
-  }
-  hipLaunchKernelGGL(k_make_order, dim3(task_blocks), dim3(256), 0, stream, offset, task_off, NB, task_shift, counters + 192, sorted, order);
+                       counters + 3, lay.heavy, lay.heavy_cap, empty_count);
+    if (!self_order) hipLaunchKernelGGL(k_order_offsets, dim3(1), dim3(64), 0, stream, counters + 32, counters + 192);
+  }
+  if (self_order) hipLaunchKernelGGL(k_make_order<true>, dim3(task_blocks), dim3(256), 0, stream, offset, task_off, NB, task_shift, counters + 192, sorted, order, (const uint32_t*)(counters + 32));
+  else hipLaunchKernelGGL(k_make_order<false>, dim3(task_blocks), dim3(256), 0, stream, offset, task_off, NB, task_shift, counters + 192, sorted, order, (const uint32_t*)nullptr);
   prof_mark(stream, "tasks");
   out->c = c; out->W = W; out->WB = WB; out->B = B; out->NB = NB; out->task_shift = task_shift; out->max_tasks = lay.max_tasks; out->nk = n * K;
-  out->tasks = tasks; out->ntasks = counters + 1; out->max_parts = counters + 2; out->order = order; out->sorted = sorted; out->task_off = task_off;
+  out->tasks = tasks; out->ntasks = counters + 1; out->max_parts = counters + 2; out->empty_count = empty_count; out->order = order; out->sorted = sorted; out->task_off = task_off;
   out->partials = lay.partials; out->pyrA = lay.pyrA; out->pyrB = lay.pyrB; out->winsum = lay.winsum;
   out->combine_lanes = lay.combine_lanes; out->seq_parts = lay.seq_parts; out->heavy_count = counters + 3; out->heavy = lay.heavy; out->heavy_cap = lay.heavy_cap; out->heavy_done = lay.heavy_done;
   out->endo = lay.endo;
@@ -1497,7 +1694,8 @@
       if (quad) hipLaunchKernelGGL(k_combine_seq_quad<L>, dim3(blocks + HEAVY_WGS), dim3(128), 0, stream, task_off, NB, partials, buckets, seq_parts, blocks,   \
                                    tv.heavy_count, (const uint2*)tv.heavy, tv.heavy_cap, tv.heavy_done, heavy_quad_max);                              \
       else hipLaunchKernelGGL(k_combine_seq<L>, dim3(blocks + HEAVY_WGS), dim3(128), 0, stream, task_off, NB, partials, buckets, seq_parts, blocks,             \
-                              tv.heavy_count, (const uint2*)tv.heavy, tv.heavy_cap, tv.heavy_done, heavy_quad_max);                                   \
+                              tv.heavy_count, (const uint2*)tv.heavy, tv.heavy_cap, tv.heavy_done, heavy_quad_max, (const uint32_t*)tv.max_parts,       \
+                              (const uint32_t*)tv.empty_count);                                                                                        \
     } while (0)
     if (combine_lanes == 1) ZK_LAUNCH_COMBINE(1);
     else if (combine_lanes == 2) ZK_LAUNCH_COMBINE(2);
diff --git a/zksnap_circuits_halo2_amd/csrc/zkhip_internal.hpp b/zksnap_circuits_halo2_amd/csrc/zkhip_internal.hpp
--- a/zksnap_circuits_halo2_amd/csrc/zkhip_internal.hpp
+++ b/zksnap_circuits_halo2_amd/csrc/zkhip_internal.hpp
@@ -30,6 +30,7 @@
   const void* tasks;
   uint32_t* ntasks;
   uint32_t* max_parts;
+  uint32_t* empty_count;
   const uint4* order;
   const uint32_t* sorted;
   const uint32_t* task_off;
```
